# peternara/FashionVisualExpl-recommend

Hardware: AMD Instinct MI355X
Metric: BPR triplets/sec (higher is better)
Workload: dtype bf16

## Files before the change

fashionvisualexpl_recommend_amd/_ffi.py:

```python
import ctypes as C
import os

HERE = os.path.dirname(os.path.abspath(__file__))
LIB_PATH = os.environ.get("BPRX_LIB") or os.path.join(HERE, "libbprx.so")
ABI_VERSION = 6
FLAG_EXPORT_USER_GRAD = 1
FLAG_EXPORT_ITEM_GRAD = 2
FLAG_DENSE_ALLREDUCE = 4
FLAG_ADAM_SWEEP, FLAG_ADAM_LAZY = 8, 16

MODEL = {"bprmf": 0, "vbpr": 1}
OPTIMIZER = {"sgd": 0, "adam_tf23": 1}
FEAT_DTYPE = {"fp32": 0, "bf16": 1, "fp8": 2}
E_INVALID, E_STATE = -1, -2
E_RANGE, E_NOMEM = -4, -5
PHASES = ["cast_Et", "proj_fwd", "triplet_grad", "proj_bwd", "reduce_parts", "apply", "dense_update", "loss_reduce", "item_seg", "seg_alloc", "row_count", "adam_catchup"]


class BprxError(RuntimeError):
    def __init__(self, code, msg):
        super().__init__("libbprx error %d: %s" % (code, msg))
        self.code = code


class Config(C.Structure):
    _fields_ = [("abi_version", C.c_int32), ("model", C.c_int32), ("num_users", C.c_int32), ("num_items", C.c_int32),
                ("embed_k", C.c_int32), ("embed_d", C.c_int32), ("feat_dim", C.c_int32), ("feat_dtype", C.c_int32),
                ("optimizer", C.c_int32), ("device", C.c_int32), ("max_batch", C.c_int64),
                ("lr", C.c_float), ("reg", C.c_float), ("beta1", C.c_float), ("beta2", C.c_float),
                ("epsilon", C.c_float), ("flags", C.c_int32), ("feat_scale", C.c_float)]


FACTORED_FIELDS = ["Ea", "Eb", "A", "Ap", "m_Ea", "v_Ea", "m_Eb", "v_Eb", "m_A", "v_A", "m_Ap", "v_Ap"]


class Factored(C.Structure):
    _fields_ = [("feat_dim_a", C.c_int32), ("feat_dim_b", C.c_int32), ("embed_a", C.c_int32), ("embed_b", C.c_int32),
                ("neg_bias_reg", C.c_float)] + [(n, C.c_void_p) for n in FACTORED_FIELDS]


ACF_WEIGHTS = ["component.W_0_u", "component.W_0_i", "component.b_0", "component.W_1", "component.b_1",
               "item.W_0_u", "item.W_0_iv", "item.W_0_ip", "item.W_0_ix", "item.b_0", "item.W_1", "item.b_1"]


ACF_GRADIENT = {"detached": 0, "full": 1}


class Acf(C.Structure):
    _fields_ = [("feat_m", C.c_int32), ("feat_c", C.c_int32), ("width_c", C.c_int32), ("width_i", C.c_int32),
                ("feat_dtype", C.c_int32), ("F", C.c_void_p), ("train_ptr", C.c_void_p), ("train_items", C.c_void_p),
                ("eval_ptr", C.c_void_p), ("eval_items", C.c_void_p), ("Pi", C.c_void_p), ("m_Pi", C.c_void_p),
                ("v_Pi", C.c_void_p), ("w", C.c_void_p * 12), ("m_w", C.c_void_p * 12), ("v_w", C.c_void_p * 12)]


AF_WEIGHTS = ["color.W1", "color.b1", "color.W2", "edges.conv", "edges.conv_b", "edges.W2", "class.W1", "class.b1", "class.W2",
              "attention.W_1", "attention.b_1", "attention.W_2", "attention.b_2"]


class Attentive(C.Structure):
    _fields_ = [("dim_color", C.c_int32), ("dim_class", C.c_int32), ("width", C.c_int32), ("dropout", C.c_float),
                ("seed", C.c_uint64), ("edges", C.c_void_p), ("color", C.c_void_p), ("cls", C.c_void_p),
                ("w", C.c_void_p * 13), ("m_w", C.c_void_p * 13), ("v_w", C.c_void_p * 13)]


TABLE_FIELDS = ["Gu", "Gi", "Bi", "Tu", "F", "E", "Bp", "m_Gu", "v_Gu", "m_Gi", "v_Gi", "m_Bi", "v_Bi",
                "m_Tu", "v_Tu", "m_E", "v_E", "m_Bp", "v_Bp"]


class Tables(C.Structure):
    _fields_ = [(n, C.c_void_p) for n in TABLE_FIELDS]


_lib = None


def lib():
    global _lib
    if _lib is not None:
        return _lib
    import torch
    if not os.path.exists(LIB_PATH):
        raise ImportError("libbprx.so not found at %s: build it with `python -m fashionvisualexpl_recommend_amd.build` "
                          "(hipcc --offload-arch=gfx950); there is no CPU fallback" % LIB_PATH)
    L = C.CDLL(LIB_PATH)
    vp, i32, i64, u32, f32 = C.c_void_p, C.c_int32, C.c_int64, C.c_uint32, C.c_float
    sig = {
        "bprx_abi_version": (C.c_int, []),
        "bprx_create": (C.c_int, [C.POINTER(Config), C.POINTER(vp)]),
        "bprx_destroy": (C.c_int, [vp]),
        "bprx_last_error": (C.c_char_p, [vp]),
        "bprx_live_device_allocs": (i64, []),
        "bprx_bind_tables": (C.c_int, [vp, C.POINTER(Tables)]),
        "bprx_bind_factored": (C.c_int, [vp, C.POINTER(Tables), C.POINTER(Factored)]),
        "bprx_explain_pairs": (C.c_int, [vp, vp, vp, i64, vp, vp]),
        "bprx_feat_explain": (C.c_int, [vp, vp, vp, vp, i64, i32, i32, vp, vp, vp, vp, vp, vp, vp]),
        "bprx_proj_stride": (i32, [vp]),
        "bprx_project_rows": (C.c_int, [vp, vp, i64, vp, vp]),
        "bprx_score_new_block": (C.c_int, [vp, i32, i32, vp, i64, vp, vp]),
        "bprx_topk_rows": (C.c_int, [vp, i64, i32, vp, i32, vp, vp, vp, vp]),
        "bprx_feat_explain_new": (C.c_int, [vp, vp, i64, vp, vp, i64, i32, i32, vp, vp, vp, vp, vp]),
        "bprx_bind_acf": (C.c_int, [vp, C.POINTER(Tables), C.POINTER(Acf)]),
        "bprx_acf_profiles": (C.c_int, [vp, vp, i64, vp, vp, vp, vp]),
        "bprx_acf_explain": (C.c_int, [vp, vp, vp, i64, vp, vp, i32, vp, vp, vp, vp, vp, vp, vp, vp, vp, vp]),
        "bprx_acf_set_gradient": (C.c_int, [vp, C.c_int]),
        "bprx_acf_get_gradient": (C.c_int, [vp]),
        "bprx_bind_attentive": (C.c_int, [vp, C.POINTER(Tables), C.POINTER(Attentive)]),
        "bprx_af_encode": (C.c_int, [vp, vp, i64, vp, vp]),
        "bprx_af_attention_pairs": (C.c_int, [vp, vp, vp, i64, vp, vp, vp]),
        "bprx_af_explain": (C.c_int, [vp, vp, vp, i64, i32, vp, vp, vp, vp, vp, vp, vp]),
        "bprx_af_score_block": (C.c_int, [vp, C.c_int32, C.c_int32, vp, vp, vp]),
        "bprx_af_dropout_mask": (C.c_int, [vp, i64, i64, vp, vp]),
        "bprx_af_get_step": (i64, [vp]),
        "bprx_af_set_step": (C.c_int, [vp, i64]),
        "bprx_set_hyper": (C.c_int, [vp, f32, f32]),
        "bprx_tables_dirty": (C.c_int, [vp, vp]),
        "bprx_set_adam_step": (C.c_int, [vp, i64, vp]),
        "bprx_get_adam_step": (i64, [vp]),
        "bprx_adam_is_lazy": (C.c_int, [vp]),
        "bprx_sync_adam": (C.c_int, [vp, vp]),
        "bprx_score_pairs": (C.c_int, [vp, vp, vp, i64, vp, vp]),
        "bprx_step": (C.c_int, [vp, vp, vp, vp, i64, vp, vp]),
        "bprx_step_begin": (C.c_int, [vp, vp, vp, vp, i64, vp]),
        "bprx_step_begin_sparse": (C.c_int, [vp, vp, vp, vp, i64, vp]),
        "bprx_step_begin_dense": (C.c_int, [vp, vp]),
        "bprx_dense_grad": (C.c_int, [vp, C.POINTER(vp), C.POINTER(i64)]),
        "bprx_step_end": (C.c_int, [vp, vp, vp]),
        "bprx_step_project": (C.c_int, [vp, vp]),
        "bprx_user_grad": (C.c_int, [vp, C.POINTER(vp), C.POINTER(vp)]),
        "bprx_clear_user_grad": (C.c_int, [vp, i64, i32, vp]),
        "bprx_item_grad": (C.c_int, [vp, C.POINTER(vp), C.POINTER(vp)]),
        "bprx_clear_item_grad": (C.c_int, [vp, i64, i32, vp]),
        "bprx_scatter_add": (C.c_int, [vp, i32, i32, vp, vp, i64, f32, vp]),
        "bprx_route_reset": (C.c_int, [vp, i64, vp, i32, vp]),
        "bprx_route_plan": (C.c_int, [vp, i64, vp, i64, i32, i32, i32, i32, vp, vp, vp, vp, vp, vp]),
        "bprx_route_gather": (C.c_int, [vp, i32, vp, i32, i32, vp, i64, vp, vp, vp]),
        "bprx_route_unpack": (C.c_int, [vp, vp, i64, vp, i32, vp, i32, vp, vp, i32, vp]),
        "bprx_route_gather_checked": (C.c_int, [vp, i32, vp, i32, i32, vp, i64, vp, vp, vp, vp]),
        "bprx_route_unpack_checked": (C.c_int, [vp, vp, i64, vp, i32, vp, i32, vp, vp, i32, vp, vp]),
        "bprx_route_pack": (C.c_int, [vp, i32, vp, i32, vp, i64, vp, vp, vp, i32, f32, vp, vp, i64, vp, i32, vp]),
        "bprx_route_scatter_add": (C.c_int, [vp, i32, vp, i32, i32, vp, vp, i64, f32, vp, vp]),
        "bprx_score_block": (C.c_int, [vp, i32, i32, vp, vp]),
        "bprx_eval_users": (C.c_int, [vp, i32, i32, vp, vp, vp, vp, vp, i32, vp, vp]),
        "bprx_topk": (C.c_int, [vp, i32, i32, vp, vp, vp, i32, vp, vp, vp, vp]),
        "bprx_eval_pos": (C.c_int, [vp, i32, i32, vp, i32, i32, vp, vp, vp, vp]),
        "bprx_eval_counts": (C.c_int, [vp, i32, i32, vp, i32, i32, vp, vp, vp, vp, vp, vp, vp]),
        "bprx_eval_finish": (C.c_int, [vp, i32, i32, i32, vp, vp, vp, i32, vp, vp]),
        "bprx_sync_check": (C.c_int, [vp, vp]),
        "bprx_probe_stream_read": (i64, [vp, i64, vp, vp]),
        "bprx_probe_stream_read_nt": (i64, [vp, i64, vp, vp]),
        "bprx_probe_row_gather": (i64, [vp, i64, i32, vp, i64, i32, vp, vp]),
        "bprx_profile_enable": (C.c_int, [vp, C.c_int]),
        "bprx_profile_read": (C.c_int, [vp, vp, vp]),
        "bprx_sample_philox": (C.c_int, [vp, vp, vp, i64, i32, C.c_uint64, C.c_uint64, i64, vp, vp, vp, vp]),
        "bprx_user_msg_floats": (C.c_int64, [vp, i64]),
        "bprx_pack_user_msg": (C.c_int, [vp, vp, i64, i64, vp, vp]),
        "bprx_apply_user_msgs": (C.c_int, [vp, vp, i32, i64, C.c_float, vp]),
        "bprx_sum_dense_parts": (C.c_int, [vp, vp, i32, vp]),
        "bprx_epoch_prepare": (C.c_int, [C.c_uint64, u32, i32, vp, vp, vp, vp]),
        "bprx_epoch_slots": (C.c_int, [vp, i32, vp, i64, vp]),
        "bprx_sample_epoch": (C.c_int, [vp, vp, vp, vp, vp, i32, i32, C.c_uint64, u32, i64, i64, vp, vp, vp, vp]),
        "bprx_index_pass_kind": (C.c_int, [vp]),
        "bprx_proj_mask_kind": (C.c_int, [vp]),
        "bprx_adam_rows": (C.c_int, [vp, vp, vp, vp, i64, C.c_float, C.c_float, C.c_float, C.c_float, vp]),
        "bprx_step_lr": (C.c_int, [vp, vp]),
        "bprx_sample_philox_h": (C.c_int, [vp, vp, vp, vp, i64, i32, C.c_uint64, C.c_uint64, i64, vp, vp, vp, i64, i64, vp]),
        "bprx_sample_epoch_h": (C.c_int, [vp, vp, vp, vp, vp, vp, i32, i32, C.c_uint64, u32, i64, i64, vp, vp, vp, i64, i64, vp]),
        "bprx_sampler_create": (C.c_int, [vp, vp, i32, i32, C.POINTER(vp)]),
        "bprx_sampler_destroy": (C.c_int, [vp]),
        "bprx_sampler_count": (i64, [vp, i32, i32]),
        "bprx_sampler_ref_stream": (i64, [vp, i32, i32, u32, u32, vp, vp, vp, i64]),
    }
    for name, (res, args) in sig.items():
        fn = getattr(L, name)
        fn.restype, fn.argtypes = res, args
    if L.bprx_abi_version() != ABI_VERSION:
        raise ImportError("libbprx.so ABI %d != binding ABI %d" % (L.bprx_abi_version(), ABI_VERSION))
    _lib = L
    return L


EXPORTS = ["bprx_abi_version", "bprx_create", "bprx_destroy", "bprx_last_error", "bprx_live_device_allocs", "bprx_bind_tables", "bprx_bind_factored", "bprx_explain_pairs", "bprx_feat_explain", "bprx_proj_stride", "bprx_project_rows", "bprx_score_new_block", "bprx_topk_rows", "bprx_feat_explain_new", "bprx_bind_acf", "bprx_acf_profiles", "bprx_acf_explain", "bprx_acf_set_gradient", "bprx_acf_get_gradient", "bprx_bind_attentive", "bprx_af_encode", "bprx_af_attention_pairs", "bprx_af_explain",
           "bprx_af_score_block", "bprx_af_dropout_mask", "bprx_af_get_step", "bprx_af_set_step", "bprx_set_hyper", "bprx_tables_dirty",
           "bprx_set_adam_step", "bprx_get_adam_step", "bprx_adam_is_lazy", "bprx_sync_adam", "bprx_score_pairs", "bprx_step", "bprx_step_begin",
           "bprx_step_begin_sparse", "bprx_step_begin_dense", "bprx_sum_dense_parts",
           "bprx_dense_grad", "bprx_step_end", "bprx_step_project", "bprx_user_grad", "bprx_clear_user_grad", "bprx_item_grad", "bprx_clear_item_grad",
           "bprx_scatter_add", "bprx_route_reset", "bprx_route_plan", "bprx_route_gather", "bprx_route_unpack", "bprx_route_gather_checked",
           "bprx_route_unpack_checked", "bprx_route_pack",
           "bprx_route_scatter_add", "bprx_score_block", "bprx_eval_users", "bprx_eval_pos", "bprx_eval_counts", "bprx_eval_finish", "bprx_topk", "bprx_sync_check", "bprx_probe_stream_read", "bprx_probe_stream_read_nt", "bprx_probe_row_gather", "bprx_profile_enable",
           "bprx_profile_read", "bprx_sample_philox", "bprx_epoch_prepare", "bprx_epoch_slots", "bprx_sample_epoch", "bprx_sample_philox_h", "bprx_sample_epoch_h", "bprx_index_pass_kind", "bprx_proj_mask_kind", "bprx_adam_rows", "bprx_step_lr", "bprx_user_msg_floats", "bprx_pack_user_msg",
           "bprx_apply_user_msgs", "bprx_sampler_create",
           "bprx_sampler_destroy", "bprx_sampler_count", "bprx_sampler_ref_stream"]


def check(handle, rc):
    if rc < 0:
        msg = lib().bprx_last_error(handle)
        raise BprxError(rc, msg.decode() if msg else "?")
    return rc
```

fashionvisualexpl_recommend_amd/csrc/bprx_api.hip:

```cpp
#include <math.h>
#include <stdlib.h>
#include <algorithm>
#include <new>

#include "bprx_internal.h"

static char g_create_err[512] = "";

static int check_ready(bprx_handle *h, int64_t B);

extern "C" int bprx_abi_version(void) { return BPRX_ABI_VERSION; }

extern "C" const char *bprx_last_error(const bprx_handle *h) { return h ? h->err : g_create_err; }

extern "C" int64_t bprx_live_device_allocs(void) { return bprx_live_allocs.load(); }

static int env_int(const char *name, int fallback) {
  const char *e = getenv(name);
  return e ? atoi(e) : fallback;
}

extern "C" int bprx_create(const bprx_config *cfg, bprx_handle **out) {
#define CFAIL(code, ...)                                        \
  do {                                                          \
    snprintf(g_create_err, sizeof(g_create_err), __VA_ARGS__);  \
    return (code);                                              \
  } while (0)
  if (!cfg || !out) CFAIL(BPRX_E_INVALID, "bprx_create: null argument");
  *out = nullptr;
  if (cfg->abi_version != BPRX_ABI_VERSION)
    CFAIL(BPRX_E_INVALID, "bprx_create: abi_version %d, library is %d", cfg->abi_version, BPRX_ABI_VERSION);
  if (cfg->model != BPRX_MODEL_BPRMF && cfg->model != BPRX_MODEL_VBPR) CFAIL(BPRX_E_INVALID, "unknown model %d", cfg->model);
  if (cfg->optimizer != BPRX_OPT_SGD && cfg->optimizer != BPRX_OPT_ADAM_TF23)
    CFAIL(BPRX_E_INVALID, "unknown optimizer %d", cfg->optimizer);
  if (cfg->num_users <= 0 || cfg->num_items <= 0 || cfg->embed_k <= 0 || cfg->max_batch <= 0)
    CFAIL(BPRX_E_INVALID, "num_users, num_items, embed_k and max_batch must be positive");
  const bool vb = cfg->model == BPRX_MODEL_VBPR;
  if (vb) {
    if (cfg->embed_d <= 0 || cfg->feat_dim <= 0) CFAIL(BPRX_E_INVALID, "VBPR needs embed_d > 0 and feat_dim > 0");
    if (cfg->embed_d > 271) CFAIL(BPRX_E_INVALID, "embed_d %d > 271 unsupported", cfg->embed_d);
    if (cfg->feat_dtype != BPRX_F_FP32 && cfg->feat_dtype != BPRX_F_BF16 && cfg->feat_dtype != BPRX_F_FP8)
      CFAIL(BPRX_E_INVALID, "unknown feat_dtype");
    if (cfg->feat_dtype == BPRX_F_BF16 && cfg->feat_dim % 128 != 0)
      CFAIL(BPRX_E_INVALID, "bf16 features need feat_dim %% 128 == 0 (got %d)", cfg->feat_dim);
    if (cfg->feat_dtype == BPRX_F_FP8 && cfg->feat_dim % 256 != 0)
      CFAIL(BPRX_E_INVALID, "fp8 features need feat_dim %% 256 == 0 (got %d)", cfg->feat_dim);
    if (cfg->feat_dtype == BPRX_F_FP8 && !(cfg->feat_scale > 0.f)) CFAIL(BPRX_E_INVALID, "fp8 features need feat_scale > 0");
  }
  const bool exported = cfg->flags & (BPRX_FLAG_EXPORT_USER_GRAD | BPRX_FLAG_EXPORT_ITEM_GRAD);
  bool adam_lazy = false;
  if (cfg->optimizer == BPRX_OPT_ADAM_TF23) {
    const double chain_us = 20.0 * (double)cfg->num_users / (double)cfg->max_batch * 0.45;
    const double sweep_us =
        ((double)cfg->num_users * (cfg->embed_k + (vb ? cfg->embed_d : 0)) + (double)cfg->num_items * (cfg->embed_k + 1)) * 24.0 / 4e6;
    adam_lazy = exported ? true : chain_us < sweep_us;
    if (cfg->flags & BPRX_FLAG_ADAM_SWEEP) adam_lazy = false;
    if (cfg->flags & BPRX_FLAG_ADAM_LAZY) adam_lazy = true;
    adam_lazy = env_int("BPRX_ADAM_LAZY", adam_lazy) != 0;
  }
  if (exported && cfg->optimizer != BPRX_OPT_SGD && !adam_lazy)
    CFAIL(BPRX_E_INVALID, "BPRX_FLAG_EXPORT_*_GRAD with adam_tf23 needs the lazy form (BPRX_ADAM_LAZY != 0)");
  if ((cfg->flags & BPRX_FLAG_EXPORT_ITEM_GRAD) && cfg->model != BPRX_MODEL_BPRMF)
    CFAIL(BPRX_E_INVALID, "BPRX_FLAG_EXPORT_ITEM_GRAD is for BPRMF (VBPR keeps its items and features local)");
  hipError_t e = hipSetDevice(cfg->device);
  if (e != hipSuccess) CFAIL(BPRX_E_HIP, "hipSetDevice(%d): %s", cfg->device, hipGetErrorString(e));

  bprx_handle *h = new (std::nothrow) bprx_handle();
  if (!h) CFAIL(BPRX_E_NOMEM, "out of host memory");
#define HFAIL(code, ...)         \
  do {                           \
    bprx_destroy(h);             \
    CFAIL(code, __VA_ARGS__);    \
  } while (0)
  h->cfg = *cfg;
  h->adam_lazy = adam_lazy;
  h->neg_bias_reg = 0.1f;
  if (!vb) { h->cfg.embed_d = 0; h->cfg.feat_dim = 0; }
  const size_t U = cfg->num_users, I = cfg->num_items, k = cfg->embed_k, d = h->cfg.embed_d, D = h->cfg.feat_dim;
  const size_t MB = cfg->max_batch;
  hipDeviceProp_t prop;
  h->num_cu = hipGetDeviceProperties(&prop, cfg->device) == hipSuccess ? prop.multiProcessorCount : 256;
  DevPool &A = h->mem;
  A.zeros(&h->dGu, U * k);
  A.zeros(&h->dGi, I * k);
  A.zeros(&h->dBi, I);
  A.zeros(&h->flagU, U);
  A.zeros(&h->flagI, I);
  A.zeros(&h->lossb, MB);
  A.zeros(&h->loss_acc, (size_t)BPRX_DENSE_BLOCKS);
  A.zeros(&h->errflag, (size_t)1);
  if (cfg->flags & BPRX_FLAG_EXPORT_USER_GRAD) A.zeros(&h->msg_cursor, (size_t)2);
  A.zeros(&h->cntU, U);
  A.zeros(&h->cntI, I);
  if (vb) {
    h->PS = 16 * (int)((d + 1 + 15) / 16);
    const size_t PS = h->PS;
    const int mr = (int)((D + 255) / 256);
    h->SK = (h->num_cu + mr - 1) / mr;
    if (cfg->feat_dtype == BPRX_F_FP8 && PS / 16 <= 9) h->SK *= 2;
    if (h->SK > 64) h->SK = 64;
    if (h->SK < 1) h->SK = 1;
    h->fwd_variant = env_int("BPRX_FWD_VARIANT", 4);
    h->proj_mask = std::min(std::max(env_int("BPRX_PROJ_MASK", 1), 0), 2);
    A.zeros(&h->dTu, U * d);
    A.zeros(&h->P, I * PS);
    A.zeros(&h->W, I * PS);
    A.zeros((uint16_t **)&h->Wb, I * PS);
    A.zeros(&h->Ppair, MB * PS);
    A.zeros((uint16_t **)&h->Et, PS * D);
    A.zeros((uint16_t **)&h->EtF, PS * D);
    if (cfg->feat_dtype == BPRX_F_FP8 && PS / 16 >= 10) A.zeros((uint8_t **)&h->EtS, PS * D);
    A.zeros(&h->dEp, D * d + D);
    A.zeros(&h->part, (size_t)h->SK * D * PS);
    A.zeros(&h->qs, (size_t)4);
    if (cfg->feat_dtype != BPRX_F_FP32)
      A.zeros((uint8_t **)&h->Ft, (size_t)((I + 31) / 32 * 32) * D * (cfg->feat_dtype == BPRX_F_FP8 ? 1 : 2));
  }
  {
    const bool fits = k % 4 == 0 && d % 4 == 0 && k <= 256 && d <= 256;
    h->seg_policy = (fits && !(cfg->flags & BPRX_FLAG_EXPORT_ITEM_GRAD)) ? std::min(std::max(env_int("BPRX_ITEM_MODE", 1), 0), 2) : 0;
    if (h->seg_policy) {
      h->seg_lead_cap = (int64_t)(I + 8192 + 4 * 1024 + 2 * MB / 64 + 64 + 64);
      h->seg_ent_cap = (int64_t)(6 * MB + 64 * 1024 + 2048);
      h->idx8_shift = 0;
      for (int sh = 8; sh <= 13 && !h->idx8_shift; ++sh)
        if ((((int64_t)I - 1) >> sh) <= 255) h->idx8_shift = sh;
      A.zeros(&h->seg_rank, (size_t)2 * MB);
      A.zeros(&h->seg_cnt, I); A.zeros(&h->seg_ptr, I);
      A.zeros(&h->seg_cursor, (size_t)6);
      A.zeros((int4 **)&h->seg_lead, (size_t)h->seg_lead_cap);
      A.zeros(&h->hot_done, I);
      A.zeros((int2 **)&h->seg_ent, (size_t)h->seg_ent_cap);
      A.zeros(&h->uslot_of, U); A.zeros(&h->ulist, MB);
      A.zeros(&h->uold, MB * (k + d));
      if (h->idx8_shift) { A.zeros(&h->own8, (size_t)2 * MB); A.zeros(&h->loc8, (size_t)2 * MB * (h->idx8_shift > 8 ? 2 : 1)); }
    }
  }
  h->list_policy = vb ? std::min(std::max(env_int("BPRX_LIST_MODE", 1), 0), 2) : 0;
  if (h->list_policy) {
    const size_t cap = 2 * MB < I ? 2 * MB : I;
    A.zeros(&h->ilist, cap); A.zeros(&h->ilist_n, (size_t)2);
  }
  h->step.SK_step = h->SK;
  if (h->adam_lazy) {
    A.zeros(&h->lastU, U); A.zeros(&h->lastI, I);
    A.zeros(&h->lr_hist, (size_t)ADAM_HIST);
  }
  h->fast_rows = (cfg->optimizer == BPRX_OPT_SGD && !(cfg->flags & BPRX_FLAG_EXPORT_USER_GRAD)) ? 1 : 0;
  if (h->fast_rows && !exported) {
    A.zeros(&h->slist, (size_t)3 * MB); A.zeros(&h->slist_n, (size_t)2);
  }
  if ((e = A.err) != hipSuccess) HFAIL(BPRX_E_NOMEM, "scratch allocation failed: %s", hipGetErrorString(e));
  if (vb && cfg->optimizer == BPRX_OPT_ADAM_TF23 && h->adam_lazy && env_int("BPRX_SIDE_STREAM", 1) != 0 &&
      (hipStreamCreateWithFlags(&h->side, hipStreamNonBlocking) != hipSuccess ||
       hipEventCreateWithFlags(&h->ev_fork, hipEventDisableTiming) != hipSuccess ||
       hipEventCreateWithFlags(&h->ev_join, hipEventDisableTiming) != hipSuccess))
    HFAIL(BPRX_E_HIP, "side stream / event creation failed");
  *out = h;
  return BPRX_OK;
#undef HFAIL
#undef CFAIL
}

extern "C" int bprx_destroy(bprx_handle *h) {
  if (!h) return BPRX_OK;
  (void)hipSetDevice(h->cfg.device);
  if (h->side) (void)hipStreamSynchronize(h->side);
  (void)h->mem.rollback(0);
  bprx_acf_free(h);
  bprx_af_free(h);
  if (h->side) (void)hipStreamDestroy(h->side);
  if (h->ev_fork) (void)hipEventDestroy(h->ev_fork);
  if (h->ev_join) (void)hipEventDestroy(h->ev_join);
  for (auto &r : h->prof_pending) { (void)hipEventDestroy(r.a); (void)hipEventDestroy(r.b); }
  for (auto e : h->prof_free) (void)hipEventDestroy(e);
  delete h;
  return BPRX_OK;
}

extern "C" int bprx_profile_enable(bprx_handle *h, int on) {
  if (!h) return BPRX_E_INVALID;
  h->prof = on != 0;
  return BPRX_OK;
}

extern "C" int bprx_profile_read(bprx_handle *h, double *ms, int64_t *launches) {
  if (!h || !ms || !launches) return BPRX_E_INVALID;
  for (auto &r : h->prof_pending) {
    BPRX_HIP(h, hipEventSynchronize(r.b));
    float t = 0.f;
    BPRX_HIP(h, hipEventElapsedTime(&t, r.a, r.b));
    ms[r.phase] += (double)t;
    launches[r.phase] += 1;
    h->prof_free.push_back(r.a);
    h->prof_free.push_back(r.b);
  }
  h->prof_pending.clear();
  return BPRX_OK;
}

static int bind_tables(bprx_handle *h, const bprx_tables *t, bool factored) {
  if (!h || !t) return BPRX_E_INVALID;
  if (!t->Gu || !t->Gi || !t->Bi) BPRX_FAIL(h, BPRX_E_INVALID, "bind_tables: Gu, Gi, Bi are required");
  const bool vb = h->cfg.model == BPRX_MODEL_VBPR;
  if (vb && (!t->Tu || !t->F || !t->E || !t->Bp)) BPRX_FAIL(h, BPRX_E_INVALID, "bind_tables: VBPR needs Tu, F, E, Bp");
  if (h->cfg.optimizer == BPRX_OPT_ADAM_TF23) {
    if (!t->m_Gu || !t->v_Gu || !t->m_Gi || !t->v_Gi || !t->m_Bi || !t->v_Bi)
      BPRX_FAIL(h, BPRX_E_INVALID, "bind_tables: adam_tf23 needs m_/v_ slots for Gu, Gi, Bi");
    if (vb && (!t->m_Tu || !t->v_Tu || (!factored && (!t->m_E || !t->v_E || !t->m_Bp || !t->v_Bp))))
      BPRX_FAIL(h, BPRX_E_INVALID, "bind_tables: adam_tf23 needs m_/v_ slots for Tu, E, Bp");
  }
  if (((uintptr_t)t->Gu | (uintptr_t)t->Gi | (uintptr_t)t->Tu | (uintptr_t)t->F | (uintptr_t)t->E) & 15)
    BPRX_FAIL(h, BPRX_E_INVALID, "bind_tables: table base pointers must be 16-byte aligned");
  h->t = *t;
  h->factored = factored;
  if (!factored) h->neg_bias_reg = 0.1f;
  h->et_valid = h->p_valid = h->absmax_valid = false;
  {
    const int rc = bprx_launch_tile_F(h);
    if (rc) return rc;
  }
  h->bound = true;
  return bprx_launch_adam_reset(h, h->adam_t, 0);
}

extern "C" int bprx_bind_tables(bprx_handle *h, const bprx_tables *t) {
  if (h && h->acf) bprx_acf_free(h);
  if (h && h->af) bprx_af_free(h);
  return bind_tables(h, t, false);
}

int bprx_bind_tables_internal(bprx_handle *h, const bprx_tables *t) { return bind_tables(h, t, false); }

extern "C" int bprx_bind_factored(bprx_handle *h, const bprx_tables *t, const bprx_factored *f) {
  if (!h || !t || !f) return BPRX_E_INVALID;
  const bprx_config &c = h->cfg;
  if (c.model != BPRX_MODEL_VBPR) BPRX_FAIL(h, BPRX_E_INVALID, "bind_factored: needs a VBPR handle");
  if (c.feat_dtype == BPRX_F_FP8) BPRX_FAIL(h, BPRX_E_INVALID, "bind_factored: fp8 features are not supported (fp32 or bf16)");
  if (c.flags & (BPRX_FLAG_EXPORT_USER_GRAD | BPRX_FLAG_EXPORT_ITEM_GRAD))
    BPRX_FAIL(h, BPRX_E_INVALID, "bind_factored: exported gradients (multi-GPU) are not supported");
  if (f->feat_dim_a <= 0 || f->feat_dim_b <= 0 || (int64_t)f->feat_dim_a + f->feat_dim_b > c.feat_dim)
    BPRX_FAIL(h, BPRX_E_INVALID, "bind_factored: need Dc, De > 0 and Dc + De <= feat_dim (%d, %d, %d)", f->feat_dim_a,
              f->feat_dim_b, c.feat_dim);
  if (f->embed_a <= 0 || f->embed_b <= 0 || f->embed_a > 256 || f->embed_b > 256)
    BPRX_FAIL(h, BPRX_E_INVALID, "bind_factored: embed_a, embed_b must lie in [1, 256] (%d, %d)", f->embed_a, f->embed_b);
  if (!(f->neg_bias_reg >= 0.f)) BPRX_FAIL(h, BPRX_E_INVALID, "bind_factored: neg_bias_reg must be >= 0");
  if (!f->Ea || !f->Eb || !f->A || !f->Ap) BPRX_FAIL(h, BPRX_E_INVALID, "bind_factored: Ea, Eb, A, Ap are required");
  if (c.optimizer == BPRX_OPT_ADAM_TF23 &&
      (!f->m_Ea || !f->v_Ea || !f->m_Eb || !f->v_Eb || !f->m_A || !f->v_A || !f->m_Ap || !f->v_Ap))
    BPRX_FAIL(h, BPRX_E_INVALID, "bind_factored: adam_tf23 needs m_/v_ slots for Ea, Eb, A, Ap");
  if (!h->gF) {
    const size_t n = (size_t)f->feat_dim_a * f->embed_a + (size_t)f->feat_dim_b * f->embed_b +
                     (size_t)(f->embed_a + f->embed_b) * (c.embed_d + 1);
    const hipError_t e = h->mem.regrow(&h->gF, n);
    if (e != hipSuccess) BPRX_FAIL(h, BPRX_E_HIP, "bind_factored: factor gradient (%zu floats): %s", n, hipGetErrorString(e));
  } else if (f->feat_dim_a != h->fx.feat_dim_a || f->feat_dim_b != h->fx.feat_dim_b || f->embed_a != h->fx.embed_a ||
             f->embed_b != h->fx.embed_b) {
    BPRX_FAIL(h, BPRX_E_INVALID, "bind_factored: the factor shapes of a handle cannot change");
  }
  int rc = bind_tables(h, t, true);
  if (rc) return rc;
  h->fx = *f;
  h->neg_bias_reg = f->neg_bias_reg;
  if ((rc = bprx_launch_fact_compose(h, nullptr))) return rc;
  BPRX_HIP(h, hipStreamSynchronize(nullptr));
  return BPRX_OK;
}

extern "C" int bprx_explain_pairs(bprx_handle *h, const int32_t *user, const int32_t *item, int64_t n, float *out, void *stream) {
  int rc = check_ready(h, 0);
  if (rc) return rc;
  if (!h->factored) BPRX_FAIL(h, BPRX_E_STATE, "explain_pairs: the handle is not bound with bprx_bind_factored");
  if (n < 0 || n > ((int64_t)1 << 32)) BPRX_FAIL(h, BPRX_E_INVALID, "explain_pairs: n = %lld out of range", (long long)n);
  if (n == 0) return BPRX_OK;
  if (!user || !item || !out) BPRX_FAIL(h, BPRX_E_INVALID, "explain_pairs: null pointer");
  hipStream_t s = (hipStream_t)stream;
  if ((rc = bprx_launch_adam_sync(h, h->adam_t, s))) return rc;
  return bprx_launch_explain(h, user, item, n, out, s);
}

extern "C" int bprx_tables_dirty(bprx_handle *h, void *stream) {
  if (!h) return BPRX_E_INVALID;
  h->et_valid = h->p_valid = h->absmax_valid = false;
  if (h->acf) bprx_acf_invalidate(h);
  if (h->af) bprx_af_invalidate(h);
  if (h->bound && h->factored) {
    const int rc = bprx_launch_fact_compose(h, (hipStream_t)stream);
    if (rc) return rc;
  }
  return h->bound ? bprx_launch_adam_reset(h, h->adam_t, (hipStream_t)stream) : BPRX_OK;
}

extern "C" int bprx_set_hyper(bprx_handle *h, float lr, float reg) {
  if (!h) return BPRX_E_INVALID;
  h->cfg.lr = lr;
  h->cfg.reg = reg;
  return BPRX_OK;
}

extern "C" int bprx_set_adam_step(bprx_handle *h, int64_t it, void *stream) {
  if (!h || it < 0) return BPRX_E_INVALID;
  h->adam_t = it;
  return h->bound ? bprx_launch_adam_reset(h, it, (hipStream_t)stream) : BPRX_OK;
}

extern "C" int64_t bprx_get_adam_step(const bprx_handle *h) { return h ? h->adam_t : -1; }
extern "C" int bprx_adam_is_lazy(const bprx_handle *h) { return h ? (h->adam_lazy ? 1 : 0) : BPRX_E_INVALID; }

static int check_ready(bprx_handle *h, int64_t B) {
  if (!h) return BPRX_E_INVALID;
  if (!h->bound) BPRX_FAIL(h, BPRX_E_STATE, "tables not bound (call bprx_bind_tables first)");
  if (B < 0 || B > h->cfg.max_batch) BPRX_FAIL(h, BPRX_E_INVALID, "B=%lld outside [0, max_batch=%lld]", (long long)B, (long long)h->cfg.max_batch);
  return BPRX_OK;
}

extern "C" int bprx_sync_adam(bprx_handle *h, void *stream) {
  int rc = check_ready(h, 0);
  if (rc) return rc;
  return bprx_launch_adam_sync(h, h->adam_t, (hipStream_t)stream);
}

extern "C" int bprx_score_pairs(bprx_handle *h, const int32_t *user, const int32_t *item, int64_t B, float *x, void *stream) {
  int rc = check_ready(h, B);
  if (rc) return rc;
  if (B == 0) return BPRX_OK;
  if (!user || !item || !x) BPRX_FAIL(h, BPRX_E_INVALID, "score_pairs: null pointer");
  hipStream_t s = (hipStream_t)stream;
  if (h->acf) return bprx_acf_score_pairs(h, user, item, B, x, s);
  if (h->af) return bprx_af_pairs(h, user, item, B, x, nullptr, s);
  if ((rc = bprx_launch_adam_sync(h, h->adam_t, s))) return rc;
  if (h->cfg.model == BPRX_MODEL_VBPR) {
    if (h->p_valid) return bprx_launch_score(h, user, item, B, nullptr, 0, x, s);
    if ((rc = bprx_launch_cast_Et(h, s))) return rc;
    if ((rc = bprx_launch_proj_fwd(h, item, B, nullptr, 0, h->Ppair, s))) return rc;
    return bprx_launch_score(h, user, item, B, h->Ppair, 1, x, s);
  }
  return bprx_launch_score(h, user, item, B, nullptr, 0, x, s);
}

static void commit_plan(bprx_handle *h, const StepPlan &p) {
  h->step = p;
  h->step_stage = 1;
  h->adam_t = p.adam_t;
  if (p.B == 0) return;
  h->idx8_n = 0;
  h->proj_fresh = false;
  h->W_dirty = p.leaves_w_dirty;
  if (p.item_mode) h->seg_slot ^= 1;
  if (p.use_list) h->slist_slot ^= 1;
}

static int launch_sparse_half(bprx_handle *h, const StepPlan &p, hipStream_t s) {
  int rc;
  if (p.adam_sync_first && (rc = bprx_launch_adam_sync(h, p.adam_t - 1, s))) return rc;
  if (p.catchup_aside) {
    BPRX_HIP(h, hipEventRecord(h->ev_fork, s));
    BPRX_HIP(h, hipStreamWaitEvent(h->side, h->ev_fork, 0));
    if ((rc = bprx_launch_adam_catchup(h, p, h->side))) return rc;
    BPRX_HIP(h, hipEventRecord(h->ev_join, h->side));
  } else if (p.catchup && (rc = bprx_launch_adam_catchup(h, p, s))) return rc;
  if (p.project && p.list_mode && (rc = bprx_launch_cast_Et(h, s))) return rc;
  if (p.index_first && (rc = bprx_launch_index_pass(h, p, s))) return rc;
  if (p.project && !p.list_mode && (rc = bprx_launch_cast_Et(h, s))) return rc;
  if (p.fwd) {
    rc = p.list_mode ? bprx_launch_proj_fwd(h, h->ilist, p.list_bound, p.list_cur, 1, h->P, s)
                     : bprx_launch_proj_fwd(h, nullptr, h->cfg.num_items, nullptr, 0, h->P, s, p.mask ? h->seg_cnt : nullptr);
    if (rc) return rc;
  }
  if (p.catchup_aside) BPRX_HIP(h, hipStreamWaitEvent(s, h->ev_join, 0));
  if (p.B == 0) return BPRX_OK;
  if (!p.index_first && (rc = bprx_launch_index_pass(h, p, s))) return rc;
  return bprx_launch_triplet_grad(h, p, s);
}

static int step_begin_sparse(bprx_handle *h, const int32_t *user, const int32_t *pos, const int32_t *neg, int64_t B, bool fused_reduce,
                             hipStream_t s) {
  int rc = check_ready(h, B);
  if (rc) return rc;
  if (h->step_stage) BPRX_FAIL(h, BPRX_E_STATE, "step_begin called twice without step_end");
  if (h->acf) BPRX_FAIL(h, BPRX_E_STATE, "step_begin: an ACF handle takes whole steps only (bprx_step)");
  if (h->af) BPRX_FAIL(h, BPRX_E_STATE, "step_begin: an AttentiveFashion handle takes whole steps only (bprx_step)");
  if (B && (!user || !pos || !neg)) BPRX_FAIL(h, BPRX_E_INVALID, "step: null index pointer");
  const StepPlan plan = plan_step(*h, user, pos, neg, B, fused_reduce);
  if (plan.error == PLAN_E_EMPTY) BPRX_FAIL(h, BPRX_E_INVALID, "step: empty batch");
  commit_plan(h, plan);
  rc = launch_sparse_half(h, h->step, s);
  if (rc) h->step_stage = 0;
  return rc;
}

extern "C" int bprx_step_begin_sparse(bprx_handle *h, const int32_t *user, const int32_t *pos, const int32_t *neg, int64_t B, void *stream) {
  return step_begin_sparse(h, user, pos, neg, B, false, (hipStream_t)stream);
}

extern "C" int bprx_step_begin_dense(bprx_handle *h, void *stream) {
  if (!h) return BPRX_E_INVALID;
  if (h->step_stage != 1) BPRX_FAIL(h, BPRX_E_STATE, "step_begin_dense without step_begin_sparse");
  hipStream_t s = (hipStream_t)stream;
  const StepPlan &p = h->step;
  const bool vb = h->cfg.model == BPRX_MODEL_VBPR;
  int rc;
  if (p.B == 0) {
    if (vb) BPRX_HIP(h, hipMemsetAsync(h->dEp, 0, ((size_t)h->cfg.feat_dim * (h->cfg.embed_d + 1)) * sizeof(float), s));
  } else {
    if (p.item_mode && (rc = bprx_launch_item_seg(h, p, s))) return rc;
    if (vb && (rc = bprx_launch_proj_bwd(h, p, s))) return rc;
    if (p.apply != APPLY_NONE && (rc = bprx_launch_apply(h, p, s))) return rc;
  }
  h->step_stage = 2;
  return BPRX_OK;
}

static int step_begin(bprx_handle *h, const int32_t *user, const int32_t *pos, const int32_t *neg, int64_t B, bool fused_reduce,
                      void *stream) {
  int rc = step_begin_sparse(h, user, pos, neg, B, fused_reduce, (hipStream_t)stream);
  if (!rc && (rc = bprx_step_begin_dense(h, stream))) h->step_stage = 0;
  return rc;
}

extern "C" int bprx_step_begin(bprx_handle *h, const int32_t *user, const int32_t *pos, const int32_t *neg, int64_t B, void *stream) {
  return step_begin(h, user, pos, neg, B, false, stream);
}

extern "C" int bprx_step_project(bprx_handle *h, void *stream) {
  int rc = check_ready(h, 0);
  if (rc) return rc;
  if (h->cfg.model != BPRX_MODEL_VBPR) return BPRX_OK;
  hipStream_t s = (hipStream_t)stream;
  if ((rc = bprx_launch_cast_Et(h, s))) return rc;
  if (!h->p_valid && (rc = bprx_launch_proj_fwd(h, nullptr, h->cfg.num_items, nullptr, 0, h->P, s))) return rc;
  h->p_valid = true;
  h->proj_fresh = true;
  return BPRX_OK;
}

extern "C" int bprx_user_grad(bprx_handle *h, float **dGu, float **dTu) {
  if (!h || !dGu || !dTu) return BPRX_E_INVALID;
  *dGu = h->dGu;
  *dTu = h->dTu;
  return BPRX_OK;
}

extern "C" int bprx_clear_user_grad(bprx_handle *h, int64_t n_rows, int32_t marks_only, void *stream) {
  if (!h || n_rows < 0 || n_rows > h->cfg.num_users) return BPRX_E_INVALID;
  hipStream_t s = (hipStream_t)stream;
  if (!marks_only) {
    BPRX_HIP(h, hipMemsetAsync(h->dGu, 0, (size_t)n_rows * h->cfg.embed_k * sizeof(float), s));
    if (h->cfg.embed_d) BPRX_HIP(h, hipMemsetAsync(h->dTu, 0, (size_t)n_rows * h->cfg.embed_d * sizeof(float), s));
  }
  BPRX_HIP(h, hipMemsetAsync(h->flagU, 0, (size_t)n_rows * sizeof(uint32_t), s));
  return BPRX_OK;
}

extern "C" int bprx_item_grad(bprx_handle *h, float **dGi, float **dBi) {
  if (!h || !dGi || !dBi) return BPRX_E_INVALID;
  *dGi = h->dGi;
  *dBi = h->dBi;
  return BPRX_OK;
}

extern "C" int bprx_clear_item_grad(bprx_handle *h, int64_t n_rows, int32_t marks_only, void *stream) {
  if (!h || n_rows < 0 || n_rows > h->cfg.num_items) return BPRX_E_INVALID;
  hipStream_t s = (hipStream_t)stream;
  if (!marks_only) {
    BPRX_HIP(h, hipMemsetAsync(h->dGi, 0, (size_t)n_rows * h->cfg.embed_k * sizeof(float), s));
    BPRX_HIP(h, hipMemsetAsync(h->dBi, 0, (size_t)n_rows * sizeof(float), s));
  }
  BPRX_HIP(h, hipMemsetAsync(h->flagI, 0, (size_t)n_rows * sizeof(uint32_t), s));
  return BPRX_OK;
}

extern "C" int bprx_dense_grad(bprx_handle *h, float **ptr, int64_t *count) {
  if (!h || !ptr || !count) return BPRX_E_INVALID;
  *ptr = h->dEp;
  *count = h->cfg.model == BPRX_MODEL_VBPR ? (int64_t)h->cfg.feat_dim * (h->cfg.embed_d + 1) : 0;
  return BPRX_OK;
}

extern "C" int bprx_step_end(bprx_handle *h, float *loss_out, void *stream) {
  if (!h) return BPRX_E_INVALID;
  if (!h->step_stage) BPRX_FAIL(h, BPRX_E_STATE, "step_end without step_begin");
  if (h->step_stage != 2) BPRX_FAIL(h, BPRX_E_STATE, "step_end before step_begin_dense");
  hipStream_t s = (hipStream_t)stream;
  const StepPlan &p = h->step;
  int rc;
  h->step_stage = 0;
  if (h->factored && (rc = bprx_launch_fact_update(h, p.lr_t, s))) return rc;
  if (p.dense_launch && (rc = bprx_launch_dense_update(h, p, s))) return rc;
  if (h->cfg.model == BPRX_MODEL_VBPR) {
    if (p.dense_launch) h->absmax_valid = h->cfg.feat_dtype == BPRX_F_FP8;
    if (p.list_mode) h->list_slot ^= 1;
    h->et_valid = p.dense_launch && h->cfg.feat_dtype == BPRX_F_BF16;
    h->p_valid = false;
  }
  if (loss_out && (rc = bprx_launch_loss_reduce(h, p.B, loss_out, s))) return rc;
  return BPRX_OK;
}

extern "C" int bprx_step(bprx_handle *h, const int32_t *user, const int32_t *pos, const int32_t *neg, int64_t B,
                         float *loss_out, void *stream) {
  if (!h) return BPRX_E_INVALID;
  if (h->acf) {
    const int rc = check_ready(h, B);
    return rc ? rc : bprx_acf_step(h, user, pos, neg, B, loss_out, (hipStream_t)stream);
  }
  if (h->af) {
    const int rc = check_ready(h, B);
    return rc ? rc : bprx_af_step(h, user, pos, neg, B, loss_out, (hipStream_t)stream);
  }
  int rc = step_begin(h, user, pos, neg, B, true, stream);
  if (!rc) rc = bprx_step_end(h, loss_out, stream);
  return rc;
}

extern "C" int bprx_score_block(bprx_handle *h, int32_t u0, int32_t u1, float *out, void *stream) {
  int rc = check_ready(h, 0);
  if (rc) return rc;
  if (u0 < 0 || u1 > h->cfg.num_users || u0 > u1 || !out) BPRX_FAIL(h, BPRX_E_INVALID, "score_block: bad user range [%d,%d)", u0, u1);
  if (u0 == u1) return BPRX_OK;
  hipStream_t s = (hipStream_t)stream;
  if ((rc = bprx_launch_adam_sync(h, h->adam_t, s))) return rc;
  if (h->af) return bprx_af_block(h, u0, u1, out, nullptr, s);
  if (h->acf) {
    if ((rc = bprx_acf_eval_profiles(h, s))) return rc;
    float *gu = h->t.Gu;
    h->t.Gu = bprx_acf_eval_gu(h);
    rc = h->cfg.embed_k % 2 == 0 ? bprx_launch_score_gemm(h, u0, u1, out, s) : bprx_launch_score_block(h, u0, u1, out, s);
    h->t.Gu = gu;
    return rc;
  }
  if (h->cfg.model == BPRX_MODEL_VBPR && !h->p_valid) {
    if ((rc = bprx_launch_cast_Et(h, s))) return rc;
    if ((rc = bprx_launch_proj_fwd(h, nullptr, h->cfg.num_items, nullptr, 0, h->P, s))) return rc;
    h->p_valid = true;
  }
  if (h->cfg.embed_k % 2 == 0 && h->cfg.embed_d % 2 == 0)
    return bprx_launch_score_gemm(h, u0, u1, out, s);
  return bprx_launch_score_block(h, u0, u1, out, s);
}

int bprx_new_items_check(bprx_handle *h, const char *what, int64_t n) {
  if (!h) return BPRX_E_INVALID;
  if (h->cfg.model != BPRX_MODEL_VBPR || h->acf || h->af)
    BPRX_FAIL(h, BPRX_E_INVALID, "%s: needs a VBPR handle (bprx_bind_tables or bprx_bind_factored)", what);
  if (h->cfg.feat_dtype == BPRX_F_FP8)
    BPRX_FAIL(h, BPRX_E_INVALID, "%s: fp8 features are not supported for new items (a new row may exceed the max-abs the codes "
              "were scaled for and would saturate): fp32 or bf16", what);
  if (n < 0 || n >= ((int64_t)1 << 31)) BPRX_FAIL(h, BPRX_E_INVALID, "%s: n = %lld out of range", what, (long long)n);
  if (!h->bound) BPRX_FAIL(h, BPRX_E_STATE, "tables not bound (call bprx_bind_tables first)");
  return BPRX_OK;
}

extern "C" int32_t bprx_proj_stride(const bprx_handle *h) {
  return h && h->cfg.model == BPRX_MODEL_VBPR ? h->PS : BPRX_E_INVALID;
}

extern "C" int bprx_project_rows(bprx_handle *h, const void *Fnew, int64_t n, float *P, void *stream) {
  int rc = bprx_new_items_check(h, "project_rows", n);
  if (rc) return rc;
  if (n == 0) return BPRX_OK;
  if (!Fnew || !P) BPRX_FAIL(h, BPRX_E_INVALID, "project_rows: null pointer");
  if ((uintptr_t)Fnew & 15) BPRX_FAIL(h, BPRX_E_INVALID, "project_rows: the table must be 16-byte aligned");
  hipStream_t s = (hipStream_t)stream;
  if ((rc = bprx_launch_adam_sync(h, h->adam_t, s))) return rc;
  if ((rc = bprx_launch_cast_Et(h, s))) return rc;
  return bprx_launch_proj_new(h, Fnew, n, P, s);
}

extern "C" int bprx_step_lr(const bprx_handle *h, float *lr_t) {
  if (!h || !lr_t) return BPRX_E_INVALID;
  *lr_t = h->step.lr_t;
  return BPRX_OK;
}

extern "C" int bprx_index_pass_kind(const bprx_handle *h) { return h ? h->step.idx_kind : 0; }
extern "C" int bprx_proj_mask_kind(const bprx_handle *h) {
  if (!h || !h->step.mask) return 0;
  const bool fwd = bprx_proj_fwd_takes_mask(*h), bwd = bprx_proj_bwd_takes_mask(*h);
  return fwd ? (bwd ? 1 : 2) : (bwd ? 3 : 0);
}

extern "C" int bprx_sync_check(bprx_handle *h, void *stream) {
  if (!h) return BPRX_E_INVALID;
  hipStream_t s = (hipStream_t)stream;
  int32_t flag = 0;
  BPRX_HIP(h, hipMemcpyAsync(&flag, h->errflag, sizeof(flag), hipMemcpyDeviceToHost, s));
  BPRX_HIP(h, hipStreamSynchronize(s));
  if (flag) {
    BPRX_HIP(h, hipMemsetAsync(h->errflag, 0, sizeof(flag), s));
    BPRX_FAIL(h, BPRX_E_RANGE, "a user/item index was out of range (code %d); it was clamped, results are invalid", flag);
  }
  return BPRX_OK;
}
```

fashionvisualexpl_recommend_amd/csrc/bprx_eval.hip:

```cpp
#include "bprx_internal.h"

namespace {

typedef __attribute__((ext_vector_type(16))) float f32x16;

constexpr int TM = 128, TN = 128, GKC = 16, GLD = GKC + 1;

struct GemmArgs {
  const float *Gu, *Gi, *Bi, *Tu, *P;
  int U, I, k, d, PS;
};

__device__ __forceinline__ void gemm_phase(const float *__restrict__ A, int lda, int arow0, int arows,
                                           const float *__restrict__ Bm, int ldb, int brow0, int brows, int K,
                                           float (*As)[GLD], float (*Bs)[GLD], f32x16 (&acc)[2][2], int wr, int wc, int lane) {
  const int t = threadIdx.x;
  for (int k0 = 0; k0 < K; k0 += GKC) {
    __syncthreads();
    {
      const int r = t >> 1, c0 = (t & 1) * 8;
#pragma unroll
      for (int x = 0; x < 8; ++x) {
        const int kk = k0 + c0 + x;
        As[r][c0 + x] = (r < arows && kk < K) ? A[(size_t)(arow0 + r) * lda + kk] : 0.f;
// ... 265 lines not shown
  __shared__ uint32_t ckey[TOPK_MAX];
  __shared__ int cidx[TOPK_MAX];
  const int u = u0 + blockIdx.x, tid = threadIdx.x;
  float *s = S + (size_t)blockIdx.x * I;
  const int64_t t0 = tr_ptr ? tr_ptr[u] : 0;
  const int ntr = tr_ptr ? (int)(tr_ptr[u + 1] - t0) : 0;
  for (int q = tid; q < ntr; q += 256) {
    const int it = tr_items[t0 + q];
    if ((unsigned)it < (unsigned)I) s[it] = -INFINITY;
  }
  const int Kc = K < I ? K : I;
  if (tid == 0) { s_prefix = 0; s_mask = 0; s_remaining = Kc; s_ngt = 0; s_neq = 0; s_bad = K > I ? 1 : 0; }
  __syncthreads();
  for (int pass = 3; pass >= 0; --pass) {
    hist[tid] = 0;
    __syncthreads();
    const uint32_t prefix = s_prefix, mask = s_mask;
    for (int i = tid; i < I; i += 256) {
      const uint32_t key = f2key(s[i]);
      if ((key & mask) == prefix) atomicAdd(&hist[(key >> (8 * pass)) & 255], 1);
    }
    __syncthreads();
    if (tid == 0) {
      int rem = s_remaining, b = 255;
      for (; b > 0; --b) {
        if (hist[b] >= rem) break;
        rem -= hist[b];
      }
      s_remaining = rem;
      s_prefix = prefix | ((uint32_t)b << (8 * pass));
      s_mask = mask | (255u << (8 * pass));
    }
    __syncthreads();
  }
  const uint32_t kth = s_prefix;
  const int want_eq = s_remaining;
  for (int i = tid; i < I; i += 256) {
    const uint32_t key = f2key(s[i]);
    if (key > kth) {
      const int p = atomicAdd(&s_ngt, 1);
      ckey[p] = key; cidx[p] = i;
    } else if (key == kth) {
      const int e = atomicAdd(&s_neq, 1);
      if (e < want_eq) { ckey[Kc - want_eq + e] = key; cidx[Kc - want_eq + e] = i; }
    }
  }
  __syncthreads();
  if (tid == 0 && (s_neq != want_eq || kth == f2key(-INFINITY))) s_bad = 1;
  __syncthreads();
  int n2 = 1;
  while (n2 < Kc) n2 <<= 1;
  for (int q = Kc + tid; q < n2; q += 256) { ckey[q] = 0u; cidx[q] = 0x7fffffff; }
  __syncthreads();
  for (int size = 2; size <= n2; size <<= 1) {
    for (int stride = size >> 1; stride > 0; stride >>= 1) {
      for (int q = tid; q < n2; q += 256) {
        const int partner = q ^ stride;
        if (partner > q) {
          const bool desc = (q & size) == 0;
          const uint32_t ka = ckey[q], kb = ckey[partner];
          const int ia = cidx[q], ib = cidx[partner];
          const bool a_better = ka > kb || (ka == kb && ia < ib);
          if (a_better != desc) { ckey[q] = kb; ckey[partner] = ka; cidx[q] = ib; cidx[partner] = ia; }
        }
      }
      __syncthreads();
    }
  }
  for (int q = tid; q < Kc; q += 256) {
    if (q + 1 < Kc && ckey[q] == ckey[q + 1]) s_bad = 1;
    idx_out[(size_t)blockIdx.x * K + q] = cidx[q];
    val_out[(size_t)blockIdx.x * K + q] = s[cidx[q]];
  }
  for (int q = Kc + tid; q < K; q += 256) { idx_out[(size_t)blockIdx.x * K + q] = -1; val_out[(size_t)blockIdx.x * K + q] = 0.f; }
  __syncthreads();
  if (tid == 0) flag_out[blockIdx.x] = s_bad;
}

}

extern "C" int bprx_topk(bprx_handle *h, int32_t u0, int32_t u1, float *scores, const int64_t *train_ptr,
                         const int32_t *train_items, int32_t K, int32_t *idx, float *val, int32_t *flag, void *stream) {
  if (!h) return BPRX_E_INVALID;
  if (u0 < 0 || u1 > h->cfg.num_users || u0 > u1 || !scores || !train_ptr || !train_items || !idx || !val || !flag)
    BPRX_FAIL(h, BPRX_E_INVALID, "topk: bad argument");
  if (K <= 0 || K > TOPK_MAX) BPRX_FAIL(h, BPRX_E_INVALID, "topk: K=%d outside [1, %d]", K, TOPK_MAX);
  if (u0 == u1) return BPRX_OK;
  hipLaunchKernelGGL(k_topk, dim3(u1 - u0), dim3(256), 0, (hipStream_t)stream, scores, u0, h->cfg.num_items, train_ptr,
                     train_items, K, idx, val, flag);
  BPRX_LAUNCH_CHECK(h, "k_topk");
  return BPRX_OK;
}

extern "C" int bprx_topk_rows(bprx_handle *h, int64_t nrows, int32_t width, float *scores, int32_t K, int32_t *idx, float *val,
                              int32_t *flag, void *stream) {
  const int rc = bprx_new_items_check(h, "topk_rows", nrows);
  if (rc) return rc;
  if (width < 1) BPRX_FAIL(h, BPRX_E_INVALID, "topk_rows: width = %d < 1", width);
  if (K <= 0 || K > TOPK_MAX) BPRX_FAIL(h, BPRX_E_INVALID, "topk_rows: K=%d outside [1, %d]", K, TOPK_MAX);
  if (nrows == 0) return BPRX_OK;
  if (!scores || !idx || !val || !flag) BPRX_FAIL(h, BPRX_E_INVALID, "topk_rows: null pointer");
  hipLaunchKernelGGL(k_topk, dim3((unsigned)nrows), dim3(256), 0, (hipStream_t)stream, scores, 0, width, (const int64_t *)nullptr,
                     (const int32_t *)nullptr, K, idx, val, flag);
  BPRX_LAUNCH_CHECK(h, "k_topk<rows>");
  return BPRX_OK;
}

extern "C" int bprx_score_new_block(bprx_handle *h, int32_t u0, int32_t u1, const float *P, int64_t n, float *out, void *stream) {
  int rc = bprx_new_items_check(h, "score_new_block", n);
  if (rc) return rc;
  if (u0 < 0 || u1 > h->cfg.num_users || u0 > u1) BPRX_FAIL(h, BPRX_E_INVALID, "score_new_block: bad user range [%d,%d)", u0, u1);
  if (n == 0 || u0 == u1) return BPRX_OK;
  if (!P || !out) BPRX_FAIL(h, BPRX_E_INVALID, "score_new_block: null pointer");
  hipStream_t s = (hipStream_t)stream;
  if ((rc = bprx_launch_adam_sync(h, h->adam_t, s))) return rc;
  if ((rc = bprx_launch_cast_Et(h, s))) return rc;
  dim3 grid((unsigned)((n + TN - 1) / TN), (unsigned)((u1 - u0 + TM - 1) / TM));
  hipLaunchKernelGGL(k_score_new_gemm, grid, dim3(256), 0, s, (const float *)h->t.Tu, P, (int)n, h->cfg.embed_d, h->PS, u0, u1, out);
  BPRX_LAUNCH_CHECK(h, "k_score_new_gemm");
  return BPRX_OK;
}

int bprx_launch_score_gemm(bprx_handle *h, int32_t u0, int32_t u1, float *out, hipStream_t s) {
  GemmArgs g;
  g.Gu = h->t.Gu; g.Gi = h->t.Gi; g.Bi = h->t.Bi; g.Tu = h->t.Tu; g.P = h->P;
  g.U = h->cfg.num_users; g.I = h->cfg.num_items; g.k = h->cfg.embed_k; g.d = h->cfg.embed_d; g.PS = h->PS;
  dim3 grid((g.I + TN - 1) / TN, (u1 - u0 + TM - 1) / TM);
  hipLaunchKernelGGL(k_score_gemm, grid, dim3(256), 0, s, g, u0, u1, out);
  BPRX_LAUNCH_CHECK(h, "k_score_gemm");
  return BPRX_OK;
}

extern "C" int bprx_eval_users(bprx_handle *h, int32_t u0, int32_t u1, const float *scores, const int64_t *train_ptr,
                               const int32_t *train_items, const int64_t *eval_ptr, const int32_t *eval_items, int32_t K,
                               double *out, void *stream) {
  if (!h) return BPRX_E_INVALID;
  if (u0 < 0 || u1 > h->cfg.num_users || u0 > u1 || !scores || !train_ptr || !train_items || !eval_ptr || !eval_items ||
      !out || K <= 0)
    BPRX_FAIL(h, BPRX_E_INVALID, "eval_users: bad argument");
  if (u0 == u1) return BPRX_OK;
  hipLaunchKernelGGL(k_eval_users, dim3(u1 - u0), dim3(256), 0, (hipStream_t)stream, scores, u0, h->cfg.num_items, train_ptr,
                     train_items, eval_ptr, eval_items, K, out, h->errflag);
  BPRX_LAUNCH_CHECK(h, "k_eval_users");
  return BPRX_OK;
}

extern "C" int bprx_eval_pos(bprx_handle *h, int32_t u0, int32_t u1, const float *scores, int32_t item_lo, int32_t items_total,
                             const int64_t *eval_ptr, const int32_t *eval_items, float *sp, void *stream) {
  if (!h) return BPRX_E_INVALID;
  if (u0 < 0 || u0 > u1 || !scores || !eval_ptr || !eval_items || !sp || item_lo < 0 || items_total <= 0)
    BPRX_FAIL(h, BPRX_E_INVALID, "eval_pos: bad argument");
  if (u0 == u1) return BPRX_OK;
  const int nb = u1 - u0;
  hipLaunchKernelGGL(k_eval_pos, dim3((unsigned)(((int64_t)nb * EVMAX + 255) / 256)), dim3(256), 0, (hipStream_t)stream, scores, u0,
                     nb, h->cfg.num_items, item_lo, items_total, eval_ptr, eval_items, sp, h->errflag);
  BPRX_LAUNCH_CHECK(h, "k_eval_pos");
  return BPRX_OK;
}

extern "C" int bprx_eval_counts(bprx_handle *h, int32_t u0, int32_t u1, const float *scores, int32_t item_lo, int32_t items_total,
                                const int64_t *train_ptr, const int32_t *train_items, const int64_t *eval_ptr,
                                const int32_t *eval_items, const float *sp, int32_t *counts, void *stream) {
  if (!h) return BPRX_E_INVALID;
  if (u0 < 0 || u0 > u1 || !scores || !train_ptr || !train_items || !eval_ptr || !eval_items || !sp || !counts || item_lo < 0)
    BPRX_FAIL(h, BPRX_E_INVALID, "eval_counts: bad argument");
  if (u0 == u1) return BPRX_OK;
  hipLaunchKernelGGL(k_eval_counts, dim3(u1 - u0), dim3(256), 0, (hipStream_t)stream, scores, u0, h->cfg.num_items, item_lo,
                     items_total, train_ptr, train_items, eval_ptr, eval_items, sp, counts);
  BPRX_LAUNCH_CHECK(h, "k_eval_counts");
  return BPRX_OK;
}

extern "C" int bprx_eval_finish(bprx_handle *h, int32_t u0, int32_t u1, int32_t items_total, const int64_t *eval_ptr,
                                const float *sp, const int32_t *counts, int32_t K, double *out, void *stream) {
  if (!h) return BPRX_E_INVALID;
  if (u0 < 0 || u0 > u1 || !eval_ptr || !sp || !counts || !out || K <= 0 || items_total <= 0)
    BPRX_FAIL(h, BPRX_E_INVALID, "eval_finish: bad argument");
  if (u0 == u1) return BPRX_OK;
  const int nb = u1 - u0;
  hipLaunchKernelGGL(k_eval_finish, dim3((unsigned)((nb + 255) / 256)), dim3(256), 0, (hipStream_t)stream, u0, nb, items_total,
                     eval_ptr, sp, counts, K, out);
  BPRX_LAUNCH_CHECK(h, "k_eval_finish");
  return BPRX_OK;
}
```

fashionvisualexpl_recommend_amd/csrc/bprx_explain.hip:

```cpp
#include "bprx_internal.h"

namespace {

constexpr int FX_TILE = 32;

struct FeatExplainArgs {
  const float *Gu, *Gi, *Bi, *Tu, *E, *Bp;
  const void *F;
  const int32_t *user, *item;
  int64_t n;
  int U, I, k, d, D, ncols, top;
  int e_vec;
  int map_vec;
  float feat_scale;
  float *score, *base, *visual;
  int32_t *col;
  float *contrib, *map;
  int32_t *errflag;
};

__device__ __forceinline__ float e4m3fn_value(uint32_t b) {
  const uint32_t s = (b & 0x80u) << 24, e = (b >> 3) & 15u, m = b & 7u;
  if (e == 15u && m == 7u) return __uint_as_float(s | 0x7fc00000u);
  if (e == 0u) {
// ... 117 lines not shown
          }
#pragma unroll
          for (int j = 0; j < V; ++j) c[j] = f[j] * wc[j];
#pragma unroll
          for (int j = 0; j < V; ++j)
            if (c0 + j < ncols) acc = acc + c[j];
          if (mrow) {
            if (V >= 4 && A.map_vec) {
#pragma unroll
              for (int j = 0; j + 3 < V; j += 4)
                if (c0 + j < ncols) *reinterpret_cast<float4 *>(mrow + c0 + j) = make_float4(c[j], c[j + 1], c[j + 2], c[j + 3]);
            } else {
#pragma unroll
              for (int j = 0; j < V; ++j)
                if (c0 + j < ncols) mrow[c0 + j] = c[j];
            }
          }
        } else {
#pragma unroll
          for (int j = 0; j < V; ++j) c[j] = 0.f;
        }
#pragma unroll
        for (int j = 0; j < V; ++j) {
          const int cc = c0 + j;
          unsigned long long m = __ballot(cc < ncols && (cnt < top || ranks_before(c[j], cc, thr_v, thr_c)));
          while (m) {
            const int src = __ffsll((long long)m) - 1;
            m &= m - 1;
            const float cv = __shfl(c[j], src, 64);
            const int ccol = cb + src * V + j;
            if (cnt < top || ranks_before(cv, ccol, thr_v, thr_c)) {
              const int rank = __popcll(__ballot(lane < cnt && ranks_before(tv, tp, cv, ccol)));
              const float uv = __shfl_up(tv, 1, 64);
              const int up = __shfl_up(tp, 1, 64);
              if (lane == rank) {
                tv = cv;
                tp = ccol;
              } else if (lane > rank && lane < top) {
                tv = uv;
                tp = up;
              }
              if (cnt < top) ++cnt;
              if (cnt == top) {
                thr_v = __shfl(tv, top - 1, 64);
                thr_c = __shfl(tp, top - 1, 64);
              }
            }
          }
        }
      }
      const float visual = wave_sum(acc);
      if (lane == 0) {
        if constexpr (NEW) {
          A.score[p] = visual;
        } else {
          A.base[p] = base;
          A.visual[p] = visual;
          A.score[p] = base + visual;
        }
      }
      if (lane < top) {
        A.col[p * top + lane] = lane < cnt ? tp : -1;
        A.contrib[p * top + lane] = lane < cnt ? tv : 0.f;
      }
    }
    __syncthreads();
    s = e;
  }
}

template <typename FT, bool NEW = false>
void launch(const FeatExplainArgs &A, bool vec, unsigned blocks, size_t lds, hipStream_t s) {
  constexpr int V = 16 / (int)sizeof(FT);
  if (vec) hipLaunchKernelGGL((k_feat_explain<FT, V, NEW>), dim3(blocks), dim3(256), lds, s, A);
  else hipLaunchKernelGGL((k_feat_explain<FT, 1, NEW>), dim3(blocks), dim3(256), lds, s, A);
}

}

extern "C" int bprx_feat_explain(bprx_handle *h, const void *F, const int32_t *user, const int32_t *item, int64_t n, int32_t ncols,
                                 int32_t top, float *score, float *base, float *visual, int32_t *col, float *contrib, float *map,
                                 void *stream) {
  if (!h) return BPRX_E_INVALID;
  if (!h->bound) BPRX_FAIL(h, BPRX_E_STATE, "tables not bound (call bprx_bind_tables first)");
  if (h->cfg.model != BPRX_MODEL_VBPR || h->acf || h->af)
    BPRX_FAIL(h, BPRX_E_STATE, "feat_explain: needs a VBPR handle (bprx_bind_tables or bprx_bind_factored)");
  const bprx_config &c = h->cfg;
  if (n < 0 || n >= ((int64_t)1 << 31)) BPRX_FAIL(h, BPRX_E_INVALID, "feat_explain: n = %lld out of range", (long long)n);
  if (ncols < 1 || ncols > c.feat_dim) BPRX_FAIL(h, BPRX_E_INVALID, "feat_explain: ncols = %d outside [1, feat_dim = %d]", ncols, c.feat_dim);
  if (top < 1 || top > 32) BPRX_FAIL(h, BPRX_E_INVALID, "feat_explain: top = %d outside [1, 32]", top);
  if (c.feat_dim > 16384)
    BPRX_FAIL(h, BPRX_E_INVALID, "feat_explain: feat_dim = %d > 16384 (one user's fp32 w row must fit in 64 KB of LDS)", c.feat_dim);
  if (n == 0) return BPRX_OK;
  if (!F || !user || !item || !score || !base || !visual || !col || !contrib) BPRX_FAIL(h, BPRX_E_INVALID, "feat_explain: null pointer");
  hipStream_t s = (hipStream_t)stream;
  const int rc = bprx_launch_adam_sync(h, h->adam_t, s);
  if (rc) return rc;
  FeatExplainArgs A;
  A.Gu = h->t.Gu; A.Gi = h->t.Gi; A.Bi = h->t.Bi; A.Tu = h->t.Tu; A.E = h->t.E; A.Bp = h->t.Bp;
  A.F = F; A.user = user; A.item = item; A.n = n;
  A.U = c.num_users; A.I = c.num_items; A.k = c.embed_k; A.d = c.embed_d; A.D = c.feat_dim; A.ncols = ncols; A.top = top;
  A.e_vec = c.embed_d % 4 == 0;
  A.map_vec = map && ncols % 4 == 0 && ((uintptr_t)map & 15) == 0;
  A.feat_scale = c.feat_dtype == BPRX_F_FP8 ? c.feat_scale : 1.0f;
  A.score = score; A.base = base; A.visual = visual; A.col = col; A.contrib = contrib; A.map = map;
  A.errflag = h->errflag;
  const size_t esz = c.feat_dtype == BPRX_F_FP32 ? 4 : (c.feat_dtype == BPRX_F_BF16 ? 2 : 1);
  const bool vec = ((uintptr_t)F & 15) == 0 && ((size_t)c.feat_dim * esz) % 16 == 0;
  const unsigned blocks = (unsigned)((n + FX_TILE - 1) / FX_TILE);
  const size_t lds = (size_t)c.feat_dim * sizeof(float);
  if (c.feat_dtype == BPRX_F_BF16) launch<uint16_t>(A, vec, blocks, lds, s);
  else if (c.feat_dtype == BPRX_F_FP8) launch<uint8_t>(A, vec, blocks, lds, s);
  else launch<float>(A, vec, blocks, lds, s);
  BPRX_LAUNCH_CHECK(h, "k_feat_explain");
  return BPRX_OK;
}

extern "C" int bprx_feat_explain_new(bprx_handle *h, const void *Fnew, int64_t n_new, const int32_t *user, const int32_t *row,
                                     int64_t n, int32_t ncols, int32_t top, float *score, int32_t *col, float *contrib, float *map,
                                     void *stream) {
  int rc = bprx_new_items_check(h, "feat_explain_new", n);
  if (rc) return rc;
  const bprx_config &c = h->cfg;
  if (n_new < 0 || n_new >= ((int64_t)1 << 31)) BPRX_FAIL(h, BPRX_E_INVALID, "feat_explain_new: n_new = %lld out of range", (long long)n_new);
  if (ncols < 1 || ncols > c.feat_dim) BPRX_FAIL(h, BPRX_E_INVALID, "feat_explain_new: ncols = %d outside [1, feat_dim = %d]", ncols, c.feat_dim);
  if (top < 1 || top > 32) BPRX_FAIL(h, BPRX_E_INVALID, "feat_explain_new: top = %d outside [1, 32]", top);
  if (c.feat_dim > 16384)
    BPRX_FAIL(h, BPRX_E_INVALID, "feat_explain_new: feat_dim = %d > 16384 (one user's fp32 w row must fit in 64 KB of LDS)", c.feat_dim);
  if (n == 0) return BPRX_OK;
  if (n_new == 0) BPRX_FAIL(h, BPRX_E_INVALID, "feat_explain_new: %lld pairs of an empty table", (long long)n);
  if (!Fnew || !user || !row || !score || !col || !contrib) BPRX_FAIL(h, BPRX_E_INVALID, "feat_explain_new: null pointer");
  hipStream_t s = (hipStream_t)stream;
  if ((rc = bprx_launch_adam_sync(h, h->adam_t, s))) return rc;
  if ((rc = bprx_launch_cast_Et(h, s))) return rc;
  FeatExplainArgs A;
  A.Gu = nullptr; A.Gi = nullptr; A.Bi = nullptr; A.Tu = h->t.Tu; A.E = h->t.E; A.Bp = h->t.Bp;
  A.F = Fnew; A.user = user; A.item = row; A.n = n;
  A.U = c.num_users; A.I = (int)n_new; A.k = c.embed_k; A.d = c.embed_d; A.D = c.feat_dim; A.ncols = ncols; A.top = top;
  A.e_vec = c.embed_d % 4 == 0;
  A.map_vec = map && ncols % 4 == 0 && ((uintptr_t)map & 15) == 0;
  A.feat_scale = 1.0f;
  A.score = score; A.base = nullptr; A.visual = nullptr; A.col = col; A.contrib = contrib; A.map = map;
  A.errflag = h->errflag;
  const size_t esz = c.feat_dtype == BPRX_F_FP32 ? 4 : 2;
  const bool vec = ((uintptr_t)Fnew & 15) == 0 && ((size_t)c.feat_dim * esz) % 16 == 0;
  const unsigned blocks = (unsigned)((n + FX_TILE - 1) / FX_TILE);
  const size_t lds = (size_t)c.feat_dim * sizeof(float);
  if (c.feat_dtype == BPRX_F_BF16) launch<uint16_t, true>(A, vec, blocks, lds, s);
  else launch<float, true>(A, vec, blocks, lds, s);
  BPRX_LAUNCH_CHECK(h, "k_feat_explain<new>");
  return BPRX_OK;
}
```

fashionvisualexpl_recommend_amd/csrc/bprx_internal.h:

```cpp
#pragma once
#include <hip/hip_runtime.h>
#include <math.h>
#include <stdint.h>
#include <stdio.h>
#include <string.h>

#include <atomic>
#include <utility>
#include <vector>

#include "bprx.h"
#include "bprx_device.h"

#define BPRX_DENSE_BLOCKS 2048

inline std::atomic<int64_t> bprx_live_allocs{0};

struct DevPool {
  struct Rec { void **slot; void *p; };
  std::vector<Rec> recs;
  hipError_t err = hipSuccess;

  DevPool() = default;
  DevPool(const DevPool &) = delete;
  DevPool &operator=(const DevPool &) = delete;
  ~DevPool() { (void)rollback(0); }

  template <typename T> void zeros(T **slot, size_t n) { get((void **)slot, n * sizeof(T), true); }
  bool ok() const { return err == hipSuccess; }
  size_t mark() const { return recs.size(); }
  hipError_t rollback(size_t mark) {
    for (; recs.size() > mark; recs.pop_back()) drop(recs.back());
    return std::exchange(err, hipSuccess);
  }
  template <typename T> hipError_t regrow(T **slot, size_t n, bool zero = false) {
    for (size_t i = 0; i < recs.size(); ++i)
      if (recs[i].slot == (void **)slot) { drop(recs[i]); recs.erase(recs.begin() + i); break; }
    const size_t mk = mark();
    get((void **)slot, n * sizeof(T), zero);
    return ok() ? hipSuccess : rollback(mk);
  }

 private:
  void get(void **slot, size_t bytes, bool zero) {
    if (!ok() || bytes == 0) return;
    void *p = nullptr;
    if ((err = hipMalloc(&p, bytes)) != hipSuccess) { (void)hipGetLastError(); return; }
    recs.push_back({slot, p});
    *slot = p;
    ++bprx_live_allocs;
    if (zero) err = hipMemset(p, 0, bytes);
  }
  void drop(const Rec &r) { (void)hipFree(r.p); *r.slot = nullptr; --bprx_live_allocs; }
};

struct AcfState;
struct AfState;

constexpr int ADAM_HIST = 8192;
constexpr int IX_RMAX = 8192;
constexpr int IX_LPAD = 4;

struct StepPlan {
  int error;
  int64_t B;
  const int32_t *user, *pos, *neg;
  int64_t adam_t;
  float lr_t;
  bool adam_sync_first;
  bool catchup, catchup_aside;
  bool list_mode;
  bool item_mode;
  bool seg_users;
  bool mask;
  bool index_first;
  bool row_count;
  bool idx8;
  int idx_kind;
  bool project, fwd;
  int fast, fastU, fastI;
  bool use_list;
  bool list_reset_cnt;
  bool w_memset, leaves_w_dirty;
  int64_t list_bound;
  int32_t *list_cur, *list_next;
  int seg_cur;
  int ix_R, ix_nown;
  int seg_lead_over;
  int slist_cur;
  int SK_step;
  bool fused_reduce;
  int apply;
  int fk, ek;
  bool dense_launch;
};
enum { PLAN_E_EMPTY = 1 };
enum { APPLY_NONE = 0, APPLY_SGD_LIST, APPLY_SGD, APPLY_ADAM_LAZY, APPLY_ADAM_SWEEP };

struct bprx_handle {
  bprx_config cfg;
  bprx_tables t;
  bool bound;
  bool adam_lazy;
  int32_t *lastU, *lastI;
  float *lr_hist;
  char err[512];

  DevPool mem;
  float *dGu, *dGi, *dBi, *dTu;
  uint32_t *flagU, *flagI;
  float *lossb;
  double *loss_acc;
  int dense_blocks;

  StepPlan step;
  int step_stage;

  int64_t adam_t;
  int64_t adam_synced;
  bool proj_fresh;
  bool et_valid;
  bool p_valid;
  bool absmax_valid;
  int qs_slot;
  bool W_dirty;
  int list_slot;
  int seg_slot;
  int slist_slot;
  const int32_t *idx8_pos, *idx8_neg;
  int64_t idx8_B, idx8_n;

  int32_t *errflag;
  int PS;
  float *P;
  float *W;
  void *Wb;
  float *Ppair;
  void *Ft;
  void *Et;
  void *EtF;
  void *EtS;
  float *dEp;
  float *part;
  int SK;
  float *qs;
  int fast_rows;
  int32_t *cntU, *cntI;
  int seg_policy;
  int32_t *seg_rank;
  int32_t *seg_cnt;
  int32_t *seg_ptr;
  int32_t *seg_cursor;
  void *seg_lead;
  int64_t seg_lead_cap;
  int64_t seg_ent_cap;
  int32_t *uslot_of;
  int32_t *ulist;
  float *uold;
  uint8_t *own8, *loc8;
  int idx8_shift;
  int proj_mask;
  bool idx8_ready(bool item_mode, const int32_t *pos, const int32_t *neg, int64_t B) const {
    return item_mode && own8 && B > 0 && idx8_n == B && idx8_B == B && idx8_pos == pos && idx8_neg == neg && B % 16 == 0;
  }
  int32_t *hot_done;
  void *seg_ent;
  int list_policy;
  int32_t *ilist;
  int32_t *ilist_n;
  int32_t *slist, *slist_n;
  int num_cu;
  int fwd_variant;
  float neg_bias_reg;
  bool factored;
  bprx_factored fx;
  float *gF;
  struct AcfState *acf;
  struct AfState *af;
  int32_t *msg_cursor;
  int32_t *msg_next;
  size_t msg_next_n;
  hipStream_t side;
  hipEvent_t ev_fork, ev_join;
  bool prof;
  struct ProfRec { int phase; hipEvent_t a, b; };
  std::vector<ProfRec> prof_pending;
  std::vector<hipEvent_t> prof_free;
};

struct BprxProfScope {
  bprx_handle *h; hipStream_t s; hipEvent_t a, b; int phase; bool on;
  BprxProfScope(bprx_handle *h_, int phase_, hipStream_t s_) : h(h_), s(s_), phase(phase_), on(h_->prof) {
    if (!on) return;
    auto get = [&]() { hipEvent_t e; if (!h->prof_free.empty()) { e = h->prof_free.back(); h->prof_free.pop_back(); }
                       else (void)hipEventCreate(&e); return e; };
    a = get(); b = get();
    (void)hipEventRecord(a, s);
  }
  ~BprxProfScope() {
    if (!on) return;
    (void)hipEventRecord(b, s);
    h->prof_pending.push_back({phase, a, b});
  }
};

#define BPRX_FAIL(h, code, ...)                                   \
  do {                                                            \
    snprintf((h)->err, sizeof((h)->err), __VA_ARGS__);            \
    return (code);                                                \
  } while (0)

#define BPRX_HIP(h, call)                                                                          \
  do {                                                                                             \
    hipError_t e__ = (call);                                                                       \
    if (e__ != hipSuccess) BPRX_FAIL(h, BPRX_E_HIP, "%s: %s", #call, hipGetErrorString(e__));      \
  } while (0)

#define BPRX_LAUNCH_CHECK(h, name)                                                                 \
  do {                                                                                             \
    hipError_t e__ = hipGetLastError();                                                            \
    if (e__ != hipSuccess) BPRX_FAIL(h, BPRX_E_HIP, "launch %s: %s", name, hipGetErrorString(e__)); \
  } while (0)

int bprx_launch_score(bprx_handle *h, const int32_t *u, const int32_t *i, int64_t B, const float *Prow,
                      int p_by_pair, float *x, hipStream_t s);
int bprx_launch_index_pass(bprx_handle *h, const StepPlan &p, hipStream_t s);
int bprx_launch_triplet_grad(bprx_handle *h, const StepPlan &p, hipStream_t s);
int bprx_launch_item_seg(bprx_handle *h, const StepPlan &p, hipStream_t s);
int bprx_launch_apply(bprx_handle *h, const StepPlan &p, hipStream_t s);
int bprx_launch_dense_update(bprx_handle *h, const StepPlan &p, hipStream_t s);
struct AdamSweepSeg { float *p, *m, *v, *g; size_t n; };
struct AdamSweepAll { AdamSweepSeg seg[4]; uint32_t *flag[2]; size_t nflag[2]; };
int bprx_launch_adam_sweep(bprx_handle *h, const AdamSweepAll &sw, float lr_t, hipStream_t s);
int bprx_launch_fill_i32(bprx_handle *h, int32_t *p, size_t n, int32_t v, hipStream_t s);
int bprx_launch_adam_catchup(bprx_handle *h, const StepPlan &p, hipStream_t s);
int bprx_launch_adam_sync(bprx_handle *h, int64_t t, hipStream_t s);
int bprx_launch_adam_reset(bprx_handle *h, int64_t t, hipStream_t s);
int bprx_launch_loss_reduce(bprx_handle *h, int64_t B, float *loss_out, hipStream_t s);
int bprx_launch_score_block(bprx_handle *h, int32_t u0, int32_t u1, float *out, hipStream_t s);
int bprx_launch_score_gemm(bprx_handle *h, int32_t u0, int32_t u1, float *out, hipStream_t s);
int bprx_launch_tile_F(bprx_handle *h);
int bprx_launch_cast_Et(bprx_handle *h, hipStream_t s);
int bprx_launch_proj_fwd(bprx_handle *h, const int32_t *rows, int64_t nrows, const int32_t *nrows_dev, int scatter, float *Pout,
                         hipStream_t s, const int32_t *occ = nullptr);
int bprx_launch_proj_bwd(bprx_handle *h, const StepPlan &p, hipStream_t s);
int bprx_launch_proj_new(bprx_handle *h, const void *Fnew, int64_t n, float *P, hipStream_t s);
int bprx_new_items_check(bprx_handle *h, const char *what, int64_t n);
bool bprx_proj_fwd_takes_mask(const bprx_handle &h);
bool bprx_proj_bwd_takes_mask(const bprx_handle &h);
int bprx_launch_fact_compose(bprx_handle *h, hipStream_t s);
int bprx_launch_fact_update(bprx_handle *h, float lr_t, hipStream_t s);
int bprx_launch_explain(bprx_handle *h, const int32_t *u, const int32_t *i, int64_t n, float *out, hipStream_t s);
int bprx_acf_step(bprx_handle *h, const int32_t *u, const int32_t *i, const int32_t *j, int64_t B, float *loss_out, hipStream_t s);
int bprx_acf_score_pairs(bprx_handle *h, const int32_t *u, const int32_t *i, int64_t B, float *x, hipStream_t s);
int bprx_acf_eval_profiles(bprx_handle *h, hipStream_t s);
float *bprx_acf_eval_gu(bprx_handle *h);
void bprx_acf_invalidate(bprx_handle *h);
void bprx_acf_free(bprx_handle *h);
int bprx_af_step(bprx_handle *h, const int32_t *u, const int32_t *i, const int32_t *j, int64_t B, float *loss_out, hipStream_t s);
int bprx_af_pairs(bprx_handle *h, const int32_t *u, const int32_t *i, int64_t n, float *x, float *alpha, hipStream_t s);
int bprx_af_block(bprx_handle *h, int32_t u0, int32_t u1, float *out, float *alpha, hipStream_t s);
void bprx_af_invalidate(bprx_handle *h);
void bprx_af_free(bprx_handle *h);

static inline float bprx_adam_lr_at(const bprx_config &c, int64_t it) {
  const float t = (float)it;
  return c.lr * sqrtf(1.0f - powf(c.beta2, t)) / (1.0f - powf(c.beta1, t));
}
static inline float bprx_adam_lr_t(const bprx_handle *h) { return bprx_adam_lr_at(h->cfg, h->adam_t); }
static inline unsigned bprx_blocks(int64_t work, int64_t per_block, int64_t cap = INT32_MAX) {
  int64_t g = (work + per_block - 1) / per_block;
  if (g > cap) g = cap;
  return (unsigned)(g < 1 ? 1 : g);
}

inline StepPlan plan_step(const bprx_handle &h, const int32_t *user, const int32_t *pos, const int32_t *neg, int64_t B,
                          bool fused_reduce = false) {
  StepPlan p = {};
  const bprx_config &c = h.cfg;
  const bool vb = c.model == BPRX_MODEL_VBPR, sgd = c.optimizer == BPRX_OPT_SGD, lazy = !sgd && h.adam_lazy;
  const bool exU = c.flags & BPRX_FLAG_EXPORT_USER_GRAD, exI = c.flags & BPRX_FLAG_EXPORT_ITEM_GRAD;
  const int64_t I = c.num_items;
  const bool bf = c.feat_dtype != BPRX_F_FP32;
  if (B == 0 && !exU && !exI) { p.error = PLAN_E_EMPTY; return p; }
  p.B = B;
  if (B) { p.user = user; p.pos = pos; p.neg = neg; }
  p.adam_t = h.adam_t;
  p.lr_t = c.lr;
  if (!sgd) {
    p.adam_t = h.adam_t + 1;
    p.lr_t = bprx_adam_lr_at(c, p.adam_t);
    p.adam_sync_first = lazy && p.adam_t - h.adam_synced >= ADAM_HIST - 2;
    p.catchup = lazy;
  }
  p.fused_reduce = fused_reduce && !h.factored;
  p.idx_kind = h.step.idx_kind;
  p.seg_cur = h.step.seg_cur; p.seg_lead_over = h.step.seg_lead_over;
  p.slist_cur = h.slist_slot;
  p.SK_step = B ? h.SK : h.step.SK_step;
  p.leaves_w_dirty = h.W_dirty;
  p.dense_launch = vb && (!h.factored || c.feat_dtype == BPRX_F_BF16);
  if (B == 0) return p;

  p.list_mode = vb && !h.proj_fresh && (h.list_policy == 2 || (h.list_policy == 1 && 2 * B < I));
  p.item_mode = !p.list_mode && (h.seg_policy == 2 || (h.seg_policy == 1 && 2 * B >= I));
  p.seg_users = p.item_mode && sgd && !exU;
  p.dense_launch = p.dense_launch || p.list_mode;
  p.fast = p.item_mode ? 0 : h.fast_rows;
  p.fastU = p.fast && !exU;
  p.fastI = p.fast && !exI;
  p.use_list = h.slist && p.fastU && p.fastI;
  p.row_count = !p.item_mode && (h.fast_rows || p.list_mode);
  p.idx8 = h.idx8_ready(p.item_mode, pos, neg, B);
  if (p.list_mode) {
    p.list_bound = 2 * B < I ? 2 * B : I;
    p.list_cur = h.ilist_n + h.list_slot; p.list_next = h.ilist_n + (h.list_slot ^ 1);
    p.list_reset_cnt = !(h.fast_rows && !exI);
    if (bf) { const int sk = (int)((p.list_bound + 127) / 128); p.SK_step = sk < 1 ? 1 : (sk > h.SK ? h.SK : sk); }
  }
  p.catchup_aside = lazy && h.side && !h.proj_fresh && !p.list_mode && !h.p_valid;
  p.project = vb && !h.proj_fresh;
  p.fwd = p.project && !h.p_valid;
  p.mask = p.project && !p.list_mode && p.item_mode && !h.p_valid &&
           (h.proj_mask == 2 ? bf : (h.proj_mask == 1 && c.feat_dtype == BPRX_F_BF16 && h.PS / 16 <= 9));
  p.index_first = p.list_mode || p.mask;
  if (p.item_mode) {
    p.idx_kind = p.idx8 ? 2 : 1;
    int64_t nown = h.num_cu > 0 ? h.num_cu : 256;
    if (nown > 1024) nown = 1024;
    if ((I + nown - 1) / nown > IX_RMAX) nown = (I + IX_RMAX - 1) / IX_RMAX;
    if (nown > I) nown = I;
    p.ix_R = p.idx8 ? 1 << h.idx8_shift : (int)((I + nown - 1) / nown);
    p.ix_nown = (int)((I + p.ix_R - 1) / p.ix_R);
    p.seg_lead_over = p.ix_nown * (p.ix_R + IX_LPAD);
    p.seg_cur = h.seg_slot;
  }
  p.leaves_w_dirty = vb && !p.list_mode && !bf;
  p.w_memset = p.leaves_w_dirty || (vb && h.W_dirty);
  p.ek = (p.item_mode || exI) ? 1 : 3;
  if (sgd) {
    p.fk = (exU || p.item_mode) ? 1 : 0;
    p.apply = p.seg_users ? APPLY_NONE : (p.use_list ? APPLY_SGD_LIST : APPLY_SGD);
  } else {
    p.fk = exU ? 1 : 0;
    p.apply = lazy ? APPLY_ADAM_LAZY : APPLY_ADAM_SWEEP;
  }
  return p;
}
```

fashionvisualexpl_recommend_amd/csrc/bprx_sparse.hip:

```cpp
#include <type_traits>

#include "bprx_internal.h"

namespace {

struct SparseArgs {
  const float *Gu, *Gi, *Bi, *Tu;
  float *dGu, *dGi, *dBi, *dTu;
  uint32_t *flagU, *flagI;
  const float *P;
  float *W;
  float *lossb;
  int32_t *errflag;
  int U, I, k, d, PS;
  float reg;
  float nb;
  int32_t *cntU, *cntI;
  float *wGu, *wGi, *wBi, *wTu;
  int fast;
  int fastU, fastI;
  float lr;
  const int4 *seg_lead;
  const int32_t *seg_nlead;
  int seg_lead_cap, seg_lead_over;
// ... 585 lines not shown
  const int wl = threadIdx.x & 63;
#pragma unroll
  for (int q = 0; q < 64 / G; ++q) {
    const int old_q = __shfl(old, q * G, 64);
    if (old_q >= t - 1) continue;
    const int row_q = __shfl(row, q * G, 64), kind_q = __shfl(kind, q * G, 64);
    adam_replay_kind<64, false>(T, kind_q == 0, row_q, wl, old_q, t - 1, a);
  }
}

template <int G, bool VEC>
__device__ __forceinline__ void adam_apply_row(float *p, float *m, float *v, float *g, int n, int lane, int t, float lr_t,
                                               const AdamLazy &a) {
  if (VEC) {
    for (int c = lane * 4; c < n; c += G * 4) {
      float4 pp = ld4(p + c), mm = ld4(m + c), vv = ld4(v + c);
      const float4 gg = ld4(g + c);
      adam_elem(pp.x, mm.x, vv.x, gg.x, a.b1, a.b2, lr_t, a.eps); adam_elem(pp.y, mm.y, vv.y, gg.y, a.b1, a.b2, lr_t, a.eps);
      adam_elem(pp.z, mm.z, vv.z, gg.z, a.b1, a.b2, lr_t, a.eps); adam_elem(pp.w, mm.w, vv.w, gg.w, a.b1, a.b2, lr_t, a.eps);
      *reinterpret_cast<float4 *>(p + c) = pp; *reinterpret_cast<float4 *>(m + c) = mm; *reinterpret_cast<float4 *>(v + c) = vv;
      *reinterpret_cast<float4 *>(g + c) = make_float4(0.f, 0.f, 0.f, 0.f);
    }
  } else {
    for (int c = lane; c < n; c += G) {
      float pp = p[c], mm = m[c], vv = v[c];
      adam_elem(pp, mm, vv, g[c], a.b1, a.b2, lr_t, a.eps);
      p[c] = pp; m[c] = mm; v[c] = vv;
      g[c] = 0.f;
    }
  }
}

template <int G, bool VEC>
__global__ __launch_bounds__(256) void k_adam_apply_lazy(AdamTables T, AdamLazy a, float *dGu, float *dTu, float *dGi, float *dBi,
                                                         uint32_t *flagU, uint32_t *flagI, const int32_t *__restrict__ user,
                                                         const int32_t *__restrict__ pos, const int32_t *__restrict__ neg,
                                                         int64_t B, int t, float lr_t, int first_kind, int end_kind) {
  const int64_t job = ((int64_t)blockIdx.x * 256 + threadIdx.x) / G + (int64_t)first_kind * B;
  const int lane = threadIdx.x % G;
  if (job >= (int64_t)end_kind * B) return;
  const int kind = (int)(job / B);
  const int64_t b = job - (int64_t)kind * B;
  const int raw = kind == 0 ? user[b] : (kind == 1 ? pos[b] : neg[b]);
  if (kind == 0 && b > 0 && user[b - 1] == raw) return;
  const int row = clamp_quiet(raw, kind == 0 ? T.U : T.I);
  uint32_t *flag = kind == 0 ? flagU + row : flagI + row;
  unsigned claimed = 0;
  if (lane == 0) claimed = atomicExch(flag, 0u);
  claimed = __shfl(claimed, 0, G);
  if (!claimed) return;
  int32_t *last = kind == 0 ? T.lastU + row : T.lastI + row;
  const int from = *last;
  if (from < t - 1) adam_replay_kind<G, VEC>(T, kind == 0, row, lane, from, t - 1, a);
  if (kind == 0) {
    adam_apply_row<G, VEC>(T.Gu + (size_t)row * T.k, T.mGu + (size_t)row * T.k, T.vGu + (size_t)row * T.k, dGu + (size_t)row * T.k, T.k, lane, t, lr_t, a);
    if (T.d) adam_apply_row<G, VEC>(T.Tu + (size_t)row * T.d, T.mTu + (size_t)row * T.d, T.vTu + (size_t)row * T.d, dTu + (size_t)row * T.d, T.d, lane, t, lr_t, a);
  } else {
    adam_apply_row<G, VEC>(T.Gi + (size_t)row * T.k, T.mGi + (size_t)row * T.k, T.vGi + (size_t)row * T.k, dGi + (size_t)row * T.k, T.k, lane, t, lr_t, a);
    if (lane == 0) adam_apply_row<1, false>(T.Bi + row, T.mBi + row, T.vBi + row, dBi + row, 1, 0, t, lr_t, a);
  }
  if (lane == 0) *last = t;
}

template <int G, bool VEC>
__global__ __launch_bounds__(256) void k_adam_sync(AdamTables T, AdamLazy a, int t) {
  const int lane = threadIdx.x % G;
  const int64_t ngroups = (int64_t)gridDim.x * 256 / G;
  for (int64_t r = ((int64_t)blockIdx.x * 256 + threadIdx.x) / G; r < (int64_t)T.U + T.I; r += ngroups) {
    const bool usr = r < T.U;
    const int row = usr ? (int)r : (int)(r - T.U);
    int32_t *last = usr ? T.lastU + row : T.lastI + row;
    const int old = *last;
    if (old >= t) continue;
    adam_replay_kind<G, VEC>(T, usr, row, lane, old, t, a);
    if (lane == 0) *last = t;
  }
}

__global__ void k_fill_i32(int32_t *p, size_t n, int32_t v) {
  for (size_t e = (size_t)blockIdx.x * blockDim.x + threadIdx.x; e < n; e += (size_t)gridDim.x * blockDim.x) p[e] = v;
}

constexpr int DU_KB = 8;
__global__ __launch_bounds__(1024) void k_dense_update(float *__restrict__ E, float *__restrict__ Bp, float *mE, float *vE,
                                                      float *mBp, float *vBp, const float *__restrict__ dEp,
                                                      const float *__restrict__ part, int SK, int D, int d, int PS, int adam,
                                                      float lr_t, float reg, float b1, float b2, float eps,
                                                      double *__restrict__ sqpart, float gscale, uint16_t *__restrict__ Et,
                                                      uint16_t *__restrict__ EtF, const int32_t *__restrict__ ilist,
                                                      const int32_t *__restrict__ ilist_n, int32_t *__restrict__ ilist_n_next,
                                                      int bound, float *__restrict__ W, int32_t *__restrict__ cnt_reset,
                                                      uint32_t *__restrict__ absmax_out, int upd) {
  __shared__ __attribute__((aligned(16))) uint16_t tile[DU_KB][288];
  if (ilist_n_next && blockIdx.x == 0 && threadIdx.x == 0) *ilist_n_next = 0;
  if (ilist) {
    int n = *ilist_n;
    n = n < bound ? n : bound;
    const int per = PS / 4;
    for (int64_t e = (int64_t)blockIdx.x * blockDim.x + threadIdx.x; e < (int64_t)n * per; e += (int64_t)gridDim.x * blockDim.x) {
      const int p = (int)(e / per), c4 = (int)(e % per);
      const int item = ilist[p];
      reinterpret_cast<float4 *>(W + (size_t)item * PS)[c4] = make_float4(0.f, 0.f, 0.f, 0.f);
      if (cnt_reset && c4 == 0) cnt_reset[item] = 0;
    }
  }
  double sq = 0.0;
  uint32_t amax = 0;
  const size_t total = (size_t)D * PS;
  const int ntile = (D + DU_KB - 1) / DU_KB;
  for (int tl = blockIdx.x; tl < ntile; tl += gridDim.x) {
    const int k0 = tl * DU_KB;
    const int PQ = PS >> 2;
    for (int q = threadIdx.x; q < DU_KB * PQ; q += (int)blockDim.x) {
      const int kr = q / PQ, n4 = (q - kr * PQ) * 4, kk = k0 + kr;
      float nvv[4] = {0.f, 0.f, 0.f, 0.f};
      if (!upd && kk < D && n4 <= d) {
#pragma unroll
        for (int c = 0; c < 4; ++c) {
          const int n = n4 + c;
          if (n <= d) nvv[c] = n < d ? E[(size_t)kk * d + n] : Bp[kk];
        }
      } else if (kk < D && n4 <= d) {
        const size_t e = (size_t)kk * PS + n4;
        float gs[4] = {0.f, 0.f, 0.f, 0.f};
        if (part) {
          int sidx = 0;
          for (; sidx + 8 <= SK; sidx += 8) {
            float4 t[8];
#pragma unroll
            for (int x = 0; x < 8; ++x) t[x] = ld4(part + (size_t)(sidx + x) * total + e);
#pragma unroll
            for (int x = 0; x < 8; ++x) { gs[0] += t[x].x; gs[1] += t[x].y; gs[2] += t[x].z; gs[3] += t[x].w; }
          }
          for (; sidx < SK; ++sidx) {
            const float4 t = ld4(part + (size_t)sidx * total + e);
            gs[0] += t.x; gs[1] += t.y; gs[2] += t.z; gs[3] += t.w;
          }
#pragma unroll
          for (int c = 0; c < 4; ++c) gs[c] *= gscale;
        } else {
#pragma unroll
          for (int c = 0; c < 4; ++c) {
            const int n = n4 + c;
            if (n <= d) gs[c] = n < d ? dEp[(size_t)kk * d + n] : dEp[(size_t)D * d + kk];
          }
        }
        float *pp[4], *pm[4], *pv_[4];
        float pv[4], mo[4] = {0.f, 0.f, 0.f, 0.f}, vo[4] = {0.f, 0.f, 0.f, 0.f};
        bool on[4];
#pragma unroll
        for (int c = 0; c < 4; ++c) {
          const int n = n4 + c;
          on[c] = n <= d;
          const int nn = on[c] ? n : d;
          pp[c] = nn < d ? E + (size_t)kk * d + nn : Bp + kk;
          pm[c] = adam ? (nn < d ? mE + (size_t)kk * d + nn : mBp + kk) : nullptr;
          pv_[c] = adam ? (nn < d ? vE + (size_t)kk * d + nn : vBp + kk) : nullptr;
          pv[c] = *pp[c];
        }
        if (adam) {
#pragma unroll
          for (int c = 0; c < 4; ++c) { mo[c] = *pm[c]; vo[c] = *pv_[c]; }
        }
#pragma unroll
        for (int c = 0; c < 4; ++c) {
          if (!on[c]) continue;
          sq += (double)pv[c] * (double)pv[c];
          const float gg = gs[c] + 2.f * reg * pv[c];
          float nv;
          if (adam) {
            nv = dense_adam_elem(pv[c], &mo[c], &vo[c], gg, 1, lr_t, b1, b2, eps);
            *pm[c] = mo[c]; *pv_[c] = vo[c];
          } else {
            nv = dense_adam_elem(pv[c], nullptr, nullptr, gg, 0, lr_t, b1, b2, eps);
          }
          *pp[c] = nv;
          nvv[c] = nv;
          const uint32_t av = __float_as_uint(nv) & 0x7fffffffu;
          amax = av > amax ? av : amax;
        }
      }
      if (Et) {
#pragma unroll
        for (int c = 0; c < 4; ++c) tile[kr][n4 + c] = (uint16_t)bf16_rne(nvv[c]);
      }
    }
    if (Et) {
      __syncthreads();
      for (int n = threadIdx.x; n < PS; n += (int)blockDim.x) {
        uint4 v;
        v.x = (uint32_t)tile[0][n] | ((uint32_t)tile[1][n] << 16);
        v.y = (uint32_t)tile[2][n] | ((uint32_t)tile[3][n] << 16);
        v.z = (uint32_t)tile[4][n] | ((uint32_t)tile[5][n] << 16);
        v.w = (uint32_t)tile[6][n] | ((uint32_t)tile[7][n] << 16);
        const int e = k0 & 127;
        *reinterpret_cast<uint4 *>(Et + ((size_t)(k0 >> 7) * PS + n) * 128 + e) = v;
        *reinterpret_cast<uint4 *>(EtF + (((((size_t)(k0 >> 7) * 4 + (e >> 5)) * (PS >> 4) + (n >> 4)) * 64) +
                                          ((e >> 3) & 3) * 16 + (n & 15)) * 8) = v;
      }
      __syncthreads();
    }
  }
  __shared__ double red[16];
  sq = wave_sum(sq);
  if ((threadIdx.x & 63) == 0) red[threadIdx.x >> 6] = sq;
  __syncthreads();
  if (threadIdx.x == 0 && sqpart) {
    double t = 0.0;
    for (int q = 0; q < (int)(blockDim.x >> 6); ++q) t += red[q];
    sqpart[blockIdx.x] = t;
  }
  if (absmax_out) {
    __shared__ uint32_t wm[16];
#pragma unroll
    for (int o = 32; o > 0; o >>= 1) { const uint32_t v = __shfl_xor(amax, o, 64); amax = v > amax ? v : amax; }
    if ((threadIdx.x & 63) == 0) wm[threadIdx.x >> 6] = amax;
    __syncthreads();
    if (threadIdx.x == 0) {
      uint32_t b = wm[0];
      for (int q = 1; q < (int)(blockDim.x >> 6); ++q) b = wm[q] > b ? wm[q] : b;
      if (b) atomicMax(absmax_out, b);
    }
  }
}

__global__ __launch_bounds__(1024) void k_loss_reduce(const float *__restrict__ lossb, int64_t B,
                                                      const double *__restrict__ sqpart, int nsq, float reg,
                                                      float *__restrict__ out) {
  double s = 0.0;
  for (int64_t b = threadIdx.x; b < B; b += 1024) s += (double)lossb[b];
  for (int q = threadIdx.x; q < nsq; q += 1024) s += (double)reg * sqpart[q];
  s = block_sum_1024(s);
  if (threadIdx.x == 0) *out = (float)s;
}

__global__ __launch_bounds__(256) void k_score_block(SparseArgs a, int u0, int u1, float *__restrict__ out) {
  const int i = blockIdx.x * 64 + (threadIdx.x & 63);
  const int ub = u0 + blockIdx.y * 4 + (threadIdx.x >> 6);
  if (i >= a.I || ub >= u1) return;
  const float *gu = a.Gu + (size_t)ub * a.k, *gi = a.Gi + (size_t)i * a.k;
  float s = 0.f;
  for (int c = 0; c < a.k; ++c) s += gu[c] * gi[c];
  float xv = a.Bi[i] + s;
  if (a.d) {
    const float *tu = a.Tu + (size_t)ub * a.d, *P = a.P + (size_t)i * a.PS;
    float t = 0.f;
    for (int c = 0; c < a.d; ++c) t += tu[c] * P[c];
    xv = xv + t + P[a.d];
  }
  out[(size_t)(ub - u0) * a.I + i] = xv;
}



constexpr int IX_T = 1024;

struct IndexSegArgs {
  const int32_t *user, *pos, *neg;
  int64_t B;
  int U, I, R, nown, nuser;
  int32_t *seg_rank, *seg_cnt, *seg_ptr;
  int Ce, Lc, ent_over, lead_over, lead_cap;
  int32_t *cur, *cur_next;
  int4 *lead;
  int32_t *cntU, *uslot_of, *ulist;
  uint16_t *Wb;
  int PS;
  int aligned;
  const uint8_t *own8, *loc8;
  int wide;
};

__global__ __launch_bounds__(IX_T) void k_index_seg(IndexSegArgs a) {
  const int tid = threadIdx.x, lane = tid & 63, wv = tid >> 6;
  if ((int)blockIdx.x < a.nuser) {
    const int64_t b = (int64_t)blockIdx.x * IX_T + tid;
    const bool valid = b < a.B;
    const int u = valid ? clamp_quiet(a.user[b], a.U) : 0;
    const unsigned long long vm = __ballot(valid);
    const int up = __shfl_up(u, 1, 64);
    const bool uhead = valid && (lane == 0 || up != u);
    const unsigned long long hm = __ballot(uhead);
    const unsigned long long le = lane == 63 ? ~0ull : ((2ull << lane) - 1ull);
    const int hl = (hm & le) ? 63 - __clzll((long long)(hm & le)) : lane;
    const unsigned long long stops = (hm | ~vm) & ~(hl == 63 ? ~0ull : ((2ull << hl) - 1ull));
    const int run_end = stops ? __ffsll((long long)stops) - 1 : 64;
    __shared__ int u_wcnt[IX_T / 64], u_base;
    int old = -1;
    if (valid && lane == hl) old = atomicAdd(a.cntU + u, run_end - hl);
    const bool firstrun = old == 0;
    const unsigned long long fm = __ballot(firstrun);
    if (lane == 0) u_wcnt[wv] = __popcll(fm);
    __syncthreads();
    if (tid == 0) {
      int t = 0;
      for (int q = 0; q < IX_T / 64; ++q) { const int c = u_wcnt[q]; u_wcnt[q] = t; t += c; }
      u_base = t ? atomicAdd(a.cur + 2, t) : 0;
    }
    __syncthreads();
    if (firstrun) {
      a.uslot_of[u] = (int)b;
      a.ulist[u_base + u_wcnt[wv] + __popcll(fm & (lane ? (~0ull >> (64 - lane)) : 0ull))] = u;
    }
    return;
  }
  extern __shared__ __attribute__((aligned(16))) int cnt[];
  __shared__ int wsc[IX_T / 64], wsl[IX_T / 64];
  __shared__ int s_gbase, s_lover, s_ltot;
  const int w = (int)blockIdx.x - a.nuser;
  const int lo = w * a.R;
  const int Rw = a.I - lo < a.R ? a.I - lo : a.R;
  for (int t = tid; t < Rw; t += IX_T) cnt[t] = 0;
  if (w == 0 && tid == 0) { a.cur_next[0] = 0; a.cur_next[1] = 0; a.cur_next[2] = 0; }
  __syncthreads();
  const int I = a.I;
  const int Lb = w == 0 ? (int)0x80000000 : lo, Hb = w == a.nown - 1 ? 0x7fffffff : lo + Rw - 1;
  const unsigned uL = (unsigned)Lb, Wm = (unsigned)Hb - (unsigned)Lb;
  auto one = [&](int v, int64_t occ) {
    if ((unsigned)v - uL <= Wm) a.seg_rank[occ] = atomicAdd(&cnt[clamp_quiet(v, I) - lo], 1);
  };
  auto four = [&](const int4 v, int64_t occ, bool in) {
    const unsigned x0 = (unsigned)v.x - uL, x1 = (unsigned)v.y - uL, x2 = (unsigned)v.z - uL, x3 = (unsigned)v.w - uL;
    const unsigned mn = min(min(x0, x1), min(x2, x3));
    if (in && mn <= Wm) { one(v.x, occ); one(v.y, occ + 1); one(v.z, occ + 2); one(v.w, occ + 3); }
  };
  if (a.own8 && a.wide) {
    const uint4 *o4 = reinterpret_cast<const uint4 *>(a.own8), *l4 = reinterpret_cast<const uint4 *>(a.loc8);
    const int n16 = (int)((2 * a.B) >> 4);
    const int nblk = (n16 + IX_T - 1) / IX_T;
    const int rot = nblk ? (int)((((unsigned)w * 2654435761u) >> 8) % (unsigned)nblk) : 0;
    const unsigned wp = (unsigned)w * 0x01010101u;
    auto dword16 = [&](unsigned o, unsigned la, unsigned lb, int occ) {
      const unsigned y = o ^ wp;
      unsigned m = ~(((y & 0x7f7f7f7fu) + 0x7f7f7f7fu) | y | 0x7f7f7f7fu);
      while (m) {
        const int by = (__ffs((int)m) - 1) >> 3;
        const unsigned l = ((by < 2 ? la : lb) >> (16 * (by & 1))) & 0xffffu;
        a.seg_rank[occ + by] = atomicAdd(&cnt[l < (unsigned)Rw ? l : (unsigned)Rw - 1u], 1);
        m &= m - 1;
      }
    };
    for (int blk = 0; blk < nblk; blk += 4) {
      uint4 vo[4], va[4], vb[4];
#pragma unroll
      for (int x = 0; x < 4; ++x) {
        int bb = blk + x + rot;
        bb = bb >= nblk ? bb - nblk : bb;
        const int e = bb * IX_T + tid;
        const int ec = e < n16 ? e : n16 - 1;
        vo[x] = o4[ec]; va[x] = l4[2 * ec]; vb[x] = l4[2 * ec + 1];
      }
#pragma unroll
      for (int x = 0; x < 4; ++x) {
        int bb = blk + x + rot;
        bb = bb >= nblk ? bb - nblk : bb;
        const int e = bb * IX_T + tid;
        const unsigned y0 = vo[x].x ^ wp, y1 = vo[x].y ^ wp, y2 = vo[x].z ^ wp, y3 = vo[x].w ^ wp;
        const unsigned any = (((y0 - 0x01010101u) & ~y0) | ((y1 - 0x01010101u) & ~y1) | ((y2 - 0x01010101u) & ~y2) |
                              ((y3 - 0x01010101u) & ~y3)) & 0x80808080u;
        if (blk + x < nblk && e < n16 && any) {
          dword16(vo[x].x, va[x].x, va[x].y, 16 * e); dword16(vo[x].y, va[x].z, va[x].w, 16 * e + 4);
          dword16(vo[x].z, vb[x].x, vb[x].y, 16 * e + 8); dword16(vo[x].w, vb[x].z, vb[x].w, 16 * e + 12);
        }
      }
    }
  } else if (a.own8) {
    const uint4 *o4 = reinterpret_cast<const uint4 *>(a.own8), *l4 = reinterpret_cast<const uint4 *>(a.loc8);
    const int n16 = (int)((2 * a.B) >> 4);
    const int nblk = (n16 + IX_T - 1) / IX_T;
    const int rot = nblk ? (int)((((unsigned)w * 2654435761u) >> 8) % (unsigned)nblk) : 0;
    const unsigned wp = (unsigned)w * 0x01010101u;
    auto dword = [&](unsigned o, unsigned l, int occ) {
      const unsigned y = o ^ wp;
      unsigned m = ~(((y & 0x7f7f7f7fu) + 0x7f7f7f7fu) | y | 0x7f7f7f7fu);
      while (m) {
        const int by = (__ffs((int)m) - 1) >> 3;
        a.seg_rank[occ + by] = atomicAdd(&cnt[(l >> (8 * by)) & 255u], 1);
        m &= m - 1;
      }
    };
    for (int blk = 0; blk < nblk; blk += 8) {
      uint4 vo[8], vl[8];
#pragma unroll
      for (int x = 0; x < 8; ++x) {
        int bb = blk + x + rot;
        bb = bb >= nblk ? bb - nblk : bb;
// ... 631 lines not shown
  msg_chain_in_rank_order(next, job, cap, nranks, [&](int rr, int ss) {
    const float *m = msgs + (size_t)rr * stride + hdr;
    const float *ig = m + (size_t)ss * k, *it = m + (size_t)cap * k + (size_t)ss * d;
    if (VEC) {
      for (int c = lane * 4; c < k; c += G * 4) {
        float4 p = ld4(pg + c); const float4 g = ld4(ig + c);
        p.x += scale * g.x; p.y += scale * g.y; p.z += scale * g.z; p.w += scale * g.w;
        *reinterpret_cast<float4 *>(pg + c) = p;
      }
      for (int c = lane * 4; c < d; c += G * 4) {
        float4 p = ld4(pt + c); const float4 g = ld4(it + c);
        p.x += scale * g.x; p.y += scale * g.y; p.z += scale * g.z; p.w += scale * g.w;
        *reinterpret_cast<float4 *>(pt + c) = p;
      }
    } else {
      for (int c = lane; c < k; c += G) pg[c] += scale * ig[c];
      for (int c = lane; c < d; c += G) pt[c] += scale * it[c];
    }
  });
  if (lane == 0) head[u] = 0u;
}

template <int G, bool VEC>
__device__ __forceinline__ void row_accum(float *__restrict__ dst, const float *__restrict__ src, int n, int lane) {
  if (VEC) {
    for (int c = lane * 4; c < n; c += G * 4) {
      float4 p = ld4(dst + c); const float4 g = ld4(src + c);
      p.x += g.x; p.y += g.y; p.z += g.z; p.w += g.w;
      *reinterpret_cast<float4 *>(dst + c) = p;
    }
  } else {
    for (int c = lane; c < n; c += G) dst[c] += src[c];
  }
}

template <int G, bool VEC>
__global__ __launch_bounds__(256) void k_adam_apply_msg_users(AdamTables T, AdamLazy a, const float *__restrict__ msgs, int nranks,
                                                              size_t stride, int cap, float *dGu, float *dTu, uint32_t *head,
                                                              const int32_t *__restrict__ next, int t, float lr_t) {
  const int64_t job = ((int64_t)blockIdx.x * 256 + threadIdx.x) / G;
  const int lane = threadIdx.x % G;
  int r, slot, row;
  if (!msg_job(msgs, nranks, stride, cap, T.U, job, r, slot, row)) return;
  if (head[row] != (uint32_t)(job + 1)) return;
  const size_t hdr = msg_hdr(cap);
  float *gg = dGu + (size_t)row * T.k, *gt = T.d ? dTu + (size_t)row * T.d : nullptr;
  msg_chain_in_rank_order(next, job, cap, nranks, [&](int rr, int ss) {
    const float *m = msgs + (size_t)rr * stride + hdr;
    const float *ig = m + (size_t)ss * T.k, *it = m + (size_t)cap * T.k + (size_t)ss * T.d;
    row_accum<G, VEC>(gg, ig, T.k, lane);
    if (T.d) row_accum<G, VEC>(gt, it, T.d, lane);
  });
  const int from = T.lastU[row];
  if (from < t - 1) adam_replay_kind<G, VEC>(T, true, row, lane, from, t - 1, a);
  adam_apply_row<G, VEC>(T.Gu + (size_t)row * T.k, T.mGu + (size_t)row * T.k, T.vGu + (size_t)row * T.k, gg, T.k, lane, t, lr_t, a);
  if (T.d) adam_apply_row<G, VEC>(T.Tu + (size_t)row * T.d, T.mTu + (size_t)row * T.d, T.vTu + (size_t)row * T.d, gt, T.d, lane, t, lr_t, a);
  if (lane == 0) { T.lastU[row] = t; head[row] = 0u; }
}

__global__ __launch_bounds__(256) void k_sum_dense_msgs(const float *__restrict__ msgs, int nranks, size_t stride, size_t off,
                                                        size_t n, float *__restrict__ dEp) {
  for (size_t e = (size_t)blockIdx.x * 256 + threadIdx.x; e < n; e += (size_t)gridDim.x * 256) {
    float s = 0.f;
    for (int r = 0; r < nranks; ++r) s += msgs[(size_t)r * stride + off + e];
    dEp[e] = s;
  }
}

}

static inline size_t msg_rows_end(const bprx_handle *h, int64_t cap) {
  return msg_hdr(cap) + (size_t)cap * (size_t)(h->cfg.embed_k + h->cfg.embed_d);
}

extern "C" int64_t bprx_user_msg_floats(const bprx_handle *h, int64_t cap) {
  if (!h || cap <= 0) return -1;
  const int64_t d = h->cfg.embed_d, D = h->cfg.feat_dim;
  const int64_t n = (int64_t)msg_rows_end(h, cap) + ((h->cfg.flags & BPRX_FLAG_DENSE_ALLREDUCE) ? 0 : D * d + D);
  return (n + 3) & ~(int64_t)3;
}

extern "C" int bprx_pack_user_msg(bprx_handle *h, const int32_t *user, int64_t B, int64_t cap, float *msg, void *stream) {
  if (!h || !msg || B < 0 || cap <= 0 || (B > 0 && !user)) return BPRX_E_INVALID;
  if (!(h->cfg.flags & BPRX_FLAG_EXPORT_USER_GRAD)) BPRX_FAIL(h, BPRX_E_STATE, "pack_user_msg needs BPRX_FLAG_EXPORT_USER_GRAD");
  if (!h->step_stage) BPRX_FAIL(h, BPRX_E_STATE, "pack_user_msg outside a step (after bprx_step_begin[_sparse])");
  if (B != h->step.B) BPRX_FAIL(h, BPRX_E_INVALID, "pack_user_msg: B differs from the pending step's");
  hipStream_t s = (hipStream_t)stream;
  const int k = h->cfg.embed_k, d = h->cfg.embed_d;
  const dim3 grid((unsigned)((B + 255) / 256));
  if (B == 0) BPRX_HIP(h, hipMemsetAsync(msg, 0, 4 * sizeof(float), s));
  else if (vec_ok(h) && ((uintptr_t)msg & 15) == 0)
    hipLaunchKernelGGL(k_pack_user_msg<true>, grid, dim3(256), 0, s, user, B, h->cfg.num_users, k, d, (int)cap, h->flagU, h->dGu,
                       h->dTu, msg, h->msg_cursor, h->errflag);
  else
    hipLaunchKernelGGL(k_pack_user_msg<false>, grid, dim3(256), 0, s, user, B, h->cfg.num_users, k, d, (int)cap, h->flagU, h->dGu,
                       h->dTu, msg, h->msg_cursor, h->errflag);
  BPRX_LAUNCH_CHECK(h, "k_pack_user_msg");
  const size_t nd = (h->cfg.flags & BPRX_FLAG_DENSE_ALLREDUCE) ? 0 : (size_t)h->cfg.feat_dim * (d + 1);
  if (nd) {
    if (h->step_stage < 2) BPRX_FAIL(h, BPRX_E_STATE, "the message carries dE|dBp: pack it after bprx_step_begin[_dense]");
    BPRX_HIP(h, hipMemcpyAsync(msg + msg_rows_end(h, cap), h->dEp, nd * sizeof(float), hipMemcpyDeviceToDevice, s));
  }
  return BPRX_OK;
}

extern "C" int bprx_apply_user_msgs(bprx_handle *h, const float *msgs, int32_t nranks, int64_t cap, float scale, void *stream) {
  if (!h || !msgs || nranks <= 0 || cap <= 0) return BPRX_E_INVALID;
  if (!h->bound) BPRX_FAIL(h, BPRX_E_STATE, "tables not bound");
  if (!(h->cfg.flags & BPRX_FLAG_EXPORT_USER_GRAD)) BPRX_FAIL(h, BPRX_E_STATE, "apply_user_msgs needs BPRX_FLAG_EXPORT_USER_GRAD");
  if ((int64_t)nranks * cap >= ((int64_t)1 << 31) - 1) BPRX_FAIL(h, BPRX_E_INVALID, "nranks * cap too large");
  hipStream_t s = (hipStream_t)stream;
  const int k = h->cfg.embed_k, d = h->cfg.embed_d;
  const size_t stride = (size_t)bprx_user_msg_floats(h, cap);
  const size_t jobs = (size_t)nranks * (size_t)cap;
  if (h->msg_next_n < jobs) {
    BPRX_HIP(h, hipStreamSynchronize(s));
    h->msg_next_n = 0;
    if (h->mem.regrow(&h->msg_next, jobs) != hipSuccess) BPRX_FAIL(h, BPRX_E_NOMEM, "apply_user_msgs: chain links (%zu entries)", jobs);
    h->msg_next_n = jobs;
  }
  const bool vec = vec_ok(h) && ((uintptr_t)msgs & 15) == 0;
  hipLaunchKernelGGL(k_msg_link, dim3((unsigned)((jobs + 255) / 256)), dim3(256), 0, s, msgs, (int)nranks, stride, (int)cap,
                     h->cfg.num_users, h->flagU, h->msg_next);
  if (h->cfg.optimizer == BPRX_OPT_ADAM_TF23) {
    const float lr_t = bprx_adam_lr_t(h);
    const int G = pick_group(k, d, vec);
    const AdamTables T = make_adam_tables(h);
    const AdamLazy al = {h->cfg.beta1, h->cfg.beta2, h->cfg.epsilon, h->lr_hist};
    DISPATCH_G(G, vec, k_adam_apply_msg_users, grid_for((int64_t)jobs, G), s, T, al, msgs, (int)nranks, stride, (int)cap,
               h->dGu, h->dTu, h->flagU, h->msg_next, (int)h->adam_t, lr_t);
  } else if (vec) {
    hipLaunchKernelGGL(k_apply_user_msgs<true>, grid_for((int64_t)jobs, 16), dim3(256), 0, s, msgs, (int)nranks, stride, (int)cap,
                       h->cfg.num_users, k, d, h->t.Gu, h->t.Tu, scale, h->flagU, h->msg_next);
  } else {
    hipLaunchKernelGGL(k_apply_user_msgs<false>, grid_for((int64_t)jobs, 16), dim3(256), 0, s, msgs, (int)nranks, stride, (int)cap,
                       h->cfg.num_users, k, d, h->t.Gu, h->t.Tu, scale, h->flagU, h->msg_next);
  }
  const size_t nd = (h->cfg.flags & BPRX_FLAG_DENSE_ALLREDUCE) ? 0 : (size_t)h->cfg.feat_dim * (d + 1);
  if (nd) {
    unsigned blocks = (unsigned)((nd + 255) / 256);
    if (blocks > 2048) blocks = 2048;
    hipLaunchKernelGGL(k_sum_dense_msgs, dim3(blocks), dim3(256), 0, s, msgs, nranks, stride, msg_rows_end(h, cap), nd, h->dEp);
  }
  BPRX_LAUNCH_CHECK(h, "k_apply_user_msgs");
  return BPRX_OK;
}

extern "C" int bprx_sum_dense_parts(bprx_handle *h, const float *parts, int32_t nranks, void *stream) {
  if (!h || !parts || nranks <= 0) return BPRX_E_INVALID;
  if (h->cfg.model != BPRX_MODEL_VBPR) BPRX_FAIL(h, BPRX_E_STATE, "sum_dense_parts: VBPR only");
  const size_t nd = (size_t)h->cfg.feat_dim * (h->cfg.embed_d + 1);
  unsigned blocks = (unsigned)((nd + 255) / 256);
  if (blocks > 2048) blocks = 2048;
  hipLaunchKernelGGL(k_sum_dense_msgs, dim3(blocks), dim3(256), 0, (hipStream_t)stream, parts, nranks, nd, (size_t)0, nd, h->dEp);
  BPRX_LAUNCH_CHECK(h, "k_sum_dense_msgs");
  return BPRX_OK;
}

int bprx_launch_score(bprx_handle *h, const int32_t *u, const int32_t *i, int64_t B, const float *Prow, int p_by_pair,
                      float *x, hipStream_t s) {
  SparseArgs a = make_args(h, h->cfg.embed_d ? (p_by_pair ? Prow : h->P) : nullptr, h->step);
  const bool vec = vec_ok(h);
  const int G = pick_group(a.k, a.d, vec);
  DISPATCH_G(G, vec, k_score, grid_for(B, G), s, a, u, i, B, p_by_pair, x);
  BPRX_LAUNCH_CHECK(h, "k_score");
  return BPRX_OK;
}

int bprx_launch_index_pass(bprx_handle *h, const StepPlan &p, hipStream_t s) {
  SparseArgs a = make_args(h, h->P, p);
  const int32_t *u = p.user, *i = p.pos, *j = p.neg;
  const int64_t B = p.B;
  if (p.item_mode) {
    BprxProfScope pc(h, BPRX_PHASE_ROW_COUNT, s);
    IndexSegArgs x;
    x.user = u; x.pos = i; x.neg = j; x.B = B; x.U = a.U; x.I = a.I;
    x.R = p.ix_R; x.nown = p.ix_nown;
    x.own8 = x.loc8 = nullptr; x.wide = 0;
    if (p.idx8) { x.own8 = h->own8; x.loc8 = h->loc8; x.wide = h->idx8_shift > 8; }
    x.seg_rank = h->seg_rank; x.seg_cnt = h->seg_cnt; x.seg_ptr = h->seg_ptr;
    x.Ce = (int)(2 * ((2 * B + x.nown - 1) / x.nown) + 64);
    x.Lc = x.R + IX_LPAD;
    x.ent_over = x.nown * x.Ce; x.lead_over = p.seg_lead_over; x.lead_cap = (int)h->seg_lead_cap;
    if ((int64_t)x.ent_over + 2 * B > h->seg_ent_cap || (int64_t)x.lead_over + 2 * B / SEG_CAP + 64 > h->seg_lead_cap)
      BPRX_FAIL(h, BPRX_E_STATE, "index pass: segment buffers too small (I=%d, B=%lld)", a.I, (long long)B);
    x.cur = h->seg_cursor + 3 * p.seg_cur; x.cur_next = h->seg_cursor + 3 * (p.seg_cur ^ 1);
    x.lead = (int4 *)h->seg_lead;
    const bool users = p.seg_users;
    x.cntU = users ? h->cntU : nullptr; x.uslot_of = users ? h->uslot_of : nullptr; x.ulist = users ? h->ulist : nullptr;
    const bool zw = a.d && h->cfg.feat_dtype != BPRX_F_FP32;
    x.Wb = zw ? (uint16_t *)h->Wb : nullptr; x.PS = a.PS;
    x.aligned = (((uintptr_t)i | (uintptr_t)j) & 15) == 0;
    x.nuser = users ? (int)((B + IX_T - 1) / IX_T) : 0;
    hipLaunchKernelGGL(k_index_seg, dim3((unsigned)(x.nown + x.nuser)), dim3(IX_T), (size_t)x.R * sizeof(int), s, x);
    BPRX_LAUNCH_CHECK(h, "k_index_seg");
    return BPRX_OK;
  }
  if (p.row_count) {
    BprxProfScope pc(h, BPRX_PHASE_ROW_COUNT, s);
    const int64_t cap = 2 * B < (int64_t)a.I ? 2 * B : (int64_t)a.I;
    hipLaunchKernelGGL(k_row_count, dim3((unsigned)((B + 255) / 256)), dim3(256), 0, s, u, i, j, B, a.U, a.I, h->cntU, h->cntI,
                       a.fastU, (a.fastI || p.list_mode) ? 1 : 0,
                       p.list_mode ? h->ilist : (int32_t *)nullptr, p.list_cur, (int)cap,
                       a.use_list ? a.slist : (int32_t *)nullptr, a.slist_n, (int)(3 * h->cfg.max_batch));
  }
  BPRX_LAUNCH_CHECK(h, "k_row_count");
  return BPRX_OK;
}

int bprx_launch_triplet_grad(bprx_handle *h, const StepPlan &p, hipStream_t s) {
  SparseArgs a = make_args(h, h->P, p);
  const int32_t *u = p.user, *i = p.pos, *j = p.neg;
  const int64_t B = p.B;
  const bool vec = vec_ok(h);
  const int G = pick_group(a.k, a.d, vec);
  BprxProfScope ps(h, BPRX_PHASE_TRIPLET, s);
  if (p.w_memset) BPRX_HIP(h, hipMemsetAsync(h->W, 0, (size_t)a.I * a.PS * sizeof(float), s));
  if (p.item_mode) {
    const SegUser su = {p.seg_users ? 0 : 1, h->uslot_of, h->uold};
    const int Gs = pick_group(a.k, a.d, true);
    const dim3 grid((unsigned)((B * Gs + TS_T - 1) / TS_T));
    with_group(Gs, [&](auto g_) { hipLaunchKernelGGL((k_triplet_seg<decltype(g_)::value>), grid, dim3(TS_T), 0, s, a, su, u, i, j, B); });
  } else {
    with_group(G, [&](auto g_) {
      constexpr int GG = decltype(g_)::value, T = TripletGradThreads<GG>::value;
      const dim3 grid((unsigned)((B * GG + T - 1) / T));
      if (vec) hipLaunchKernelGGL((k_triplet_grad<GG, true>), grid, dim3(T), 0, s, a, u, i, j, B);
      else hipLaunchKernelGGL((k_triplet_grad<GG, false>), grid, dim3(T), 0, s, a, u, i, j, B);
    });
  }
  BPRX_LAUNCH_CHECK(h, "k_triplet_grad");
  return BPRX_OK;
}

int bprx_launch_item_seg(bprx_handle *h, const StepPlan &p, hipStream_t s) {
  SparseArgs a = make_args(h, nullptr, p);
  const int64_t B = p.B;
  const float lr_t = p.lr_t;
  const int G = pick_group(a.k, a.d, true);
  const int adam = h->cfg.optimizer == BPRX_OPT_ADAM_TF23 ? (h->adam_lazy ? 2 : 1) : 0;
  const bool bf = h->cfg.feat_dtype != BPRX_F_FP32;
  float *Wf = a.d && !bf ? h->W : nullptr;
  uint16_t *Wb = a.d && bf ? (uint16_t *)h->Wb : nullptr;
  const AdamFuse af = {h->t.m_Gi, h->t.v_Gi, h->t.m_Bi, h->t.v_Bi, h->lastI, h->cfg.beta1, h->cfg.beta2, h->cfg.epsilon, (int)p.adam_t};
  BprxProfScope ps(h, BPRX_PHASE_ITEM_SEG, s);
  const int64_t bound = (int64_t)p.seg_lead_over + 2 * B / SEG_CAP + 64;
  int64_t nfin = B * G / IS_T / 4;
  nfin = nfin < 16 ? 16 : (nfin > 2048 ? 2048 : nfin);
  a.nfin = p.seg_users ? (int)nfin : 0;
  const dim3 grid((unsigned)((bound * G + IS_T - 1) / IS_T + a.nfin));
  with_group(G, [&](auto g_) {
    constexpr int GG = decltype(g_)::value;
    if (adam == 2) hipLaunchKernelGGL((k_item_seg<GG, 2>), grid, dim3(IS_T), 0, s, a, h->t.Gi, h->t.Bi, Wf, Wb, lr_t, af);
    else if (adam) hipLaunchKernelGGL((k_item_seg<GG, 1>), grid, dim3(IS_T), 0, s, a, h->t.Gi, h->t.Bi, Wf, Wb, lr_t, af);
    else hipLaunchKernelGGL((k_item_seg<GG, 0>), grid, dim3(IS_T), 0, s, a, h->t.Gi, h->t.Bi, Wf, Wb, lr_t, af);
  });
  BPRX_LAUNCH_CHECK(h, "k_item_seg");
  return BPRX_OK;
}

int bprx_launch_apply(bprx_handle *h, const StepPlan &p, hipStream_t s) {
  SparseArgs a = make_args(h, nullptr, p);
  const size_t U = a.U, I = a.I, k = a.k, d = a.d;
  const int32_t *u = p.user, *i = p.pos, *j = p.neg;
  const int64_t B = p.B;
  const float lr_t = p.lr_t;
  const bool vec = vec_ok(h);
  const int G = pick_group(a.k, a.d, vec);
  BprxProfScope ps(h, BPRX_PHASE_APPLY, s);
  if (p.apply == APPLY_SGD_LIST) {
    int64_t blocks = (3 * B * G + 255) / 256;
    if (blocks > 1024) blocks = 1024;
    DISPATCH_G(G, vec, k_apply_sgd_list, dim3((unsigned)blocks), s, h->t.Gu, h->t.Gi, h->t.Bi, h->t.Tu, a, h->slist,
               h->slist_n + p.slist_cur, h->slist_n + (p.slist_cur ^ 1), (int)(3 * h->cfg.max_batch), lr_t);
    BPRX_LAUNCH_CHECK(h, "k_apply_sgd_list");
    return BPRX_OK;
  }
  if (p.apply == APPLY_SGD) {
    if (p.ek > p.fk)
      DISPATCH_G(G, vec, k_apply_sgd, grid_for((int64_t)(p.ek - p.fk) * B, G), s, h->t.Gu, h->t.Gi, h->t.Bi, h->t.Tu, a, u, i, j, B,
                 lr_t, p.fk, p.ek);
    BPRX_LAUNCH_CHECK(h, "k_apply_sgd");
    return BPRX_OK;
  }
  if (p.apply == APPLY_ADAM_LAZY) {
    const AdamTables T = make_adam_tables(h);
    const AdamLazy al = {h->cfg.beta1, h->cfg.beta2, h->cfg.epsilon, h->lr_hist};
    if (p.ek > p.fk)
      DISPATCH_G(G, vec, k_adam_apply_lazy, grid_for((int64_t)(p.ek - p.fk) * B, G), s, T, al, h->dGu, h->dTu, h->dGi, h->dBi, h->flagU,
                 h->flagI, u, i, j, B, (int)p.adam_t, lr_t, p.fk, p.ek);
    BPRX_LAUNCH_CHECK(h, "k_adam_apply_lazy");
    return BPRX_OK;
  }
  AdamSweepAll sw;
  sw.seg[0] = {h->t.Bi, h->t.m_Bi, h->t.v_Bi, h->dBi, I};
  sw.seg[1] = {h->t.Gu, h->t.m_Gu, h->t.v_Gu, h->dGu, U * k};
  sw.seg[2] = {h->t.Gi, h->t.m_Gi, h->t.v_Gi, h->dGi, I * k};
  sw.seg[3] = {h->t.Tu, h->t.m_Tu, h->t.v_Tu, h->dTu, d ? U * d : (size_t)0};
  sw.flag[0] = h->flagU; sw.nflag[0] = U; sw.flag[1] = h->flagI; sw.nflag[1] = I;
  return bprx_launch_adam_sweep(h, sw, lr_t, s);
}

int bprx_launch_adam_sweep(bprx_handle *h, const AdamSweepAll &sw, float lr_t, hipStream_t s) {
  const hipError_t e = adam_sweep(sw, h->cfg.beta1, h->cfg.beta2, lr_t, h->cfg.epsilon, s);
  if (e != hipSuccess) BPRX_FAIL(h, BPRX_E_HIP, "launch k_adam_sweep: %s", hipGetErrorString(e));
  return BPRX_OK;
}

int bprx_launch_fill_i32(bprx_handle *h, int32_t *p, size_t n, int32_t v, hipStream_t s) {
  hipLaunchKernelGGL(k_fill_i32, dim3(512), dim3(256), 0, s, p, n, v);
  BPRX_LAUNCH_CHECK(h, "k_fill_i32");
  return BPRX_OK;
}

int bprx_launch_adam_catchup(bprx_handle *h, const StepPlan &p, hipStream_t s) {
  const bool vec = vec_ok(h);
  const int G = pick_group(h->cfg.embed_k, h->cfg.embed_d, vec);
  const AdamTables T = make_adam_tables(h);
  const AdamLazy al = {h->cfg.beta1, h->cfg.beta2, h->cfg.epsilon, h->lr_hist};
  BprxProfScope ps(h, BPRX_PHASE_ADAM_CATCHUP, s);
  DISPATCH_G(G, vec, k_adam_catchup, grid_for(p.B ? 3 * p.B : 1, G), s, T, al, p.user, p.pos, p.neg, p.B, (int)p.adam_t, p.lr_t,
             h->lr_hist);
  BPRX_LAUNCH_CHECK(h, "k_adam_catchup");
  return BPRX_OK;
}

int bprx_launch_adam_sync(bprx_handle *h, int64_t t, hipStream_t s) {
  if (!h->adam_lazy || h->adam_synced >= t) return BPRX_OK;
  const bool vec = vec_ok(h);
  const int G = pick_group(h->cfg.embed_k, h->cfg.embed_d, vec);
  const AdamTables T = make_adam_tables(h);
  const AdamLazy al = {h->cfg.beta1, h->cfg.beta2, h->cfg.epsilon, h->lr_hist};
  const int64_t rows = (int64_t)T.U + T.I;
  int64_t blocks = (rows * G + 255) / 256;
  if (blocks > 8192) blocks = 8192;
  DISPATCH_G(G, vec, k_adam_sync, dim3((unsigned)blocks), s, T, al, (int)t);
  BPRX_LAUNCH_CHECK(h, "k_adam_sync");
  h->adam_synced = t;
  return BPRX_OK;
}

int bprx_launch_adam_reset(bprx_handle *h, int64_t t, hipStream_t s) {
  if (!h->adam_lazy) return BPRX_OK;
  int rc;
  if ((rc = bprx_launch_fill_i32(h, h->lastU, (size_t)h->cfg.num_users, (int32_t)t, s))) return rc;
  if ((rc = bprx_launch_fill_i32(h, h->lastI, (size_t)h->cfg.num_items, (int32_t)t, s))) return rc;
  if (s == nullptr) BPRX_HIP(h, hipStreamSynchronize(nullptr));
  h->adam_synced = t;
  return BPRX_OK;
}

int bprx_launch_dense_update(bprx_handle *h, const StepPlan &p, hipStream_t s) {
  const int D = h->cfg.feat_dim;
  unsigned blocks = (unsigned)((D + DU_KB - 1) / DU_KB);
  if (blocks > BPRX_DENSE_BLOCKS) blocks = BPRX_DENSE_BLOCKS;
  const bool upd = !h->factored;
  if (upd) h->dense_blocks = (int)blocks;
  BprxProfScope ps(h, BPRX_PHASE_DENSE, s);
  const float *part = (p.fused_reduce && h->cfg.feat_dtype != BPRX_F_FP32) ? h->part : nullptr;
  const float gscale = (part && h->cfg.feat_dtype == BPRX_F_FP8) ? 1.0f / h->cfg.feat_scale : 1.0f;
  const bool images = h->cfg.feat_dtype == BPRX_F_BF16;
  const bool lm = p.list_mode;
  int threads = (DU_KB * (h->PS / 4) + 63) / 64 * 64;
  threads = threads < 256 ? 256 : (threads > 1024 ? 1024 : threads);
  hipLaunchKernelGGL(k_dense_update, dim3(blocks), dim3((unsigned)threads), 0, s, h->t.E, h->t.Bp, h->t.m_E, h->t.v_E, h->t.m_Bp,
                     h->t.v_Bp, h->dEp, part, p.SK_step, D, h->cfg.embed_d, h->PS,
                     h->cfg.optimizer == BPRX_OPT_ADAM_TF23 ? 1 : 0, p.lr_t, h->cfg.reg, h->cfg.beta1, h->cfg.beta2,
                     h->cfg.epsilon, upd ? h->loss_acc : (double *)nullptr, gscale, images ? (uint16_t *)h->Et : (uint16_t *)nullptr, (uint16_t *)h->EtF,
                     lm ? (const int32_t *)h->ilist : (const int32_t *)nullptr, (const int32_t *)p.list_cur,
                     p.list_next, (int)p.list_bound, h->W,
                     (lm && p.list_reset_cnt) ? h->cntI : (int32_t *)nullptr,
                     h->cfg.feat_dtype == BPRX_F_FP8 ? (uint32_t *)h->qs + 2 + h->qs_slot : (uint32_t *)nullptr, upd ? 1 : 0);
  BPRX_LAUNCH_CHECK(h, "k_dense_update");
  return BPRX_OK;
}

int bprx_launch_loss_reduce(bprx_handle *h, int64_t B, float *loss_out, hipStream_t s) {
  BprxProfScope ps(h, BPRX_PHASE_LOSS, s);
  hipLaunchKernelGGL(k_loss_reduce, dim3(1), dim3(1024), 0, s, h->lossb, B, h->loss_acc,
                     h->cfg.model == BPRX_MODEL_VBPR ? h->dense_blocks : 0, h->cfg.reg, loss_out);
  BPRX_LAUNCH_CHECK(h, "k_loss_reduce");
  return BPRX_OK;
}

int bprx_launch_score_block(bprx_handle *h, int32_t u0, int32_t u1, float *out, hipStream_t s) {
  SparseArgs a = make_args(h, h->P, h->step);
  dim3 grid((a.I + 63) / 64, (u1 - u0 + 3) / 4);
  hipLaunchKernelGGL(k_score_block, grid, dim3(256), 0, s, a, u0, u1, out);
  BPRX_LAUNCH_CHECK(h, "k_score_block");
  return BPRX_OK;
}
```

fashionvisualexpl_recommend_amd/engine.py:

```python
import ctypes as C

import numpy as np
import torch

from . import _ffi

PARAM_NAMES = ("Gu", "Gi", "Bi", "Tu", "E", "Bp")
FACTORED_PARAM_NAMES = ("Gu", "Gi", "Bi", "Tu", "Ec", "Ee", "E", "Bp")


def _ptr(t):
    return None if (t is None or t.numel() == 0) else C.c_void_p(t.data_ptr())


def _stream():
    return C.c_void_p(torch.cuda.current_stream().cuda_stream)


def as_index(x, device):
    if isinstance(x, torch.Tensor):
        t = x.reshape(-1)
        if t.dtype != torch.int32:
            t = t.to(torch.int32)
        return t.to(device, non_blocking=True).contiguous()
    return torch.as_tensor(np.ascontiguousarray(np.asarray(x).reshape(-1), dtype=np.int32), device=device)


class Engine:
    def __init__(self, model, num_users, num_items, embed_k, embed_d=0, feat_dim=0, feat_dtype="fp32",
                 optimizer="adam_tf23", lr=1e-3, reg=0.0, max_batch=256, device=None,
                 beta1=0.9, beta2=0.999, epsilon=1e-7, export_user_grad=False, export_item_grad=False, feat_scale=448.0,
                 dense_allreduce=False, adam_form=None):
        if not torch.cuda.is_available():
            raise RuntimeError("fashionvisualexpl_recommend_amd needs a ROCm GPU (MI355X); there is no CPU fallback")
        self.lib = _ffi.lib()
        self.device = torch.device("cuda", torch.cuda.current_device() if device is None else device)
        self.model, self.optimizer = model, optimizer
        self.U, self.I, self.k = int(num_users), int(num_items), int(embed_k)
        self.d, self.D = (int(embed_d), int(feat_dim)) if model == "vbpr" else (0, 0)
        self.feat_dtype = feat_dtype
        self.feat_scale = float(feat_scale)
        self.max_batch = int(max_batch)
        cfg = _ffi.Config(_ffi.ABI_VERSION, _ffi.MODEL[model], self.U, self.I, self.k, self.d, self.D,
                          _ffi.FEAT_DTYPE[feat_dtype], _ffi.OPTIMIZER[optimizer], self.device.index, self.max_batch,
                          lr, reg, beta1, beta2, epsilon,
                          (_ffi.FLAG_EXPORT_USER_GRAD if export_user_grad else 0) |
                          (_ffi.FLAG_EXPORT_ITEM_GRAD if export_item_grad else 0) |
                          (_ffi.FLAG_DENSE_ALLREDUCE if dense_allreduce else 0) |
                          {None: 0, "sweep": _ffi.FLAG_ADAM_SWEEP, "lazy": _ffi.FLAG_ADAM_LAZY}[adam_form], self.feat_scale)
        h = C.c_void_p()
        _ffi.check(None, self.lib.bprx_create(C.byref(cfg), C.byref(h)))
        self.h = h
        self._t = {}
        self._loss = torch.zeros(1, dtype=torch.float32, device=self.device)

    @property
    def t(self):
        if self.optimizer == "adam_tf23" and getattr(self, "h", None) and self._t:
            self.sync_adam()
        return self._t

    @t.setter
    def t(self, v):
        self._t = v

    def adam_is_lazy(self):
        return bool(self.lib.bprx_adam_is_lazy(self.h))

    def sync_adam(self):
        _ffi.check(self.h, self.lib.bprx_sync_adam(self.h, _stream()))

    def close(self):
        if getattr(self, "h", None):
            self.lib.bprx_destroy(self.h)
            self.h = None

    def __del__(self):
        try:
            self.close()
        except Exception:
            pass

    def bind(self, Gu, Gi, Bi, Tu=None, F=None, E=None, Bp=None, slots=None):
        def prep(x, shape, dtype=torch.float32):
            if x is None:
                return None
            x = torch.as_tensor(x)
            x = x.to(device=self.device, dtype=dtype).reshape(shape).contiguous()
            return x
        t = {"Gu": prep(Gu, (self.U, self.k)), "Gi": prep(Gi, (self.I, self.k)), "Bi": prep(Bi, (self.I,))}
        if self.model == "vbpr":
            if self.feat_dtype == "fp8":
                Ft = torch.as_tensor(F)
                if Ft.dtype != torch.float8_e4m3fn:
                    Ft = (Ft.to(device=self.device, dtype=torch.float32) * self.feat_scale).to(torch.float8_e4m3fn)
                Fp = Ft.to(self.device).reshape(self.I, self.D).contiguous()
            else:
                Fp = prep(F, (self.I, self.D), torch.bfloat16 if self.feat_dtype == "bf16" else torch.float32)
            t.update(Tu=prep(Tu, (self.U, self.d)), F=Fp, E=prep(E, (self.D, self.d)), Bp=prep(Bp, (self.D,)))
        if self.optimizer == "adam_tf23":
            for n in PARAM_NAMES:
                if t.get(n) is None:
                    continue
                for s in ("m_", "v_"):
                    given = None if slots is None else slots.get(s + n)
                    t[s + n] = torch.zeros_like(t[n]) if given is None else prep(given, tuple(t[n].shape))
        tb = _ffi.Tables()
        for n in _ffi.TABLE_FIELDS:
            setattr(tb, n, None if t.get(n) is None else t[n].data_ptr())
        torch.cuda.current_stream(self.device).synchronize()
        _ffi.check(self.h, self.lib.bprx_bind_tables(self.h, C.byref(tb)))
        self.t = t
        return self

    def bind_factored(self, Gu, Gi, Bi, Tu, F, Ec, Ee, E, Bp, feat_dim_a, feat_dim_b, neg_bias_reg=1.0, slots=None):
        if self.model != "vbpr":
            raise ValueError("bind_factored needs an Engine(model='vbpr', ...)")
        def prep(x, shape, dtype=torch.float32):
            return torch.as_tensor(x).to(device=self.device, dtype=dtype).reshape(shape).contiguous()
        Ec, Ee = torch.as_tensor(Ec), torch.as_tensor(Ee)
        ea, eb = int(Ec.shape[1]), int(Ee.shape[1])
        t = {"Gu": prep(Gu, (self.U, self.k)), "Gi": prep(Gi, (self.I, self.k)), "Bi": prep(Bi, (self.I,)),
             "Tu": prep(Tu, (self.U, self.d)),
             "F": prep(F, (self.I, self.D), torch.bfloat16 if self.feat_dtype == "bf16" else torch.float32),
             "Ec": prep(Ec, (feat_dim_a, ea)), "Ee": prep(Ee, (feat_dim_b, eb)),
             "E": prep(E, (ea + eb, self.d)), "Bp": prep(Bp, (ea + eb,)),
             "E_eff": torch.zeros((self.D, self.d), dtype=torch.float32, device=self.device),
             "Bp_eff": torch.zeros(self.D, dtype=torch.float32, device=self.device)}
        if self.optimizer == "adam_tf23":
            for n in FACTORED_PARAM_NAMES:
                for s_ in ("m_", "v_"):
                    given = None if slots is None else slots.get(s_ + n)
                    t[s_ + n] = torch.zeros_like(t[n]) if given is None else prep(given, tuple(t[n].shape))
        tb = _ffi.Tables()
        for n in _ffi.TABLE_FIELDS:
            v = {"E": t["E_eff"], "Bp": t["Bp_eff"]}.get(n) if n in ("E", "Bp", "m_E", "v_E", "m_Bp", "v_Bp") else t.get(n)
            setattr(tb, n, None if v is None else v.data_ptr())
        fx = _ffi.Factored(int(feat_dim_a), int(feat_dim_b), ea, eb, float(neg_bias_reg))
        for n, name in zip(_ffi.FACTORED_FIELDS, ("Ec", "Ee", "E", "Bp", "m_Ec", "v_Ec", "m_Ee", "v_Ee", "m_E", "v_E", "m_Bp", "v_Bp")):
            setattr(fx, n, None if t.get(name) is None else t[name].data_ptr())
        torch.cuda.current_stream(self.device).synchronize()
        _ffi.check(self.h, self.lib.bprx_bind_factored(self.h, C.byref(tb), C.byref(fx)))
        self.factored = True
        self.t = t
        return self

    def csr(self, lists):
        lens = np.fromiter((len(l) for l in lists), dtype=np.int64, count=len(lists))
        ptr = np.zeros(len(lists) + 1, np.int64)
        np.cumsum(lens, out=ptr[1:])
        items = np.fromiter((int(i) for l in lists for i in l), dtype=np.int64, count=int(ptr[-1])).astype(np.int32)
        return (torch.as_tensor(ptr, device=self.device), torch.as_tensor(items, device=self.device))

# ... 582 lines not shown
```

fashionvisualexpl_recommend_amd/models.py:

```python
import os
import pickle
from time import time

import numpy as np
import torch

from . import configs
from .engine import Engine, as_index
from .evaluator import Evaluator
from .synth import glorot_uniform


class _Scores:

    def __init__(self, t):
        self.tensor = t

    def numpy(self):
        return self.tensor.cpu().numpy()


class RecommenderModel:
    def __init__(self, data, params):
        self.data = data
# ... 41 lines not shown
        elems = kw["num_users"] * (kw["embed_k"] + kw.get("embed_d", 0)) + kw["num_items"] * (kw["embed_k"] + 1)
        return "lazy" if chain_us < elems * 24.0 / 4e6 else "sweep"

    def _build(self, init):
        t, _ = self._init_tables(init)
        self.engine = Engine(optimizer=self.optimizer_name, lr=self.learning_rate, reg=self.reg,
                             max_batch=max(self.batch_size, 4096), adam_form=self._adam_form(), **self._engine_kwargs())
        self.engine.bind(**t)
        self._alias()

    def _alias(self):
        """The reference's attribute surface (model.Gu, .Gi, .Bi, .Tu, .F, .E, .Bp) is served by the class properties below:
        they go through engine.t, which first brings every row up to date when adam_tf23 runs lazily (bprx_sync_adam) -- a
        raw alias of the tensor would show rows that have not been replayed yet."""

    def call(self, inputs, training=None, mask=None):
        user, item = inputs
        u, i = as_index(user, self.engine.device).long(), as_index(item, self.engine.device).long()
        xui = self.engine.score_pairs(u, i)
        return xui, self.Bi[i], self.Gu[u], self.Gi[i]

    __call__ = call

    def predict_block(self, u0, u1):
        return self.engine.score_block(u0, u1).cpu().numpy()

    def predict_all(self):
        return _Scores(self.engine.score_block(0, self.num_users))

    def train_step(self, batch):
        user, pos, neg = (as_index(b, self.engine.device) for b in batch)
        return float(self.engine.step(user, pos, neg).item())

    def state_dict(self):
        sd = {n: v.detach().clone() for n, v in self.engine.t.items() if n != "F"}
        sd["adam_step"] = self.engine.adam_step
        return sd

    def load_state_dict(self, sd):
        for n, v in sd.items():
            if n == "adam_step":
                self.engine.adam_step = v
            else:
                self.engine.t[n].copy_(v)
        self.engine.tables_dirty()

    def weights_path(self, epoch):
        rec = getattr(self.params, "rec", self.model_kind)
        return os.path.join(configs.weight_dir(), self.params.dataset, rec, f'weights-{epoch}-{self.directory_parameters}.pt')

    def train(self, resume=False):
        max_metrics = {'hr': 0, 'p': 0, 'r': 0, 'auc': 0, 'ndcg': 0}
        best_state = None
        best_epoch = self.restore_epochs
        best_epoch_print = 'No best epoch found!'
        results = {}
        steps_total = (sum(len(pos) for pos in self.data.training_list) // self.params.batch_size) * self.params.epochs
        if getattr(self.params, "sampler", "ref_stream") == "philox":
            from .engine import EpochWalkSampler
            smp = EpochWalkSampler(self.data.training_list, self.num_items, device=self.engine.device,
                                   seed=getattr(self.params, "init_seed", 0)).feeds(self.engine)
            next_batch = (smp.sample(self.params.batch_size) for _ in range(steps_total))
        else:
            next_batch = self.data.next_triple_batch(self.engine.device)
        steps = 0
        loss = 0
        it = 1
        steps_per_epoch = sum([len(pos) for pos in self.data.training_list]) // self.params.batch_size
        rec = getattr(self.params, "rec", self.model_kind)
        wdir = os.path.join(configs.weight_dir(), self.params.dataset, rec)
        rdir = os.path.join(configs.results_dir(), self.params.dataset, rec)
        os.makedirs(wdir, exist_ok=True)
        os.makedirs(rdir, exist_ok=True)
        if resume:
            path = self.weights_path(self.restore_epochs)
            self.load_state_dict(torch.load(path, map_location=self.engine.device, weights_only=True))
            for _ in range(self.restore_epochs * steps_per_epoch):
                next(next_batch)
            it = self.restore_epochs + 1
            print('Restored epoch {0} from {1}'.format(self.restore_epochs, path))
        start_ep = time()
        print('Start training...')
        loss_buf = torch.zeros(max(1, steps_per_epoch), dtype=torch.float32, device=self.engine.device)
        for batch in next_batch:
            steps += 1
            user, pos, neg = (as_index(b, self.engine.device) for b in batch)
            self.engine.step(user, pos, neg, loss_out=loss_buf, loss_index=steps - 1)
            if steps == steps_per_epoch:
                loss = float(loss_buf[:steps].double().sum().item())
                epoch_text = 'Epoch {0}/{1} \tLoss: {2:.3f}'.format(it, self.params.epochs, loss / steps)
                epoch_print = self.evaluator.eval(it, results, epoch_text, start_ep)
                for metric in max_metrics.keys():
                    if max_metrics[metric] <= results[it][metric + '_v']:
                        max_metrics[metric] = results[it][metric + '_v']
                        if metric == self.params.best_metric:
                            best_epoch, best_state, best_epoch_print = it, self.state_dict(), epoch_print
                if (it % self.verbose == 0 or it == 1) and self.verbose != -1:
                    torch.save(self.state_dict(), os.path.join(wdir, f'weights-{it}-{self.directory_parameters}.pt'))
                start_ep = time()
                it += 1
                loss = 0
                steps = 0
        print('Training end...')
        self._store_recs(os.path.join(rdir, f'recs-{it - 1}-{self.directory_parameters}.tsv'))
        with open(os.path.join(rdir, f'results-metrics-{self.directory_parameters}') + '.pkl', 'wb') as f:
            pickle.dump(results, f)
        print("Store Best Model at Epoch {0}".format(best_epoch))
        print(best_epoch_print)
        last_state = self.state_dict()
        if best_state is not None:
            torch.save(best_state, os.path.join(wdir, f'best-weights-{best_epoch}-{self.directory_parameters}.pt'))
            self.load_state_dict(best_state)
        self._store_recs(os.path.join(rdir, f'best-recs-{best_epoch}-{self.directory_parameters}.tsv'))
        self.load_state_dict(last_state)
        print('End Store Best Model!')
        print('Best Values for Each Metric:\nHR\tPrec\tRec\tAUC\tnDCG\n{}\t{}\t{}\t{}\t{}\n'.format(
            max_metrics['hr'], max_metrics['p'], max_metrics['r'], max_metrics['auc'], max_metrics['ndcg']))
        self.results = results
        return results

    def _store_recs(self, path):
        self.evaluator.store_recommendation(path=path)


def _table_property(name):
    return property(lambda self: self.engine.t[name], doc="bound tensor %s (current: lazy adam_tf23 rows are replayed first)" % name)


for _n in ("Gu", "Gi", "Bi", "Tu", "F", "E", "Bp"):
    setattr(BPRMF, _n, _table_property(_n))


class VBPR(BPRMF):
    model_kind = "vbpr"

    def __init__(self, data, params, init=None, features=None):
        self.embed_d = params.embed_d
        self._features = features
        self.feat_explain = int(getattr(params, "feat_explain", 0) or 0)
        if not 0 <= self.feat_explain <= 32:
            raise ValueError("%s: feat_explain is 0 (off) .. 32 (got %r)" % (type(self).__name__, self.feat_explain))
        super().__init__(data, params, init)
        self.directory_parameters = f'batch_{params.batch_size}-D_{params.embed_d}-K_{params.embed_k}' \
                                    f'-lr_{params.lr}-reg_{params.reg}'

    def process_cnn_visual_features(self):
        f = self._features
        if f is None:
            f = np.load(configs.cnn_features_path(self.params.dataset, getattr(self.params, "cnn_model", "vgg19"),
                                                  getattr(self.params, "output_layer", "fc2")))
        f = np.asarray(f)
        self.feat_norm = np.max(np.abs(f))
        self.cnn_features = f / self.feat_norm
        self.dim_cnn_features = self.cnn_features.shape[1]

    def _init_tables(self, init):
        t, rs = super()._init_tables(init)
        self.process_cnn_visual_features()
        D, d = self.dim_cnn_features, self.embed_d
        v = {"Bp": glorot_uniform(rs, D, 1).reshape(-1),
             "Tu": glorot_uniform(rs, self.num_users, d),
             "F": self.cnn_features.astype(np.float32),
             "E": glorot_uniform(rs, D, d)}
        v.update({k: val for k, val in init.items() if k in v})
        t.update(v)
        return t, rs

    def _engine_kwargs(self):
        return dict(model="vbpr", num_users=self.num_users, num_items=self.num_items, embed_k=self.embed_k,
                    embed_d=self.embed_d, feat_dim=self.dim_cnn_features,
                    feat_dtype=getattr(self.params, "dtype", "fp32"))

    def call(self, inputs, training=None, mask=None):
        user, item = inputs
        u, i = as_index(user, self.engine.device).long(), as_index(item, self.engine.device).long()
        xui = self.engine.score_pairs(u, i)
        return xui, self.Gu[u], self.Gi[i], self.F[i], self.Tu[u], self.Bi[i]

    __call__ = call

    @property
    def feat_cols(self):
        return self.dim_cnn_features

    def explain(self, users, items, top=5, maps=False):
# ... 524 lines not shown
```

include/bprx.h:

```cpp
#ifndef BPRX_H_
#define BPRX_H_

#include <stdint.h>

#ifdef __cplusplus
extern "C" {
#endif

#define BPRX_ABI_VERSION 6

#if defined(__GNUC__)
#define BPRX_API __attribute__((visibility("default")))
#else
#define BPRX_API
#endif

enum { BPRX_MODEL_BPRMF = 0, BPRX_MODEL_VBPR = 1 };
enum { BPRX_OPT_SGD = 0, BPRX_OPT_ADAM_TF23 = 1 };
enum { BPRX_F_FP32 = 0, BPRX_F_BF16 = 1, BPRX_F_FP8 = 2 };

enum {
  BPRX_OK = 0,
  BPRX_E_INVALID = -1,
  BPRX_E_STATE = -2,
  BPRX_E_HIP = -3,
  BPRX_E_RANGE = -4,
  BPRX_E_NOMEM = -5
};

typedef struct bprx_handle bprx_handle;
typedef struct bprx_sampler bprx_sampler;

typedef struct {
  int32_t abi_version;
  int32_t model;
  int32_t num_users;
  int32_t num_items;
  int32_t embed_k;
  int32_t embed_d;
  int32_t feat_dim;
  int32_t feat_dtype;
  int32_t optimizer;
  int32_t device;
  int64_t max_batch;
  float lr;
  float reg;
  float beta1, beta2, epsilon;
  int32_t flags;
  float feat_scale;
} bprx_config;

enum { BPRX_FLAG_EXPORT_USER_GRAD = 1, BPRX_FLAG_EXPORT_ITEM_GRAD = 2, BPRX_FLAG_DENSE_ALLREDUCE = 4,
       BPRX_FLAG_ADAM_SWEEP = 8, BPRX_FLAG_ADAM_LAZY = 16 };

typedef struct {
  float *Gu;
  float *Gi;
  float *Bi;
  float *Tu;
  const void *F;
  float *E;
  float *Bp;
  float *m_Gu, *v_Gu, *m_Gi, *v_Gi, *m_Bi, *v_Bi, *m_Tu, *v_Tu, *m_E, *v_E, *m_Bp, *v_Bp;
} bprx_tables;

BPRX_API int bprx_abi_version(void);

BPRX_API int bprx_create(const bprx_config *cfg, bprx_handle **out);
BPRX_API int bprx_destroy(bprx_handle *h);
BPRX_API const char *bprx_last_error(const bprx_handle *h);
BPRX_API int64_t bprx_live_device_allocs(void);

BPRX_API int bprx_bind_tables(bprx_handle *h, const bprx_tables *t);
BPRX_API int bprx_tables_dirty(bprx_handle *h, void *stream);
BPRX_API int bprx_set_hyper(bprx_handle *h, float lr, float reg);
BPRX_API int bprx_set_adam_step(bprx_handle *h, int64_t iterations, void *stream);
BPRX_API int bprx_sync_adam(bprx_handle *h, void *stream);
BPRX_API int64_t bprx_get_adam_step(const bprx_handle *h);
BPRX_API int bprx_adam_is_lazy(const bprx_handle *h);

typedef struct {
  int32_t feat_dim_a, feat_dim_b;
  int32_t embed_a, embed_b;
  float neg_bias_reg;
  float *Ea, *Eb, *A, *Ap;
  float *m_Ea, *v_Ea, *m_Eb, *v_Eb, *m_A, *v_A, *m_Ap, *v_Ap;
} bprx_factored;
BPRX_API int bprx_bind_factored(bprx_handle *h, const bprx_tables *t, const bprx_factored *f);
BPRX_API int bprx_explain_pairs(bprx_handle *h, const int32_t *user, const int32_t *item, int64_t n, float *out, void *stream);

BPRX_API int bprx_feat_explain(bprx_handle *h, const void *F, const int32_t *user, const int32_t *item, int64_t n, int32_t ncols,
                               int32_t top, float *score, float *base, float *visual, int32_t *col, float *contrib, float *map,
                               void *stream);

BPRX_API int32_t bprx_proj_stride(const bprx_handle *h);
BPRX_API int bprx_project_rows(bprx_handle *h, const void *Fnew, int64_t n, float *P, void *stream);
BPRX_API int bprx_score_new_block(bprx_handle *h, int32_t u0, int32_t u1, const float *P, int64_t n, float *out, void *stream);
BPRX_API int bprx_topk_rows(bprx_handle *h, int64_t nrows, int32_t width, float *scores, int32_t K, int32_t *idx, float *val,
                            int32_t *flag, void *stream);
BPRX_API int bprx_feat_explain_new(bprx_handle *h, const void *Fnew, int64_t n_new, const int32_t *user, const int32_t *row,
                                   int64_t n, int32_t ncols, int32_t top, float *score, int32_t *col, float *contrib, float *map,
                                   void *stream);

enum {
  BPRX_ACF_C_WU = 0, BPRX_ACF_C_WI = 1, BPRX_ACF_C_B0 = 2, BPRX_ACF_C_W1 = 3, BPRX_ACF_C_B1 = 4,
  BPRX_ACF_I_WU = 5, BPRX_ACF_I_WV = 6, BPRX_ACF_I_WP = 7, BPRX_ACF_I_WX = 8, BPRX_ACF_I_B0 = 9,
  BPRX_ACF_I_W1 = 10, BPRX_ACF_I_B1 = 11, BPRX_ACF_NW = 12
};
typedef struct {
  int32_t feat_m, feat_c;
  int32_t width_c, width_i;
  int32_t feat_dtype;
  const void *F;
  const int64_t *train_ptr;
  const int32_t *train_items;
  const int64_t *eval_ptr;
  const int32_t *eval_items;
  float *Pi, *m_Pi, *v_Pi;
  float *w[BPRX_ACF_NW];
  float *m_w[BPRX_ACF_NW], *v_w[BPRX_ACF_NW];
} bprx_acf;
BPRX_API int bprx_bind_acf(bprx_handle *h, const bprx_tables *t, const bprx_acf *a);
BPRX_API int bprx_acf_profiles(bprx_handle *h, const int32_t *users, int64_t n, const int64_t *hist_ptr,
                               const int32_t *hist_items, float *out, void *stream);
BPRX_API int bprx_acf_explain(bprx_handle *h, const int32_t *user, const int32_t *item, int64_t n, const int64_t *hist_ptr,
                              const int32_t *hist_items, int32_t top, float *score, float *base, int32_t *pos,
                              int32_t *hist_item, float *alpha, float *contrib, int32_t *peak, float *beta_peak, float *beta,
                              void *stream);
enum { BPRX_ACF_GRAD_DETACHED = 0, BPRX_ACF_GRAD_FULL = 1 };
BPRX_API int bprx_acf_set_gradient(bprx_handle *h, int mode);
BPRX_API int bprx_acf_get_gradient(bprx_handle *h);

enum {
  BPRX_AF_COL_W1 = 0, BPRX_AF_COL_B1 = 1, BPRX_AF_COL_W2 = 2,
  BPRX_AF_EDG_CW = 3, BPRX_AF_EDG_CB = 4, BPRX_AF_EDG_W2 = 5,
  BPRX_AF_CLS_W1 = 6, BPRX_AF_CLS_B1 = 7, BPRX_AF_CLS_W2 = 8,
  BPRX_AF_ATT_W1 = 9, BPRX_AF_ATT_B1 = 10, BPRX_AF_ATT_W2 = 11, BPRX_AF_ATT_B2 = 12,
  BPRX_AF_NW = 13
};
#define BPRX_AF_IMG 224
#define BPRX_AF_HID 256
#define BPRX_AF_CH 64
typedef struct {
  int32_t dim_color, dim_class;
  int32_t width;
  float dropout;
  uint64_t seed;
  const uint8_t *edges;
  const float *color;
  const float *cls;
  float *w[BPRX_AF_NW];
  float *m_w[BPRX_AF_NW], *v_w[BPRX_AF_NW];
} bprx_attentive;
BPRX_API int bprx_bind_attentive(bprx_handle *h, const bprx_tables *t, const bprx_attentive *a);
BPRX_API int bprx_af_encode(bprx_handle *h, const int32_t *items, int64_t n, float *out, void *stream);
BPRX_API int bprx_af_attention_pairs(bprx_handle *h, const int32_t *user, const int32_t *item, int64_t n, float *x, float *alpha,
                                     void *stream);
BPRX_API int bprx_af_explain(bprx_handle *h, const int32_t *user, const int32_t *item, int64_t n, int32_t grid, float *x,
                             float *alpha, float *parts, float *map, int32_t *peak_cell, float *peak_val, void *stream);
BPRX_API int bprx_af_score_block(bprx_handle *h, int32_t u0, int32_t u1, float *scores, float *alpha, void *stream);
// ... 115 lines not shown
```

Baseline: 314.1 million.

## Defer VBPR dense update into next step and settle lazily before table reads

The fused step no longer launches the dense projection update and loss reduction at step end. It records their arguments as pending work and emits them at the start of the next step, where they can be carried or fused with the sparse half (carry_dense). Every API entry that reads tables first settles any pending work, and the training loop enables loss lag and settles at each epoch boundary. The aim is to remove a launch and a serialization point per step, at the cost of added state-machine complexity and the risk of stale reads if some path misses a settle.

```diff
diff --git a/fashionvisualexpl_recommend_amd/_ffi.py b/fashionvisualexpl_recommend_amd/_ffi.py
--- a/fashionvisualexpl_recommend_amd/_ffi.py
+++ b/fashionvisualexpl_recommend_amd/_ffi.py
@@ -70,6 +70,8 @@
 class Tables(C.Structure):
     _fields_ = [(n, C.c_void_p) for n in TABLE_FIELDS]
 
+
+DEFER_ENTRIES = ("bprx_settle", "bprx_dense_pending", "bprx_set_loss_lag")
 
 _lib = None
 
@@ -169,8 +171,13 @@
         "bprx_sampler_destroy": (C.c_int, [vp]),
         "bprx_sampler_count": (i64, [vp, i32, i32]),
         "bprx_sampler_ref_stream": (i64, [vp, i32, i32, u32, u32, vp, vp, vp, i64]),
+        "bprx_settle": (C.c_int, [vp, vp]),
+        "bprx_dense_pending": (C.c_int, [vp]),
+        "bprx_set_loss_lag": (C.c_int, [vp, C.c_int]),
     }
     for name, (res, args) in sig.items():
+        if name in DEFER_ENTRIES and not hasattr(L, name):
+            continue
         fn = getattr(L, name)
         fn.restype, fn.argtypes = res, args
     if L.bprx_abi_version() != ABI_VERSION:
@@ -189,7 +196,7 @@
            "bprx_route_scatter_add", "bprx_score_block", "bprx_eval_users", "bprx_eval_pos", "bprx_eval_counts", "bprx_eval_finish", "bprx_topk", "bprx_sync_check", "bprx_probe_stream_read", "bprx_probe_stream_read_nt", "bprx_probe_row_gather", "bprx_profile_enable",
            "bprx_profile_read", "bprx_sample_philox", "bprx_epoch_prepare", "bprx_epoch_slots", "bprx_sample_epoch", "bprx_sample_philox_h", "bprx_sample_epoch_h", "bprx_index_pass_kind", "bprx_proj_mask_kind", "bprx_adam_rows", "bprx_step_lr", "bprx_user_msg_floats", "bprx_pack_user_msg",
            "bprx_apply_user_msgs", "bprx_sampler_create",
-           "bprx_sampler_destroy", "bprx_sampler_count", "bprx_sampler_ref_stream"]
+           "bprx_sampler_destroy", "bprx_sampler_count", "bprx_sampler_ref_stream", "bprx_settle", "bprx_dense_pending", "bprx_set_loss_lag"]
 
 
 def check(handle, rc):
diff --git a/fashionvisualexpl_recommend_amd/csrc/bprx_api.hip b/fashionvisualexpl_recommend_amd/csrc/bprx_api.hip
--- a/fashionvisualexpl_recommend_amd/csrc/bprx_api.hip
+++ b/fashionvisualexpl_recommend_amd/csrc/bprx_api.hip
@@ -102,6 +102,7 @@
     if (h->SK < 1) h->SK = 1;
     h->fwd_variant = env_int("BPRX_FWD_VARIANT", 4);
     h->proj_mask = std::min(std::max(env_int("BPRX_PROJ_MASK", 1), 0), 2);
+    h->dense_defer = env_int("BPRX_DENSE_DEFER", 1) != 0;
     A.zeros(&h->dTu, U * d);
     A.zeros(&h->P, I * PS);
     A.zeros(&h->W, I * PS);
@@ -165,6 +166,7 @@
 extern "C" int bprx_destroy(bprx_handle *h) {
   if (!h) return BPRX_OK;
   (void)hipSetDevice(h->cfg.device);
+  h->pend.on = false;
   if (h->side) (void)hipStreamSynchronize(h->side);
   (void)h->mem.rollback(0);
   bprx_acf_free(h);
@@ -212,6 +214,7 @@
   }
   if (((uintptr_t)t->Gu | (uintptr_t)t->Gi | (uintptr_t)t->Tu | (uintptr_t)t->F | (uintptr_t)t->E) & 15)
     BPRX_FAIL(h, BPRX_E_INVALID, "bind_tables: table base pointers must be 16-byte aligned");
+  { const int rc = bprx_settle_pending(h, nullptr); if (rc) return rc; }
   h->t = *t;
   h->factored = factored;
   if (!factored) h->neg_bias_reg = 0.1f;
@@ -270,6 +273,7 @@
 extern "C" int bprx_explain_pairs(bprx_handle *h, const int32_t *user, const int32_t *item, int64_t n, float *out, void *stream) {
   int rc = check_ready(h, 0);
   if (rc) return rc;
+  if ((rc = bprx_settle_pending(h, (hipStream_t)stream))) return rc;
   if (!h->factored) BPRX_FAIL(h, BPRX_E_STATE, "explain_pairs: the handle is not bound with bprx_bind_factored");
   if (n < 0 || n > ((int64_t)1 << 32)) BPRX_FAIL(h, BPRX_E_INVALID, "explain_pairs: n = %lld out of range", (long long)n);
   if (n == 0) return BPRX_OK;
@@ -281,6 +285,7 @@
 
 extern "C" int bprx_tables_dirty(bprx_handle *h, void *stream) {
   if (!h) return BPRX_E_INVALID;
+  { const int rc = bprx_settle_pending(h, (hipStream_t)stream); if (rc) return rc; }
   h->et_valid = h->p_valid = h->absmax_valid = false;
   if (h->acf) bprx_acf_invalidate(h);
   if (h->af) bprx_af_invalidate(h);
@@ -300,6 +305,7 @@
 
 extern "C" int bprx_set_adam_step(bprx_handle *h, int64_t it, void *stream) {
   if (!h || it < 0) return BPRX_E_INVALID;
+  { const int rc = bprx_settle_pending(h, (hipStream_t)stream); if (rc) return rc; }
   h->adam_t = it;
   return h->bound ? bprx_launch_adam_reset(h, it, (hipStream_t)stream) : BPRX_OK;
 }
@@ -314,9 +320,32 @@
   return BPRX_OK;
 }
 
+int bprx_settle_pending(bprx_handle *h, hipStream_t s) {
+  if (!h || !h->pend.on) return BPRX_OK;
+  const DensePending q = h->pend;
+  h->pend.on = false;
+  int rc = bprx_launch_dense_args(h, q.a, s);
+  if (!rc && q.loss_out) rc = bprx_launch_loss_reduce_at(h, q.loss_B, q.loss_nsq, q.loss_reg, q.loss_out, s);
+  return rc;
+}
+
+extern "C" int bprx_settle(bprx_handle *h, void *stream) {
+  if (!h) return BPRX_E_INVALID;
+  return bprx_settle_pending(h, (hipStream_t)stream);
+}
+
+extern "C" int bprx_dense_pending(const bprx_handle *h) { return h ? (h->pend.on ? 1 : 0) : BPRX_E_INVALID; }
+
+extern "C" int bprx_set_loss_lag(bprx_handle *h, int on) {
+  if (!h) return BPRX_E_INVALID;
+  h->loss_lag = on != 0;
+  return BPRX_OK;
+}
+
 extern "C" int bprx_sync_adam(bprx_handle *h, void *stream) {
   int rc = check_ready(h, 0);
   if (rc) return rc;
+  if ((rc = bprx_settle_pending(h, (hipStream_t)stream))) return rc;
   return bprx_launch_adam_sync(h, h->adam_t, (hipStream_t)stream);
 }
 
@@ -326,6 +355,7 @@
   if (B == 0) return BPRX_OK;
   if (!user || !item || !x) BPRX_FAIL(h, BPRX_E_INVALID, "score_pairs: null pointer");
   hipStream_t s = (hipStream_t)stream;
+  if ((rc = bprx_settle_pending(h, s))) return rc;
   if (h->acf) return bprx_acf_score_pairs(h, user, item, B, x, s);
   if (h->af) return bprx_af_pairs(h, user, item, B, x, nullptr, s);
   if ((rc = bprx_launch_adam_sync(h, h->adam_t, s))) return rc;
@@ -361,6 +391,11 @@
   } else if (p.catchup && (rc = bprx_launch_adam_catchup(h, p, s))) return rc;
   if (p.project && p.list_mode && (rc = bprx_launch_cast_Et(h, s))) return rc;
   if (p.index_first && (rc = bprx_launch_index_pass(h, p, s))) return rc;
+  if (p.carry_dense) {
+    const DensePending q = h->pend;
+    h->pend.on = false;
+    if (q.loss_out && (rc = bprx_launch_loss_reduce_at(h, q.loss_B, q.loss_nsq, q.loss_reg, q.loss_out, s))) return rc;
+  }
   if (p.project && !p.list_mode && (rc = bprx_launch_cast_Et(h, s))) return rc;
   if (p.fwd) {
     rc = p.list_mode ? bprx_launch_proj_fwd(h, h->ilist, p.list_bound, p.list_cur, 1, h->P, s)
@@ -383,6 +418,7 @@
   if (B && (!user || !pos || !neg)) BPRX_FAIL(h, BPRX_E_INVALID, "step: null index pointer");
   const StepPlan plan = plan_step(*h, user, pos, neg, B, fused_reduce);
   if (plan.error == PLAN_E_EMPTY) BPRX_FAIL(h, BPRX_E_INVALID, "step: empty batch");
+  if (plan.settle_first && (rc = bprx_settle_pending(h, s))) return rc;
   commit_plan(h, plan);
   rc = launch_sparse_half(h, h->step, s);
   if (rc) h->step_stage = 0;
@@ -390,7 +426,8 @@
 }
 
 extern "C" int bprx_step_begin_sparse(bprx_handle *h, const int32_t *user, const int32_t *pos, const int32_t *neg, int64_t B, void *stream) {
-  return step_begin_sparse(h, user, pos, neg, B, false, (hipStream_t)stream);
+  const int rc = bprx_settle_pending(h, (hipStream_t)stream);
+  return rc ? rc : step_begin_sparse(h, user, pos, neg, B, false, (hipStream_t)stream);
 }
 
 extern "C" int bprx_step_begin_dense(bprx_handle *h, void *stream) {
@@ -419,7 +456,8 @@
 }
 
 extern "C" int bprx_step_begin(bprx_handle *h, const int32_t *user, const int32_t *pos, const int32_t *neg, int64_t B, void *stream) {
-  return step_begin(h, user, pos, neg, B, false, stream);
+  const int rc = bprx_settle_pending(h, (hipStream_t)stream);
+  return rc ? rc : step_begin(h, user, pos, neg, B, false, stream);
 }
 
 extern "C" int bprx_step_project(bprx_handle *h, void *stream) {
@@ -427,6 +465,7 @@
   if (rc) return rc;
   if (h->cfg.model != BPRX_MODEL_VBPR) return BPRX_OK;
   hipStream_t s = (hipStream_t)stream;
+  if ((rc = bprx_settle_pending(h, s))) return rc;
   if ((rc = bprx_launch_cast_Et(h, s))) return rc;
   if (!h->p_valid && (rc = bprx_launch_proj_fwd(h, nullptr, h->cfg.num_items, nullptr, 0, h->P, s))) return rc;
   h->p_valid = true;
@@ -444,6 +483,7 @@
 extern "C" int bprx_clear_user_grad(bprx_handle *h, int64_t n_rows, int32_t marks_only, void *stream) {
   if (!h || n_rows < 0 || n_rows > h->cfg.num_users) return BPRX_E_INVALID;
   hipStream_t s = (hipStream_t)stream;
+  { const int rc = bprx_settle_pending(h, s); if (rc) return rc; }
   if (!marks_only) {
     BPRX_HIP(h, hipMemsetAsync(h->dGu, 0, (size_t)n_rows * h->cfg.embed_k * sizeof(float), s));
     if (h->cfg.embed_d) BPRX_HIP(h, hipMemsetAsync(h->dTu, 0, (size_t)n_rows * h->cfg.embed_d * sizeof(float), s));
@@ -462,6 +502,7 @@
 extern "C" int bprx_clear_item_grad(bprx_handle *h, int64_t n_rows, int32_t marks_only, void *stream) {
   if (!h || n_rows < 0 || n_rows > h->cfg.num_items) return BPRX_E_INVALID;
   hipStream_t s = (hipStream_t)stream;
+  { const int rc = bprx_settle_pending(h, s); if (rc) return rc; }
   if (!marks_only) {
     BPRX_HIP(h, hipMemsetAsync(h->dGi, 0, (size_t)n_rows * h->cfg.embed_k * sizeof(float), s));
     BPRX_HIP(h, hipMemsetAsync(h->dBi, 0, (size_t)n_rows * sizeof(float), s));
@@ -477,7 +518,7 @@
   return BPRX_OK;
 }
 
-extern "C" int bprx_step_end(bprx_handle *h, float *loss_out, void *stream) {
+static int step_end(bprx_handle *h, float *loss_out, void *stream, bool may_defer) {
   if (!h) return BPRX_E_INVALID;
   if (!h->step_stage) BPRX_FAIL(h, BPRX_E_STATE, "step_end without step_begin");
   if (h->step_stage != 2) BPRX_FAIL(h, BPRX_E_STATE, "step_end before step_begin_dense");
@@ -486,16 +527,23 @@
   int rc;
   h->step_stage = 0;
   if (h->factored && (rc = bprx_launch_fact_update(h, p.lr_t, s))) return rc;
-  if (p.dense_launch && (rc = bprx_launch_dense_update(h, p, s))) return rc;
+  const bool defer = may_defer && p.dense_launch && p.defer_ok && (!loss_out || h->loss_lag);
+  if (defer) {
+    h->pend.a = bprx_dense_args(h, p);
+    h->pend.loss_out = loss_out; h->pend.loss_B = p.B; h->pend.loss_nsq = h->dense_blocks; h->pend.loss_reg = h->cfg.reg;
+    h->pend.on = true;
+  } else if (p.dense_launch && (rc = bprx_launch_dense_update(h, p, s))) return rc;
   if (h->cfg.model == BPRX_MODEL_VBPR) {
     if (p.dense_launch) h->absmax_valid = h->cfg.feat_dtype == BPRX_F_FP8;
     if (p.list_mode) h->list_slot ^= 1;
     h->et_valid = p.dense_launch && h->cfg.feat_dtype == BPRX_F_BF16;
     h->p_valid = false;
   }
-  if (loss_out && (rc = bprx_launch_loss_reduce(h, p.B, loss_out, s))) return rc;
-  return BPRX_OK;
-}
+  if (loss_out && !defer && (rc = bprx_launch_loss_reduce(h, p.B, loss_out, s))) return rc;
+  return BPRX_OK;
+}
+
+extern "C" int bprx_step_end(bprx_handle *h, float *loss_out, void *stream) { return step_end(h, loss_out, stream, false); }
 
 extern "C" int bprx_step(bprx_handle *h, const int32_t *user, const int32_t *pos, const int32_t *neg, int64_t B,
                          float *loss_out, void *stream) {
@@ -509,7 +557,7 @@
     return rc ? rc : bprx_af_step(h, user, pos, neg, B, loss_out, (hipStream_t)stream);
   }
   int rc = step_begin(h, user, pos, neg, B, true, stream);
-  if (!rc) rc = bprx_step_end(h, loss_out, stream);
+  if (!rc) rc = step_end(h, loss_out, stream, true);
   return rc;
 }
 
@@ -519,6 +567,7 @@
   if (u0 < 0 || u1 > h->cfg.num_users || u0 > u1 || !out) BPRX_FAIL(h, BPRX_E_INVALID, "score_block: bad user range [%d,%d)", u0, u1);
   if (u0 == u1) return BPRX_OK;
   hipStream_t s = (hipStream_t)stream;
+  if ((rc = bprx_settle_pending(h, s))) return rc;
   if ((rc = bprx_launch_adam_sync(h, h->adam_t, s))) return rc;
   if (h->af) return bprx_af_block(h, u0, u1, out, nullptr, s);
   if (h->acf) {
@@ -562,6 +611,7 @@
   if (!Fnew || !P) BPRX_FAIL(h, BPRX_E_INVALID, "project_rows: null pointer");
   if ((uintptr_t)Fnew & 15) BPRX_FAIL(h, BPRX_E_INVALID, "project_rows: the table must be 16-byte aligned");
   hipStream_t s = (hipStream_t)stream;
+  if ((rc = bprx_settle_pending(h, s))) return rc;
   if ((rc = bprx_launch_adam_sync(h, h->adam_t, s))) return rc;
   if ((rc = bprx_launch_cast_Et(h, s))) return rc;
   return bprx_launch_proj_new(h, Fnew, n, P, s);
@@ -583,6 +633,7 @@
 extern "C" int bprx_sync_check(bprx_handle *h, void *stream) {
   if (!h) return BPRX_E_INVALID;
   hipStream_t s = (hipStream_t)stream;
+  { const int rc = bprx_settle_pending(h, s); if (rc) return rc; }
   int32_t flag = 0;
   BPRX_HIP(h, hipMemcpyAsync(&flag, h->errflag, sizeof(flag), hipMemcpyDeviceToHost, s));
   BPRX_HIP(h, hipStreamSynchronize(s));
diff --git a/fashionvisualexpl_recommend_amd/csrc/bprx_eval.hip b/fashionvisualexpl_recommend_amd/csrc/bprx_eval.hip
--- a/fashionvisualexpl_recommend_amd/csrc/bprx_eval.hip
+++ b/fashionvisualexpl_recommend_amd/csrc/bprx_eval.hip
@@ -371,6 +371,7 @@
 extern "C" int bprx_topk(bprx_handle *h, int32_t u0, int32_t u1, float *scores, const int64_t *train_ptr,
                          const int32_t *train_items, int32_t K, int32_t *idx, float *val, int32_t *flag, void *stream) {
   if (!h) return BPRX_E_INVALID;
+  { const int rc_ = bprx_settle_pending(h, (hipStream_t)stream); if (rc_) return rc_; }
   if (u0 < 0 || u1 > h->cfg.num_users || u0 > u1 || !scores || !train_ptr || !train_items || !idx || !val || !flag)
     BPRX_FAIL(h, BPRX_E_INVALID, "topk: bad argument");
   if (K <= 0 || K > TOPK_MAX) BPRX_FAIL(h, BPRX_E_INVALID, "topk: K=%d outside [1, %d]", K, TOPK_MAX);
@@ -385,6 +386,7 @@
                               int32_t *flag, void *stream) {
   const int rc = bprx_new_items_check(h, "topk_rows", nrows);
   if (rc) return rc;
+  { const int rc_ = bprx_settle_pending(h, (hipStream_t)stream); if (rc_) return rc_; }
   if (width < 1) BPRX_FAIL(h, BPRX_E_INVALID, "topk_rows: width = %d < 1", width);
   if (K <= 0 || K > TOPK_MAX) BPRX_FAIL(h, BPRX_E_INVALID, "topk_rows: K=%d outside [1, %d]", K, TOPK_MAX);
   if (nrows == 0) return BPRX_OK;
@@ -398,6 +400,7 @@
 extern "C" int bprx_score_new_block(bprx_handle *h, int32_t u0, int32_t u1, const float *P, int64_t n, float *out, void *stream) {
   int rc = bprx_new_items_check(h, "score_new_block", n);
   if (rc) return rc;
+  { const int rc_ = bprx_settle_pending(h, (hipStream_t)stream); if (rc_) return rc_; }
   if (u0 < 0 || u1 > h->cfg.num_users || u0 > u1) BPRX_FAIL(h, BPRX_E_INVALID, "score_new_block: bad user range [%d,%d)", u0, u1);
   if (n == 0 || u0 == u1) return BPRX_OK;
   if (!P || !out) BPRX_FAIL(h, BPRX_E_INVALID, "score_new_block: null pointer");
@@ -424,6 +427,7 @@
                                const int32_t *train_items, const int64_t *eval_ptr, const int32_t *eval_items, int32_t K,
                                double *out, void *stream) {
   if (!h) return BPRX_E_INVALID;
+  { const int rc_ = bprx_settle_pending(h, (hipStream_t)stream); if (rc_) return rc_; }
   if (u0 < 0 || u1 > h->cfg.num_users || u0 > u1 || !scores || !train_ptr || !train_items || !eval_ptr || !eval_items ||
       !out || K <= 0)
     BPRX_FAIL(h, BPRX_E_INVALID, "eval_users: bad argument");
@@ -437,6 +441,7 @@
 extern "C" int bprx_eval_pos(bprx_handle *h, int32_t u0, int32_t u1, const float *scores, int32_t item_lo, int32_t items_total,
                              const int64_t *eval_ptr, const int32_t *eval_items, float *sp, void *stream) {
   if (!h) return BPRX_E_INVALID;
+  { const int rc_ = bprx_settle_pending(h, (hipStream_t)stream); if (rc_) return rc_; }
   if (u0 < 0 || u0 > u1 || !scores || !eval_ptr || !eval_items || !sp || item_lo < 0 || items_total <= 0)
     BPRX_FAIL(h, BPRX_E_INVALID, "eval_pos: bad argument");
   if (u0 == u1) return BPRX_OK;
@@ -451,6 +456,7 @@
                                 const int64_t *train_ptr, const int32_t *train_items, const int64_t *eval_ptr,
                                 const int32_t *eval_items, const float *sp, int32_t *counts, void *stream) {
   if (!h) return BPRX_E_INVALID;
+  { const int rc_ = bprx_settle_pending(h, (hipStream_t)stream); if (rc_) return rc_; }
   if (u0 < 0 || u0 > u1 || !scores || !train_ptr || !train_items || !eval_ptr || !eval_items || !sp || !counts || item_lo < 0)
     BPRX_FAIL(h, BPRX_E_INVALID, "eval_counts: bad argument");
   if (u0 == u1) return BPRX_OK;
@@ -463,6 +469,7 @@
 extern "C" int bprx_eval_finish(bprx_handle *h, int32_t u0, int32_t u1, int32_t items_total, const int64_t *eval_ptr,
                                 const float *sp, const int32_t *counts, int32_t K, double *out, void *stream) {
   if (!h) return BPRX_E_INVALID;
+  { const int rc_ = bprx_settle_pending(h, (hipStream_t)stream); if (rc_) return rc_; }
   if (u0 < 0 || u0 > u1 || !eval_ptr || !sp || !counts || !out || K <= 0 || items_total <= 0)
     BPRX_FAIL(h, BPRX_E_INVALID, "eval_finish: bad argument");
   if (u0 == u1) return BPRX_OK;
diff --git a/fashionvisualexpl_recommend_amd/csrc/bprx_explain.hip b/fashionvisualexpl_recommend_amd/csrc/bprx_explain.hip
--- a/fashionvisualexpl_recommend_amd/csrc/bprx_explain.hip
+++ b/fashionvisualexpl_recommend_amd/csrc/bprx_explain.hip
@@ -223,6 +223,7 @@
                                  int32_t top, float *score, float *base, float *visual, int32_t *col, float *contrib, float *map,
                                  void *stream) {
   if (!h) return BPRX_E_INVALID;
+  { const int rc_ = bprx_settle_pending(h, (hipStream_t)stream); if (rc_) return rc_; }
   if (!h->bound) BPRX_FAIL(h, BPRX_E_STATE, "tables not bound (call bprx_bind_tables first)");
   if (h->cfg.model != BPRX_MODEL_VBPR || h->acf || h->af)
     BPRX_FAIL(h, BPRX_E_STATE, "feat_explain: needs a VBPR handle (bprx_bind_tables or bprx_bind_factored)");
@@ -262,6 +263,7 @@
                                      void *stream) {
   int rc = bprx_new_items_check(h, "feat_explain_new", n);
   if (rc) return rc;
+  { const int rc_ = bprx_settle_pending(h, (hipStream_t)stream); if (rc_) return rc_; }
   const bprx_config &c = h->cfg;
   if (n_new < 0 || n_new >= ((int64_t)1 << 31)) BPRX_FAIL(h, BPRX_E_INVALID, "feat_explain_new: n_new = %lld out of range", (long long)n_new);
   if (ncols < 1 || ncols > c.feat_dim) BPRX_FAIL(h, BPRX_E_INVALID, "feat_explain_new: ncols = %d outside [1, feat_dim = %d]", ncols, c.feat_dim);
diff --git a/fashionvisualexpl_recommend_amd/csrc/bprx_internal.h b/fashionvisualexpl_recommend_amd/csrc/bprx_internal.h
--- a/fashionvisualexpl_recommend_amd/csrc/bprx_internal.h
+++ b/fashionvisualexpl_recommend_amd/csrc/bprx_internal.h
@@ -93,9 +93,39 @@
   int apply;
   int fk, ek;
   bool dense_launch;
+  bool defer_ok;
+  bool carry_dense;
+  bool settle_first;
 };
 enum { PLAN_E_EMPTY = 1 };
 enum { APPLY_NONE = 0, APPLY_SGD_LIST, APPLY_SGD, APPLY_ADAM_LAZY, APPLY_ADAM_SWEEP };
+
+struct DenseArgs {
+  float *E, *Bp, *mE, *vE, *mBp, *vBp;
+  const float *dEp, *part;
+  int SK, D, d, PS, adam;
+  float lr_t, reg, b1, b2, eps;
+  double *sqpart;
+  float gscale;
+  uint16_t *Et, *EtF;
+  const int32_t *ilist, *ilist_n;
+  int32_t *ilist_n_next;
+  int bound;
+  float *W;
+  int32_t *cnt_reset;
+  uint32_t *absmax_out;
+  int upd;
+  int nvb, vT;
+};
+
+struct DensePending {
+  bool on;
+  DenseArgs a;
+  float *loss_out;
+  int64_t loss_B;
+  int loss_nsq;
+  float loss_reg;
+};
 
 struct bprx_handle {
   bprx_config cfg;
@@ -112,6 +142,9 @@
   float *lossb;
   double *loss_acc;
   int dense_blocks;
+  int dense_defer;
+  int loss_lag;
+  DensePending pend;
 
   StepPlan step;
   int step_stage;
@@ -229,6 +262,9 @@
 int bprx_launch_item_seg(bprx_handle *h, const StepPlan &p, hipStream_t s);
 int bprx_launch_apply(bprx_handle *h, const StepPlan &p, hipStream_t s);
 int bprx_launch_dense_update(bprx_handle *h, const StepPlan &p, hipStream_t s);
+DenseArgs bprx_dense_args(bprx_handle *h, const StepPlan &p);
+int bprx_launch_dense_args(bprx_handle *h, const DenseArgs &a, hipStream_t s);
+int bprx_settle_pending(bprx_handle *h, hipStream_t s);
 struct AdamSweepSeg { float *p, *m, *v, *g; size_t n; };
 struct AdamSweepAll { AdamSweepSeg seg[4]; uint32_t *flag[2]; size_t nflag[2]; };
 int bprx_launch_adam_sweep(bprx_handle *h, const AdamSweepAll &sw, float lr_t, hipStream_t s);
@@ -237,6 +273,7 @@
 int bprx_launch_adam_sync(bprx_handle *h, int64_t t, hipStream_t s);
 int bprx_launch_adam_reset(bprx_handle *h, int64_t t, hipStream_t s);
 int bprx_launch_loss_reduce(bprx_handle *h, int64_t B, float *loss_out, hipStream_t s);
+int bprx_launch_loss_reduce_at(bprx_handle *h, int64_t B, int nsq, float reg, float *loss_out, hipStream_t s);
 int bprx_launch_score_block(bprx_handle *h, int32_t u0, int32_t u1, float *out, hipStream_t s);
 int bprx_launch_score_gemm(bprx_handle *h, int32_t u0, int32_t u1, float *out, hipStream_t s);
 int bprx_launch_tile_F(bprx_handle *h);
@@ -300,6 +337,7 @@
   p.SK_step = B ? h.SK : h.step.SK_step;
   p.leaves_w_dirty = h.W_dirty;
   p.dense_launch = vb && (!h.factored || c.feat_dtype == BPRX_F_BF16);
+  p.settle_first = h.pend.on;
   if (B == 0) return p;
 
   p.list_mode = vb && !h.proj_fresh && (h.list_policy == 2 || (h.list_policy == 1 && 2 * B < I));
@@ -324,6 +362,10 @@
   p.mask = p.project && !p.list_mode && p.item_mode && !h.p_valid &&
            (h.proj_mask == 2 ? bf : (h.proj_mask == 1 && c.feat_dtype == BPRX_F_BF16 && h.PS / 16 <= 9));
   p.index_first = p.list_mode || p.mask;
+  p.defer_ok = h.dense_defer && p.dense_launch && p.fused_reduce && !p.list_mode && !h.factored;
+  p.carry_dense = h.pend.on && p.item_mode;
+  p.settle_first = h.pend.on && !p.carry_dense;
+  p.index_first = p.index_first || p.carry_dense;
   if (p.item_mode) {
     p.idx_kind = p.idx8 ? 2 : 1;
     int64_t nown = h.num_cu > 0 ? h.num_cu : 256;
diff --git a/fashionvisualexpl_recommend_amd/csrc/bprx_sparse.hip b/fashionvisualexpl_recommend_amd/csrc/bprx_sparse.hip
--- a/fashionvisualexpl_recommend_amd/csrc/bprx_sparse.hip
+++ b/fashionvisualexpl_recommend_amd/csrc/bprx_sparse.hip
@@ -691,36 +691,41 @@
 }
 
 constexpr int DU_KB = 8;
-__global__ __launch_bounds__(1024) void k_dense_update(float *__restrict__ E, float *__restrict__ Bp, float *mE, float *vE,
-                                                      float *mBp, float *vBp, const float *__restrict__ dEp,
-                                                      const float *__restrict__ part, int SK, int D, int d, int PS, int adam,
-                                                      float lr_t, float reg, float b1, float b2, float eps,
-                                                      double *__restrict__ sqpart, float gscale, uint16_t *__restrict__ Et,
-                                                      uint16_t *__restrict__ EtF, const int32_t *__restrict__ ilist,
-                                                      const int32_t *__restrict__ ilist_n, int32_t *__restrict__ ilist_n_next,
-                                                      int bound, float *__restrict__ W, int32_t *__restrict__ cnt_reset,
-                                                      uint32_t *__restrict__ absmax_out, int upd) {
-  __shared__ __attribute__((aligned(16))) uint16_t tile[DU_KB][288];
-  if (ilist_n_next && blockIdx.x == 0 && threadIdx.x == 0) *ilist_n_next = 0;
-  if (ilist) {
-    int n = *ilist_n;
-    n = n < bound ? n : bound;
+struct DenseLds {
+  __attribute__((aligned(16))) uint16_t tile[DU_KB][288];
+  double red[16];
+  uint32_t wm[16];
+};
+__device__ __forceinline__ void dense_update_block(const DenseArgs &a, const int vb, const int vt, const bool live, DenseLds &L) {
+  float *__restrict__ const E = a.E; float *__restrict__ const Bp = a.Bp;
+  float *const mE = a.mE, *const vE = a.vE, *const mBp = a.mBp, *const vBp = a.vBp;
+  const float *__restrict__ const dEp = a.dEp; const float *__restrict__ const part = a.part;
+  uint16_t *__restrict__ const Et = a.Et; uint16_t *__restrict__ const EtF = a.EtF;
+  const int SK = a.SK, D = a.D, d = a.d, PS = a.PS, adam = a.adam, upd = a.upd, nvb = a.nvb, vT = a.vT;
+  const float lr_t = a.lr_t, reg = a.reg, b1 = a.b1, b2 = a.b2, eps = a.eps, gscale = a.gscale;
+  uint16_t (*const tile)[288] = L.tile;
+  if (a.ilist_n_next && live && vb == 0 && vt == 0) *a.ilist_n_next = 0;
+  if (a.ilist && live) {
+    int n = *a.ilist_n;
+    n = n < a.bound ? n : a.bound;
     const int per = PS / 4;
-    for (int64_t e = (int64_t)blockIdx.x * blockDim.x + threadIdx.x; e < (int64_t)n * per; e += (int64_t)gridDim.x * blockDim.x) {
+    for (int64_t e = (int64_t)vb * vT + vt; e < (int64_t)n * per; e += (int64_t)nvb * vT) {
       const int p = (int)(e / per), c4 = (int)(e % per);
-      const int item = ilist[p];
-      reinterpret_cast<float4 *>(W + (size_t)item * PS)[c4] = make_float4(0.f, 0.f, 0.f, 0.f);
-      if (cnt_reset && c4 == 0) cnt_reset[item] = 0;
+      const int item = a.ilist[p];
+      reinterpret_cast<float4 *>(a.W + (size_t)item * PS)[c4] = make_float4(0.f, 0.f, 0.f, 0.f);
+      if (a.cnt_reset && c4 == 0) a.cnt_reset[item] = 0;
     }
   }
   double sq = 0.0;
   uint32_t amax = 0;
   const size_t total = (size_t)D * PS;
   const int ntile = (D + DU_KB - 1) / DU_KB;
-  for (int tl = blockIdx.x; tl < ntile; tl += gridDim.x) {
+  for (int t0 = 0; t0 < ntile; t0 += nvb) {
+    const int tl = t0 + vb;
+    const bool on = live && tl < ntile;
     const int k0 = tl * DU_KB;
     const int PQ = PS >> 2;
-    for (int q = threadIdx.x; q < DU_KB * PQ; q += (int)blockDim.x) {
+    for (int q = vt; on && q < DU_KB * PQ; q += vT) {
       const int kr = q / PQ, n4 = (q - kr * PQ) * 4, kk = k0 + kr;
       float nvv[4] = {0.f, 0.f, 0.f, 0.f};
       if (!upd && kk < D && n4 <= d) {
@@ -756,12 +761,12 @@
         }
         float *pp[4], *pm[4], *pv_[4];
         float pv[4], mo[4] = {0.f, 0.f, 0.f, 0.f}, vo[4] = {0.f, 0.f, 0.f, 0.f};
-        bool on[4];
+        bool on4[4];
 #pragma unroll
         for (int c = 0; c < 4; ++c) {
           const int n = n4 + c;
-          on[c] = n <= d;
-          const int nn = on[c] ? n : d;
+          on4[c] = n <= d;
+          const int nn = on4[c] ? n : d;
           pp[c] = nn < d ? E + (size_t)kk * d + nn : Bp + kk;
           pm[c] = adam ? (nn < d ? mE + (size_t)kk * d + nn : mBp + kk) : nullptr;
           pv_[c] = adam ? (nn < d ? vE + (size_t)kk * d + nn : vBp + kk) : nullptr;
@@ -773,7 +778,7 @@
         }
 #pragma unroll
         for (int c = 0; c < 4; ++c) {
-          if (!on[c]) continue;
+          if (!on4[c]) continue;
           sq += (double)pv[c] * (double)pv[c];
           const float gg = gs[c] + 2.f * reg * pv[c];
           float nv;
@@ -796,7 +801,7 @@
     }
     if (Et) {
       __syncthreads();
-      for (int n = threadIdx.x; n < PS; n += (int)blockDim.x) {
+      for (int n = vt; on && n < PS; n += vT) {
         uint4 v;
         v.x = (uint32_t)tile[0][n] | ((uint32_t)tile[1][n] << 16);
         v.y = (uint32_t)tile[2][n] | ((uint32_t)tile[3][n] << 16);
@@ -810,27 +815,30 @@
       __syncthreads();
     }
   }
-  __shared__ double red[16];
   sq = wave_sum(sq);
-  if ((threadIdx.x & 63) == 0) red[threadIdx.x >> 6] = sq;
+  if (live && (vt & 63) == 0) L.red[vt >> 6] = sq;
   __syncthreads();
-  if (threadIdx.x == 0 && sqpart) {
+  if (live && vt == 0 && a.sqpart) {
     double t = 0.0;
-    for (int q = 0; q < (int)(blockDim.x >> 6); ++q) t += red[q];
-    sqpart[blockIdx.x] = t;
-  }
-  if (absmax_out) {
-    __shared__ uint32_t wm[16];
+    for (int q = 0; q < (vT >> 6); ++q) t += L.red[q];
+    a.sqpart[vb] = t;
+  }
+  if (a.absmax_out) {
 #pragma unroll
     for (int o = 32; o > 0; o >>= 1) { const uint32_t v = __shfl_xor(amax, o, 64); amax = v > amax ? v : amax; }
-    if ((threadIdx.x & 63) == 0) wm[threadIdx.x >> 6] = amax;
+    if (live && (vt & 63) == 0) L.wm[vt >> 6] = amax;
     __syncthreads();
-    if (threadIdx.x == 0) {
-      uint32_t b = wm[0];
-      for (int q = 1; q < (int)(blockDim.x >> 6); ++q) b = wm[q] > b ? wm[q] : b;
-      if (b) atomicMax(absmax_out, b);
-    }
-  }
+    if (live && vt == 0) {
+      uint32_t b = L.wm[0];
+      for (int q = 1; q < (vT >> 6); ++q) b = L.wm[q] > b ? L.wm[q] : b;
+      if (b) atomicMax(a.absmax_out, b);
+    }
+  }
+}
+
+__global__ __launch_bounds__(1024) void k_dense_update(DenseArgs a) {
+  __shared__ DenseLds L;
+  dense_update_block(a, (int)blockIdx.x, (int)threadIdx.x, true, L);
 }
 
 __global__ __launch_bounds__(1024) void k_loss_reduce(const float *__restrict__ lossb, int64_t B,
@@ -878,6 +886,8 @@
   int aligned;
   const uint8_t *own8, *loc8;
   int wide;
+  int ndense;
+  DenseArgs dn;
 };
 
 __global__ __launch_bounds__(IX_T) void k_index_seg(IndexSegArgs a) {
@@ -911,6 +921,14 @@
       a.uslot_of[u] = (int)b;
       a.ulist[u_base + u_wcnt[wv] + __popcll(fm & (lane ? (~0ull >> (64 - lane)) : 0ull))] = u;
     }
+    return;
+  }
+  if ((int)blockIdx.x >= a.nuser + a.nown) {
+    __shared__ DenseLds dl[IX_T / 256];
+    const int S = IX_T / a.dn.vT, sub = tid / a.dn.vT;
+    const int vb = ((int)blockIdx.x - a.nuser - a.nown) * S + sub;
+    const bool live = sub < S && vb < a.dn.nvb;
+    dense_update_block(a.dn, vb, tid - sub * a.dn.vT, live, dl[live ? sub : 0]);
     return;
   }
   extern __shared__ __attribute__((aligned(16))) int cnt[];
@@ -1708,6 +1726,7 @@
 
 extern "C" int bprx_pack_user_msg(bprx_handle *h, const int32_t *user, int64_t B, int64_t cap, float *msg, void *stream) {
   if (!h || !msg || B < 0 || cap <= 0 || (B > 0 && !user)) return BPRX_E_INVALID;
+  { const int rc_ = bprx_settle_pending(h, (hipStream_t)stream); if (rc_) return rc_; }
   if (!(h->cfg.flags & BPRX_FLAG_EXPORT_USER_GRAD)) BPRX_FAIL(h, BPRX_E_STATE, "pack_user_msg needs BPRX_FLAG_EXPORT_USER_GRAD");
   if (!h->step_stage) BPRX_FAIL(h, BPRX_E_STATE, "pack_user_msg outside a step (after bprx_step_begin[_sparse])");
   if (B != h->step.B) BPRX_FAIL(h, BPRX_E_INVALID, "pack_user_msg: B differs from the pending step's");
@@ -1732,6 +1751,7 @@
 
 extern "C" int bprx_apply_user_msgs(bprx_handle *h, const float *msgs, int32_t nranks, int64_t cap, float scale, void *stream) {
   if (!h || !msgs || nranks <= 0 || cap <= 0) return BPRX_E_INVALID;
+  { const int rc_ = bprx_settle_pending(h, (hipStream_t)stream); if (rc_) return rc_; }
   if (!h->bound) BPRX_FAIL(h, BPRX_E_STATE, "tables not bound");
   if (!(h->cfg.flags & BPRX_FLAG_EXPORT_USER_GRAD)) BPRX_FAIL(h, BPRX_E_STATE, "apply_user_msgs needs BPRX_FLAG_EXPORT_USER_GRAD");
   if ((int64_t)nranks * cap >= ((int64_t)1 << 31) - 1) BPRX_FAIL(h, BPRX_E_INVALID, "nranks * cap too large");
@@ -1774,6 +1794,7 @@
 
 extern "C" int bprx_sum_dense_parts(bprx_handle *h, const float *parts, int32_t nranks, void *stream) {
   if (!h || !parts || nranks <= 0) return BPRX_E_INVALID;
+  { const int rc_ = bprx_settle_pending(h, (hipStream_t)stream); if (rc_) return rc_; }
   if (h->cfg.model != BPRX_MODEL_VBPR) BPRX_FAIL(h, BPRX_E_STATE, "sum_dense_parts: VBPR only");
   const size_t nd = (size_t)h->cfg.feat_dim * (h->cfg.embed_d + 1);
   unsigned blocks = (unsigned)((nd + 255) / 256);
@@ -1818,7 +1839,13 @@
     x.Wb = zw ? (uint16_t *)h->Wb : nullptr; x.PS = a.PS;
     x.aligned = (((uintptr_t)i | (uintptr_t)j) & 15) == 0;
     x.nuser = users ? (int)((B + IX_T - 1) / IX_T) : 0;
-    hipLaunchKernelGGL(k_index_seg, dim3((unsigned)(x.nown + x.nuser)), dim3(IX_T), (size_t)x.R * sizeof(int), s, x);
+    x.ndense = 0; x.dn = DenseArgs{};
+    if (p.carry_dense) {
+      x.dn = h->pend.a;
+      const int S = IX_T / x.dn.vT;
+      x.ndense = (x.dn.nvb + S - 1) / S;
+    }
+    hipLaunchKernelGGL(k_index_seg, dim3((unsigned)(x.nown + x.nuser + x.ndense)), dim3(IX_T), (size_t)x.R * sizeof(int), s, x);
     BPRX_LAUNCH_CHECK(h, "k_index_seg");
     return BPRX_OK;
   }
@@ -1976,37 +2003,53 @@
   return BPRX_OK;
 }
 
-int bprx_launch_dense_update(bprx_handle *h, const StepPlan &p, hipStream_t s) {
+DenseArgs bprx_dense_args(bprx_handle *h, const StepPlan &p) {
   const int D = h->cfg.feat_dim;
   unsigned blocks = (unsigned)((D + DU_KB - 1) / DU_KB);
   if (blocks > BPRX_DENSE_BLOCKS) blocks = BPRX_DENSE_BLOCKS;
   const bool upd = !h->factored;
   if (upd) h->dense_blocks = (int)blocks;
-  BprxProfScope ps(h, BPRX_PHASE_DENSE, s);
   const float *part = (p.fused_reduce && h->cfg.feat_dtype != BPRX_F_FP32) ? h->part : nullptr;
-  const float gscale = (part && h->cfg.feat_dtype == BPRX_F_FP8) ? 1.0f / h->cfg.feat_scale : 1.0f;
   const bool images = h->cfg.feat_dtype == BPRX_F_BF16;
   const bool lm = p.list_mode;
   int threads = (DU_KB * (h->PS / 4) + 63) / 64 * 64;
   threads = threads < 256 ? 256 : (threads > 1024 ? 1024 : threads);
-  hipLaunchKernelGGL(k_dense_update, dim3(blocks), dim3((unsigned)threads), 0, s, h->t.E, h->t.Bp, h->t.m_E, h->t.v_E, h->t.m_Bp,
-                     h->t.v_Bp, h->dEp, part, p.SK_step, D, h->cfg.embed_d, h->PS,
-                     h->cfg.optimizer == BPRX_OPT_ADAM_TF23 ? 1 : 0, p.lr_t, h->cfg.reg, h->cfg.beta1, h->cfg.beta2,
-                     h->cfg.epsilon, upd ? h->loss_acc : (double *)nullptr, gscale, images ? (uint16_t *)h->Et : (uint16_t *)nullptr, (uint16_t *)h->EtF,
-                     lm ? (const int32_t *)h->ilist : (const int32_t *)nullptr, (const int32_t *)p.list_cur,
-                     p.list_next, (int)p.list_bound, h->W,
-                     (lm && p.list_reset_cnt) ? h->cntI : (int32_t *)nullptr,
-                     h->cfg.feat_dtype == BPRX_F_FP8 ? (uint32_t *)h->qs + 2 + h->qs_slot : (uint32_t *)nullptr, upd ? 1 : 0);
+  DenseArgs a = {};
+  a.E = h->t.E; a.Bp = h->t.Bp; a.mE = h->t.m_E; a.vE = h->t.v_E; a.mBp = h->t.m_Bp; a.vBp = h->t.v_Bp;
+  a.dEp = h->dEp; a.part = part; a.SK = p.SK_step; a.D = D; a.d = h->cfg.embed_d; a.PS = h->PS;
+  a.adam = h->cfg.optimizer == BPRX_OPT_ADAM_TF23 ? 1 : 0;
+  a.lr_t = p.lr_t; a.reg = h->cfg.reg; a.b1 = h->cfg.beta1; a.b2 = h->cfg.beta2; a.eps = h->cfg.epsilon;
+  a.sqpart = upd ? h->loss_acc : nullptr;
+  a.gscale = (part && h->cfg.feat_dtype == BPRX_F_FP8) ? 1.0f / h->cfg.feat_scale : 1.0f;
+  a.Et = images ? (uint16_t *)h->Et : nullptr; a.EtF = (uint16_t *)h->EtF;
+  a.ilist = lm ? h->ilist : nullptr; a.ilist_n = p.list_cur; a.ilist_n_next = p.list_next; a.bound = (int)p.list_bound;
+  a.W = h->W; a.cnt_reset = (lm && p.list_reset_cnt) ? h->cntI : nullptr;
+  a.absmax_out = h->cfg.feat_dtype == BPRX_F_FP8 ? (uint32_t *)h->qs + 2 + h->qs_slot : nullptr;
+  a.upd = upd ? 1 : 0;
+  a.nvb = (int)blocks; a.vT = threads;
+  return a;
+}
+
+int bprx_launch_dense_args(bprx_handle *h, const DenseArgs &a, hipStream_t s) {
+  BprxProfScope ps(h, BPRX_PHASE_DENSE, s);
+  hipLaunchKernelGGL(k_dense_update, dim3((unsigned)a.nvb), dim3((unsigned)a.vT), 0, s, a);
   BPRX_LAUNCH_CHECK(h, "k_dense_update");
   return BPRX_OK;
 }
 
-int bprx_launch_loss_reduce(bprx_handle *h, int64_t B, float *loss_out, hipStream_t s) {
+int bprx_launch_dense_update(bprx_handle *h, const StepPlan &p, hipStream_t s) {
+  return bprx_launch_dense_args(h, bprx_dense_args(h, p), s);
+}
+
+int bprx_launch_loss_reduce_at(bprx_handle *h, int64_t B, int nsq, float reg, float *loss_out, hipStream_t s) {
   BprxProfScope ps(h, BPRX_PHASE_LOSS, s);
-  hipLaunchKernelGGL(k_loss_reduce, dim3(1), dim3(1024), 0, s, h->lossb, B, h->loss_acc,
-                     h->cfg.model == BPRX_MODEL_VBPR ? h->dense_blocks : 0, h->cfg.reg, loss_out);
+  hipLaunchKernelGGL(k_loss_reduce, dim3(1), dim3(1024), 0, s, h->lossb, B, h->loss_acc, nsq, reg, loss_out);
   BPRX_LAUNCH_CHECK(h, "k_loss_reduce");
   return BPRX_OK;
+}
+
+int bprx_launch_loss_reduce(bprx_handle *h, int64_t B, float *loss_out, hipStream_t s) {
+  return bprx_launch_loss_reduce_at(h, B, h->cfg.model == BPRX_MODEL_VBPR ? h->dense_blocks : 0, h->cfg.reg, loss_out, s);
 }
 
 int bprx_launch_score_block(bprx_handle *h, int32_t u0, int32_t u1, float *out, hipStream_t s) {
diff --git a/fashionvisualexpl_recommend_amd/engine.py b/fashionvisualexpl_recommend_amd/engine.py
--- a/fashionvisualexpl_recommend_amd/engine.py
+++ b/fashionvisualexpl_recommend_amd/engine.py
@@ -1,4 +1,5 @@
 import ctypes as C
+import weakref
 
 import numpy as np
 import torch
@@ -24,6 +25,46 @@
             t = t.to(torch.int32)
         return t.to(device, non_blocking=True).contiguous()
     return torch.as_tensor(np.ascontiguousarray(np.asarray(x).reshape(-1), dtype=np.int32), device=device)
+
+
+class _Bound(dict):
+
+    def __init__(self, engine, tensors):
+        super().__init__(tensors)
+        self._engine = weakref.ref(engine)
+
+    def _settle(self):
+        e = self._engine()
+        if e is not None:
+            e.settle()
+
+    def __getitem__(self, name):
+        self._settle()
+        return dict.__getitem__(self, name)
+
+    def get(self, name, default=None):
+        self._settle()
+        return dict.get(self, name, default)
+
+    def items(self):
+        self._settle()
+        return dict.items(self)
+
+    def values(self):
+        self._settle()
+        return dict.values(self)
+
+    def keys(self):
+        self._settle()
+        return dict.keys(self)
+
+    def __iter__(self):
+        self._settle()
+        return dict.__iter__(self)
+
+    def copy(self):
+        self._settle()
+        return dict(dict.items(self))
 
 
 class Engine:
@@ -56,19 +97,34 @@
 
     @property
     def t(self):
-        if self.optimizer == "adam_tf23" and getattr(self, "h", None) and self._t:
-            self.sync_adam()
+        if getattr(self, "h", None) and self._t:
+            self.settle()
+            if self.optimizer == "adam_tf23":
+                self.sync_adam()
         return self._t
 
     @t.setter
     def t(self, v):
-        self._t = v
+        self._t = _Bound(self, v)
 
     def adam_is_lazy(self):
         return bool(self.lib.bprx_adam_is_lazy(self.h))
 
     def sync_adam(self):
         _ffi.check(self.h, self.lib.bprx_sync_adam(self.h, _stream()))
+
+    def settle(self):
+        if getattr(self, "h", None) and hasattr(self.lib, "bprx_settle"):
+            _ffi.check(self.h, self.lib.bprx_settle(self.h, _stream()))
+
+    def dense_pending(self):
+        return bool(self.lib.bprx_dense_pending(self.h)) if hasattr(self.lib, "bprx_dense_pending") else False
+
+    def set_loss_lag(self, on):
+        if not on:
+            self.settle()
+        if getattr(self, "h", None) and hasattr(self.lib, "bprx_set_loss_lag"):
+            _ffi.check(self.h, self.lib.bprx_set_loss_lag(self.h, 1 if on else 0))
 
     def close(self):
         if getattr(self, "h", None):
diff --git a/fashionvisualexpl_recommend_amd/models.py b/fashionvisualexpl_recommend_amd/models.py
--- a/fashionvisualexpl_recommend_amd/models.py
+++ b/fashionvisualexpl_recommend_amd/models.py
@@ -147,25 +147,30 @@
         start_ep = time()
         print('Start training...')
         loss_buf = torch.zeros(max(1, steps_per_epoch), dtype=torch.float32, device=self.engine.device)
-        for batch in next_batch:
-            steps += 1
-            user, pos, neg = (as_index(b, self.engine.device) for b in batch)
-            self.engine.step(user, pos, neg, loss_out=loss_buf, loss_index=steps - 1)
-            if steps == steps_per_epoch:
-                loss = float(loss_buf[:steps].double().sum().item())
-                epoch_text = 'Epoch {0}/{1} \tLoss: {2:.3f}'.format(it, self.params.epochs, loss / steps)
-                epoch_print = self.evaluator.eval(it, results, epoch_text, start_ep)
-                for metric in max_metrics.keys():
-                    if max_metrics[metric] <= results[it][metric + '_v']:
-                        max_metrics[metric] = results[it][metric + '_v']
-                        if metric == self.params.best_metric:
-                            best_epoch, best_state, best_epoch_print = it, self.state_dict(), epoch_print
-                if (it % self.verbose == 0 or it == 1) and self.verbose != -1:
-                    torch.save(self.state_dict(), os.path.join(wdir, f'weights-{it}-{self.directory_parameters}.pt'))
-                start_ep = time()
-                it += 1
-                loss = 0
-                steps = 0
+        self.engine.set_loss_lag(True)
+        try:
+            for batch in next_batch:
+                steps += 1
+                user, pos, neg = (as_index(b, self.engine.device) for b in batch)
+                self.engine.step(user, pos, neg, loss_out=loss_buf, loss_index=steps - 1)
+                if steps == steps_per_epoch:
+                    self.engine.settle()
+                    loss = float(loss_buf[:steps].double().sum().item())
+                    epoch_text = 'Epoch {0}/{1} \tLoss: {2:.3f}'.format(it, self.params.epochs, loss / steps)
+                    epoch_print = self.evaluator.eval(it, results, epoch_text, start_ep)
+                    for metric in max_metrics.keys():
+                        if max_metrics[metric] <= results[it][metric + '_v']:
+                            max_metrics[metric] = results[it][metric + '_v']
+                            if metric == self.params.best_metric:
+                                best_epoch, best_state, best_epoch_print = it, self.state_dict(), epoch_print
+                    if (it % self.verbose == 0 or it == 1) and self.verbose != -1:
+                        torch.save(self.state_dict(), os.path.join(wdir, f'weights-{it}-{self.directory_parameters}.pt'))
+                    start_ep = time()
+                    it += 1
+                    loss = 0
+                    steps = 0
+        finally:
+            self.engine.set_loss_lag(False)
         print('Training end...')
         self._store_recs(os.path.join(rdir, f'recs-{it - 1}-{self.directory_parameters}.tsv'))
         with open(os.path.join(rdir, f'results-metrics-{self.directory_parameters}') + '.pkl', 'wb') as f:
diff --git a/include/bprx.h b/include/bprx.h
--- a/include/bprx.h
+++ b/include/bprx.h
@@ -76,6 +76,9 @@
 BPRX_API int bprx_set_hyper(bprx_handle *h, float lr, float reg);
 BPRX_API int bprx_set_adam_step(bprx_handle *h, int64_t iterations, void *stream);
 BPRX_API int bprx_sync_adam(bprx_handle *h, void *stream);
+BPRX_API int bprx_settle(bprx_handle *h, void *stream);
+BPRX_API int bprx_dense_pending(const bprx_handle *h);
+BPRX_API int bprx_set_loss_lag(bprx_handle *h, int on);
 BPRX_API int64_t bprx_get_adam_step(const bprx_handle *h);
 BPRX_API int bprx_adam_is_lazy(const bprx_handle *h);
 
```

Measured after the change: 318.4 million (median of 6 runs). 1.01x the previous value.
